# sbokov/AddingDisparityFiltering

Measured on AMD Instinct MI355X. Metric: filtered Mpixels/s (+ achieved HBM GB/s) on 4K disparity, 1/2/4/8 GPUs vs CPU ref, higher is better.
Workload: dtype f32

## Files before the change

addingdisparityfiltering_amd/__init__.py:

```python
from .ximgproc import (
    AM_MAX_TREE_HEIGHT,
    AdaptiveManifoldFilter,
    AdfError,
    BM_COST_CENSUS_CS,
    BM_COST_CENSUS_DENSE,
    BM_COST_CENSUS_SPARSE,
    BM_COST_MCT_DENSE,
    BM_COST_MCT_SPARSE,
    BM_COST_SAD,
    BORDER_CONSTANT,
    BORDER_DEFAULT,
    BORDER_REFLECT,
    BORDER_REFLECT_101,
    BORDER_REPLICATE,
    BORDER_WRAP,
    COLOR_BGR2GRAY,
    CV_16S,
    CV_32F,
    CV_32FC1,
    CV_8U,
    DTF_IC,
    DTF_NC,
    DTF_RF,
    DTFilter,
    DTWindowFilter,
    DT_MAX_ITERS,
    DT_NC_MAX_RADIUS,
    DisparityFilter,
    DisparityWLSFilter,
    FastGlobalSmootherFilter,
    GF_MAX_RADIUS,
    GuidedFilter,
    HANDOFF_IMAGE,
    HANDOFF_IMAGE_PAIR_TAIL,
    HANDOFF_PAIR_PLANE,
    INTER_LINEAR,
    JBF_MAX_RADIUS,
    PATH_CONF_BAND,
    PATH_FUSED_FIRST_PASS,
    PATH_MERGED_PREP,
    PATH_ROW_WEIGHTS_GUIDE,
    PATH_SCALED_FUSED,
    PATH_SCALED_HALF,
    RGF_MAX_ITERS,
    SGBM_COST_BT,
    SGBM_COST_CENSUS_CS,
    SGBM_COST_CENSUS_DENSE,
    SGBM_COST_CENSUS_SPARSE,
    SGBM_COST_MCT_DENSE,
    SGBM_COST_MCT_SPARSE,
    SGBM_RIGHT_FROM_VOLUME,
    SGBM_RIGHT_MATCHER,
    SOLVER_EXACT,
    SOLVER_WAVE,
    StereoBM,
    StereoMatcher,
    StereoSGBM,
    UNKNOWN_DISPARITY,
    WMF_COS,
    WMF_EXP,
    WMF_IV1,
    WMF_IV2,
    WMF_JAC,
    WMF_OFF,
    amFilter,
    amFilterWorkspaceBytes,
    amPlan,
    censusTransform,
    computeBadPixelPercent,
    computeMSE,
    createAMFilter,
    createDTFilter,
    createDTWindowFilter,
    createDisparityWLSFilter,
    createDisparityWLSFilterGeneric,
    createFastGlobalSmootherFilter,
    createGuidedFilter,
    createRightMatcher,
    cvtColor,
    dtFilter,
    dtFilterWorkspaceBytes,
    dtNcRadii,
    dtRfTable,
    dtWindowFilter,
    dtWindowFilterWorkspaceBytes,
    fastGlobalSmootherFilter,
    filterSpeckles,
    releaseCachedMemory,
    getDisparityVis,
    guidedFilter,
    guidedFilterWorkspaceBytes,
    halfSize,
    initUndistortRectifyMap,
    jbfTables,
    jointBilateralFilter,
    matcherViews,
    pointCloud,
    pointCloudWorkspaceBytes,
    readGT,
# ... 17 lines not shown
```

addingdisparityfiltering_amd/_lib.py:

```python
import ctypes as C
import os

_HERE = os.path.dirname(os.path.abspath(__file__))
LIB_PATH = os.environ.get("ADF_WLS_LIB") or os.path.join(_HERE, "libadf_wls.so")

ADF_OK, ADF_EBADARG, ADF_ESIZE, ADF_EHIP, ADF_ENOMEM, ADF_ENODEV = range(6)
SOLVER_EXACT, SOLVER_WAVE = 0, 1
PATH_CONF_BAND, PATH_FUSED_FIRST_PASS, PATH_MERGED_PREP, PATH_SCALED_FUSED, PATH_SCALED_HALF = 1, 2, 4, 8, 16
PATH_ROW_WEIGHTS_GUIDE = 32
HANDOFF_PAIR_PLANE, HANDOFF_IMAGE, HANDOFF_IMAGE_PAIR_TAIL = 0, 1, 2
DEPTH_8U, DEPTH_16S, DEPTH_32S, DEPTH_32F = 0, 3, 4, 5
SGBM_COST_BT, SGBM_COST_CENSUS_DENSE, SGBM_COST_CENSUS_SPARSE = 0, 1, 2
BM_COST_SAD, BM_COST_CENSUS_DENSE, BM_COST_CENSUS_SPARSE = 0, 1, 2
SGBM_COST_MCT_DENSE, SGBM_COST_MCT_SPARSE, SGBM_COST_CENSUS_CS = 4, 5, 6
BM_COST_MCT_DENSE, BM_COST_MCT_SPARSE, BM_COST_CENSUS_CS = 4, 5, 6
SGBM_RIGHT_MATCHER, SGBM_RIGHT_FROM_VOLUME = 0, 1
MISSING_NONE, MISSING_MIN, MISSING_VALUE = 0, 1, 2
WMF_EXP, WMF_IV1, WMF_IV2, WMF_COS, WMF_JAC, WMF_OFF = range(6)
WMF_WEIGHT_ONE, WMF_TABLE_LEVELS, WMF_MAX_RADIUS = 65536, 3 * 256 * 256, 31
GF_MAX_RADIUS = 31
DTF_NC, DTF_IC, DTF_RF, DT_MAX_ITERS = 0, 1, 2, 8
DT_NC_MAX_RADIUS = 127
JBF_MAX_RADIUS = 31
BORDER_REPLICATE, BORDER_REFLECT, BORDER_WRAP, BORDER_REFLECT_101 = 1, 2, 3, 4
RGF_MAX_ITERS = 16
AM_MAX_TREE_HEIGHT = 8


class AdfError(RuntimeError):

    def __init__(self, code, msg):
        super().__init__("adf error %d: %s" % (code, msg))
        self.code = code


class KernelTime(C.Structure):
    _fields_ = [("name", C.c_char * 48), ("launches", C.c_int), ("total_ms", C.c_double),
                ("alg_bytes", C.c_double), ("moved_bytes", C.c_double)]


class Rect(C.Structure):
    _fields_ = [("x", C.c_int), ("y", C.c_int), ("width", C.c_int), ("height", C.c_int)]


class ReprojectParams(C.Structure):
    _fields_ = [("Q", C.c_double * 16), ("disp_scale", C.c_double), ("missing_mode", C.c_int), ("missing_value", C.c_double)]


class RectifyParams(C.Structure):
    _fields_ = [("fx", C.c_double), ("fy", C.c_double), ("cx", C.c_double), ("cy", C.c_double),
                ("dist", C.c_double * 8), ("ir", C.c_double * 9)]


class AmPlan(C.Structure):
    _fields_ = [(k, C.c_int) for k in ("df", "height", "sh", "sw", "manifolds")] + \
               [(k, C.c_float) for k in ("a_root", "a_child", "sr2", "arg_w", "ss", "ratio", "ln_a", "arg_out")]


_vp, _i, _d, _pd, _sz = C.c_void_p, C.c_int, C.c_double, C.c_ssize_t, C.c_size_t
_FILTER_DEV = [_vp, _i, _vp, _pd, _pd, _vp, _pd, _pd, _i, _i, _i, _vp, _pd, _pd, _vp, _pd, _pd,
               C.POINTER(Rect), _vp]
_REPROJECT_DEV = [_i, _vp, _i, _pd, _pd, _i, _i, C.POINTER(ReprojectParams), _vp, _pd, _pd, _i, _vp, _sz, _vp]
_POINT_CLOUD_DEV = [_i, _vp, _i, _pd, _pd, _i, _i, C.POINTER(ReprojectParams), C.POINTER(Rect), _d, _d, _vp, _pd, _pd, _i,
                    _vp, _pd, _vp, _pd, _vp, _pd, _i, _vp, _vp, _sz, _vp]
_RECTIFY_MAP_DEV = [C.POINTER(RectifyParams), _i, _i, _vp, _pd, _vp, _pd, _vp]
_REMAP_DEV = [_i, _vp, _pd, _pd, _i, _i, _i, _vp, _pd, _vp, _pd, _vp, _pd, _pd, _i, _i, _i, _i, _vp, _vp]
_RECTIFY_VIEWS_DEV = [_i, _vp, _pd, _pd, _i, _i, _i, C.POINTER(RectifyParams), _vp, _pd, _pd, _i, _i, _i, _i, _vp, _vp]
_WMF_DEV = [_i, _vp, _pd, _pd, _i, _vp, _pd, _pd, _i, _vp, _pd, _pd, _i, _i, _i, _d, _i, _vp, _pd, _pd, _i, _d, _vp]
_GF_DEV = [_i, _vp, _pd, _pd, _i, _vp, _pd, _pd, _i, _vp, _pd, _pd, _i, _i, _i, _i, _d, _vp, _sz, _vp]
_DT_DEV = [_i, _vp, _pd, _pd, _i, _vp, _pd, _pd, _i, _vp, _pd, _pd, _i, _i, _i, _d, _d, _i, _i, _vp, _sz, _vp]
_JBF_DEV = [_i, _vp, _pd, _pd, _i, _vp, _pd, _pd, _i, _vp, _pd, _pd, _i, _i, _i, _i, _d, _d, _i, _vp]
_AM_DEV = [_i, _vp, _pd, _pd, _i, _vp, _pd, _pd, _i, _vp, _pd, _pd, _i, _i, _i, _d, _d, _i, _i, _vp, _sz, _vp]
_RGF_DEV = [_i, _vp, _pd, _pd, _vp, _pd, _pd, _i, _i, _i, _i, _d, _d, _i, _i, _vp, _sz, _vp]
_FILTER_SCALED_DEV = [_vp, _i, _vp, _pd, _pd, _i, _i, _vp, _pd, _pd, _i, _i, _i, _vp, _pd, _pd, _vp, _pd, _pd,
                      C.POINTER(Rect), _vp]
_FILTER_TYPED_DEV = _FILTER_SCALED_DEV[:5] + [_i] + _FILTER_SCALED_DEV[5:16] + [_i] + _FILTER_SCALED_DEV[16:]
SYMBOLS = [
    ("adf_version", _i, []),
    ("adf_last_error", C.c_char_p, []),
    ("adf_device_count", _i, []),
    ("adf_device_pci_bus_id", _i, [_i, C.c_char_p, _i]),
    ("adf_wls_create", _i, [C.POINTER(_vp), _i, _i, _i, _i, _i, _i]),
    ("adf_wls_destroy", None, [_vp]),
    ("adf_wls_set_lambda", _i, [_vp, _d]),
    ("adf_wls_get_lambda", _i, [_vp, C.POINTER(_d)]),
    ("adf_wls_set_sigma_color", _i, [_vp, _d]),
    ("adf_wls_get_sigma_color", _i, [_vp, C.POINTER(_d)]),
    ("adf_wls_set_lrc_thresh", _i, [_vp, _i]),
    ("adf_wls_get_lrc_thresh", _i, [_vp, C.POINTER(_i)]),
    ("adf_wls_set_depth_discontinuity_radius", _i, [_vp, _i]),
    ("adf_wls_get_depth_discontinuity_radius", _i, [_vp, C.POINTER(_i)]),
    ("adf_wls_set_fgs_params", _i, [_vp, _d, _i]),
    ("adf_wls_set_solver", _i, [_vp, _i]),
    ("adf_wls_get_solver", _i, [_vp, C.POINTER(_i)]),
    ("adf_wls_get_last_solver", _i, [_vp, C.POINTER(_i)]),
    ("adf_wls_get_last_path", _i, [_vp, C.POINTER(_i)]),
    ("adf_wls_get_last_solver_path", _i, [_vp, C.POINTER(_i)]),
    ("adf_wls_get_last_handoff", _i, [_vp, C.POINTER(_i)]),
    ("adf_wls_get_inner_handoffs", _i, [_vp, C.POINTER(_i), C.POINTER(_i)]),
    ("adf_wls_filter_device", _i, _FILTER_DEV),
    ("adf_wls_filter_host", _i, _FILTER_DEV[:-1]),
    ("adf_wls_filter_scaled_device", _i, _FILTER_SCALED_DEV),
    ("adf_wls_filter_scaled_host", _i, _FILTER_SCALED_DEV[:-1]),
    ("adf_wls_filter_f32_device", _i, _FILTER_DEV),
    ("adf_wls_filter_f32_host", _i, _FILTER_DEV[:-1]),
    ("adf_wls_filter_scaled_f32_device", _i, _FILTER_SCALED_DEV),
    ("adf_wls_filter_scaled_f32_host", _i, _FILTER_SCALED_DEV[:-1]),
    ("adf_wls_filter_typed_device", _i, _FILTER_TYPED_DEV),
    ("adf_wls_filter_typed_host", _i, _FILTER_TYPED_DEV[:-1]),
    ("adf_wls_get_confidence_device", _i, [_vp, _i, _vp, _pd, _vp]),
    ("adf_wls_get_confidence_host", _i, [_vp, _i, _vp, _pd]),
    ("adf_wls_get_device", _i, [_vp, C.POINTER(_i)]),
    ("adf_wls_get_roi", _i, [_vp, C.POINTER(Rect)]),
    ("adf_wls_sync", _i, [_vp, _vp]),
    ("adf_wls_workspace_bytes", _sz, [_vp]),
    ("adf_wls_profile_enable", _i, [_vp, _i]),
    ("adf_wls_profile_read", _i, [_vp, _vp, _i, C.POINTER(_i)]),
    ("adf_fgs_create", _i, [C.POINTER(_vp), _vp, _pd, _i, _i, _i, _d, _d, _d, _i, _i]),
    ("adf_fgs_create_device", _i, [C.POINTER(_vp), _vp, _pd, _i, _i, _i, _d, _d, _d, _i, _i, _vp]),
    ("adf_fgs_destroy", None, [_vp]),
    ("adf_release_cached_memory", None, []),
    ("adf_weight_table_host", _i, [C.c_float, _vp, _i]),
    ("adf_fgs_get_device", _i, [_vp, C.POINTER(_i)]),
    ("adf_fgs_get_solver", _i, [_vp, C.POINTER(_i)]),
    ("adf_fgs_filter_host", _i, [_vp, _vp, _pd, _vp, _pd, _i, _i]),
    ("adf_fgs_filter_device", _i, [_vp, _vp, _pd, _vp, _pd, _i, _i, _vp]),
    ("adf_compute_mse_host", _i, [_vp, _pd, _vp, _pd, _i, _i, C.POINTER(Rect), C.POINTER(_d)]),
    ("adf_compute_mse_device", _i, [_vp, _pd, _vp, _pd, _i, _i, C.POINTER(Rect), C.POINTER(_d), _vp]),
    ("adf_compute_bad_pixel_percent_host", _i, [_vp, _pd, _vp, _pd, _i, _i, C.POINTER(Rect), _i, C.POINTER(_d)]),
    ("adf_compute_bad_pixel_percent_device", _i, [_vp, _pd, _vp, _pd, _i, _i, C.POINTER(Rect), _i, C.POINTER(_d), _vp]),
    ("adf_get_disparity_vis_host", _i, [_vp, _pd, _vp, _pd, _i, _i, _d]),
    ("adf_get_disparity_vis_device", _i, [_vp, _pd, _vp, _pd, _i, _i, _d, _vp]),
    ("adf_bm_create", _i, [C.POINTER(_vp), _i, _i]),
    ("adf_bm_destroy", None, [_vp]),
    ("adf_bm_set_params", _i, [_vp, _i, _i, _i, _i, _i, _i]),
    ("adf_bm_get_device", _i, [_vp, C.POINTER(_i)]),
    ("adf_bm_get_params", _i, [_vp] + [C.POINTER(_i)] * 6),
    ("adf_bm_set_cost", _i, [_vp, _i, _i]),
    ("adf_bm_get_cost", _i, [_vp, C.POINTER(_i), C.POINTER(_i)]),
    ("adf_bm_compute_device", _i, [_vp, _i, _vp, _pd, _pd, _vp, _pd, _pd, _i, _i, _vp, _pd, _pd, _vp]),
    ("adf_bm_compute_both_device", _i, [_vp, _i, _vp, _pd, _pd, _vp, _pd, _pd, _i, _i, _vp, _pd, _pd, _vp, _pd, _pd, _vp]),
    ("adf_bm_compute_host", _i, [_vp, _i, _vp, _pd, _pd, _vp, _pd, _pd, _i, _i, _vp, _pd, _pd]),
    ("adf_bm_compute_cost_device", _i, [_vp, _i, _vp, _pd, _pd, _vp, _pd, _pd, _i, _i, _vp, _pd, _pd, _vp, _pd, _pd, _vp]),
    ("adf_bm_compute_cost_host", _i, [_vp, _i, _vp, _pd, _pd, _vp, _pd, _pd, _i, _i, _vp, _pd, _pd, _vp, _pd, _pd]),
    ("adf_bm_compute_both_cost_device", _i, [_vp, _i, _vp, _pd, _pd, _vp, _pd, _pd, _i, _i] + [_vp, _pd, _pd] * 4 + [_vp]),
    ("adf_sgbm_create", _i, [C.POINTER(_vp), _i, _i, _i]),
    ("adf_sgbm_destroy", None, [_vp]),
    ("adf_sgbm_get_device", _i, [_vp, C.POINTER(_i)]),
    ("adf_sgbm_set_params", _i, [_vp] + [_i] * 8),
    ("adf_sgbm_get_params", _i, [_vp] + [C.POINTER(_i)] * 8),
    ("adf_sgbm_set_disp12_max_diff", _i, [_vp, _i]),
    ("adf_sgbm_get_disp12_max_diff", _i, [_vp, C.POINTER(_i)]),
    ("adf_sgbm_set_cost", _i, [_vp, _i, _i]),
    ("adf_sgbm_get_cost", _i, [_vp, C.POINTER(_i), C.POINTER(_i)]),
    ("adf_sgbm_compute_device", _i, [_vp, _i, _vp, _pd, _pd, _vp, _pd, _pd, _i, _i, _i, _vp, _pd, _pd, _vp]),
    ("adf_sgbm_compute_host", _i, [_vp, _i, _vp, _pd, _pd, _vp, _pd, _pd, _i, _i, _i, _vp, _pd, _pd]),
    ("adf_sgbm_compute_both_device", _i, [_vp, _i, _vp, _pd, _pd, _vp, _pd, _pd, _i, _i, _i, _vp, _pd, _pd, _vp, _pd, _pd, _i, _vp]),
    ("adf_sgbm_compute_both_host", _i, [_vp, _i, _vp, _pd, _pd, _vp, _pd, _pd, _i, _i, _i, _vp, _pd, _pd, _vp, _pd, _pd, _i]),
    ("adf_census_transform_device", _i, [_i, _vp, _pd, _pd, _i, _i, _i, _i, _vp, _pd, _pd, _vp]),
    ("adf_census_transform_host", _i, [_i, _vp, _pd, _pd, _i, _i, _i, _i, _vp, _pd, _pd]),
    ("adf_filter_speckles_workspace_bytes", _sz, [_i, _i, _i]),
    ("adf_filter_speckles_device", _i, [_i, _vp, _pd, _pd, _i, _i, _i, _i, _i, _vp, _sz, _vp]),
    ("adf_filter_speckles_host", _i, [_i, _vp, _pd, _pd, _i, _i, _i, _i, _i]),
    ("adf_validate_disparity_device", _i, [_i, _vp, _pd, _pd, _vp, _pd, _pd, _i, _i, _i, _i, _i, _i, _vp]),
    ("adf_validate_disparity_host", _i, [_i, _vp, _pd, _pd, _vp, _pd, _pd, _i, _i, _i, _i, _i, _i]),
    ("adf_half_size", _i, [_i, C.POINTER(_i)]),
    ("adf_prepare_views_device", _i, [_i, _vp, _pd, _pd, _i, _i, _i, _vp, _pd, _pd, _i, _i, _i, _vp]),
    ("adf_prepare_views_host", _i, [_i, _vp, _pd, _pd, _i, _i, _i, _vp, _pd, _pd, _i, _i, _i]),
    ("adf_reproject_workspace_bytes", _sz, [_i]),
    ("adf_reproject_to_3d_device", _i, _REPROJECT_DEV),
    ("adf_reproject_to_3d_host", _i, _REPROJECT_DEV[:-3]),
    ("adf_point_cloud_workspace_bytes", _sz, [_i, _i, _i]),
    ("adf_point_cloud_device", _i, _POINT_CLOUD_DEV),
    ("adf_point_cloud_host", _i, _POINT_CLOUD_DEV[:-3]),
    ("adf_rectify_params_init", _i, [_vp, _vp, _i, _vp, _vp, _i, C.POINTER(RectifyParams)]),
    ("adf_init_undistort_rectify_map_device", _i, _RECTIFY_MAP_DEV),
    ("adf_init_undistort_rectify_map_host", _i, _RECTIFY_MAP_DEV[:-1]),
    ("adf_remap_device", _i, _REMAP_DEV),
    ("adf_remap_host", _i, _REMAP_DEV[:-1]),
    ("adf_rectify_views_device", _i, _RECTIFY_VIEWS_DEV),
    ("adf_rectify_views_host", _i, _RECTIFY_VIEWS_DEV[:-1]),
    ("adf_wmf_weight_table_host", _i, [_d, _i, _vp, _i]),
    ("adf_weighted_median_filter_device", _i, _WMF_DEV),
    ("adf_weighted_median_filter_host", _i, _WMF_DEV[:-1]),
    ("adf_guided_filter_workspace_bytes", _sz, [_i, _i, _i, _i]),
    ("adf_guided_filter_device", _i, _GF_DEV),
    ("adf_guided_filter_host", _i, _GF_DEV[:-3]),
    ("adf_dt_filter_workspace_bytes", _sz, [_i, _i, _i]),
    ("adf_dt_rf_table_host", _i, [_d, _d, _i, _i, _vp]),
    ("adf_dt_filter_device", _i, _DT_DEV),
    ("adf_dt_filter_host", _i, _DT_DEV[:-3]),
    ("adf_dt_window_filter_workspace_bytes", _sz, [_i, _i, _i]),
    ("adf_dt_nc_radii_host", _i, [_d, _i, _vp]),
    ("adf_dt_window_filter_device", _i, _DT_DEV),
    ("adf_dt_window_filter_host", _i, _DT_DEV[:-3]),
    ("adf_jbf_tables_host", _i, [_i, _d, _d, _i, _vp, _vp, C.POINTER(_i)]),
    ("adf_joint_bilateral_filter_device", _i, _JBF_DEV),
    ("adf_joint_bilateral_filter_host", _i, _JBF_DEV[:-1]),
    ("adf_rolling_guidance_workspace_bytes", _sz, [_i, _i, _i, _i, _i]),
    ("adf_rgf_tables_host", _i, [_i, _i, _d, _d, _vp, _vp, C.POINTER(_i), C.POINTER(_i), C.POINTER(C.c_float)]),
    ("adf_rolling_guidance_filter_device", _i, _RGF_DEV),
    ("adf_rolling_guidance_filter_host", _i, _RGF_DEV[:-3]),
    ("adf_am_plan_host", _i, [_d, _d, _i, _i, _i, C.POINTER(AmPlan), _vp]),
    ("adf_am_exp_host", _i, [_vp, _vp, _sz]),
    ("adf_am_filter_workspace_bytes", _sz, [_i, _i, _i, _i, _d, _d, _i]),
# ... 38 lines not shown
```

addingdisparityfiltering_amd/csrc/adf_api.hip:

```cpp
#include "adf_host.h"

#include <cmath>
#include <cstdio>
#include <cstdlib>
#include <cstring>
#include <new>

using namespace adf;

static inline int round_up(int v, int m) { return (v + m - 1) / m * m; }
template <class T> static const T* pairs_on(const T* p, ptrdiff_t pair_stride, int k)
{
    return p ? (const T*)((const char*)p + (ptrdiff_t)k * pair_stride) : nullptr;
}

static Geom make_geom(int W, int H, int rx, int ry, int rw, int rh)
{
    Geom g;
    g.W = W; g.H = H; g.rx = rx; g.ry = ry; g.rw = rw; g.rh = rh;
    g.pw = round_up(rw, 64);
    g.ph = round_up(rh, 64);
    size_t a = (size_t)round_up(rh, TILE_ROWS) * g.pw, b = (size_t)rw * g.ph;
    g.plane = ((a > b ? a : b) + 63) / 64 * 64;
    g.frame = (size_t)W * H;
// ... 1 lines not shown
    g.cpitch = round_up(W + g.cx0 + 3, 4);
    g.cframe = (size_t)g.cpitch * H;
    return g;
}

static Geom plain_conf_layout(Geom g) { g.cx0 = 0; g.cpitch = g.W; g.cframe = g.frame; return g; }

enum KClass { K_FILL = 0, K_WEIGHTS, K_DISC, K_LRC, K_PROLOGUE, K_PASS_H_FIRST, K_PASS_H, K_PASS_V, K_PASS_V_LAST, K_RESIZE, K_QUANT, K_COUNT };
static const char* const kclass_names[K_COUNT] = {"fill_outside", "weights", "discontinuity", "lrc_confidence",
                                                  "plain_prologue", "pass_h_first", "pass_h", "pass_v", "pass_v_last", "resize", "quantise_maps"};
struct Bytes { double alg, moved; };
static Bytes same_bytes(double b) { return Bytes{b, b}; }
static Bytes fill_bytes(double outside, bool conf, double out_b) { return same_bytes(((conf ? 4.0 : 0.0) + out_b) * outside); }
static Bytes weights_bytes(double P, int gch, bool chor) { return same_bytes((gch + (chor ? 8.0 : 4.0)) * P); }
static Bytes disc_bytes(double P, bool both) { return both ? Bytes{4.0 * P, 12.0 * P} : Bytes{2.0 * P, 6.0 * P}; }
static Bytes band_bytes(double P) { return same_bytes(8.0 * P); }
static Bytes merged_bytes(double P, double outside, int gch, double out_b) { return same_bytes((8.0 + gch + 8.0) * P + (4.0 + out_b) * outside); }
static Bytes conf_left_bytes(double P, bool rhs) { const double wu = rhs ? 8.0 : 0.0; return Bytes{(4.0 + wu) * P, (12.0 + wu) * P}; }
static Bytes lrc_bytes(double F, double P, bool rhs, double map_b, double fill)
{
    return Bytes{4.0 * F + (rhs ? 8.0 * P : 0.0) + fill, 4.0 * F + (rhs ? 18.0 + map_b : 12.0) * P + fill};
}
static Bytes prologue_bytes(double P, bool weighted, double map_b) { return same_bytes(((weighted ? 12.0 : 4.0) + map_b) * P); }
static Bytes resize_bytes(double dst_px, double src_px, double elem_b) { return same_bytes(elem_b * dst_px + elem_b * src_px); }
static Bytes quant_bytes(double px, bool q, bool right, bool v) { return same_bytes(((right ? 8.0 : 4.0) + (q ? (right ? 4.0 : 2.0) : 0.0) + (v ? 4.0 : 0.0)) * px); }

struct Profiler {
    bool on = false;
    struct Rec { int cls; hipEvent_t a, b; double alg, moved; };
    std::vector<Rec> recs;
    std::vector<hipEvent_t> pool;
    hipEvent_t get()
    {
        if (!pool.empty()) { hipEvent_t e = pool.back(); pool.pop_back(); return e; }
        hipEvent_t e = nullptr;
        if (hipEventCreate(&e) != hipSuccess) return nullptr;
        return e;
    }
    void clear() { for (auto& r : recs) { pool.push_back(r.a); pool.push_back(r.b); } recs.clear(); }
    void destroy() { clear(); for (auto e : pool) hipEventDestroy(e); pool.clear(); }
};
struct ProfScope {
    Profiler* p; hipStream_t st; Profiler::Rec r{};
    ProfScope(Profiler* prof, int cls, double alg, double moved, hipStream_t s) : p(prof && prof->on ? prof : nullptr), st(s)
    {
        if (!p) return;
        r.cls = cls; r.alg = alg; r.moved = moved; r.a = p->get(); r.b = p->get();
        if (r.a) hipEventRecord(r.a, st);
    }
    ProfScope(Profiler* prof, int cls, Bytes b, hipStream_t s) : ProfScope(prof, cls, b.alg, b.moved, s) {}
    ~ProfScope()
    {
        if (!p) return;
        if (r.b) hipEventRecord(r.b, st);
        if (r.a && r.b) p->recs.push_back(r);
    }
};

struct SolvePlanes {
    float* CH; float* CV;
    float* D; float* F0; float* F1;
    float* A0; float* A1;
    float* B0; float* B1;
};

struct FinalOut {
    int epilogue; void* out; ptrdiff_t stride, pair_stride; int x0, y0, cn, c;
};

static double epilogue_bytes(int epilogue)
{
    return (epilogue == EPI_F32 || epilogue == EPI_WLS_CONF_F32) ? 4.0 : epilogue == EPI_U8 ? 1.0 : 2.0;
}

template <class Args>
static void set_final_out(Args& a, const FinalOut& fo)
{
    a.out = fo.out; a.out_stride = fo.stride; a.out_pair_stride = fo.pair_stride;
    a.out_x0 = fo.x0; a.out_y0 = fo.y0; a.out_cn = fo.cn; a.out_c = fo.c;
}

struct HandoffImage {
    float* image = nullptr; int m = 0; bool inner = false, first = false;
    bool at(int it, int num_iter) const
    {
        if (!image || num_iter < 2) return false;
        return it == num_iter - 1 ? true : it > 0 ? inner : first;
    }
    int inner_count(int num_iter) const
    {
        int n = 0;
        for (int it = 0; it + 1 < num_iter; it++) n += at(it, num_iter);
        return n;
    }
};

static int run_passes(bool wave, const Geom& g, const SolvePlanes& p, int n_rhs, float lambda, float atten, int num_iter,
                      const FinalOut& fo, int n_pairs, hipStream_t st, Profiler* prof = nullptr,
                      const FusedInputs* fuse = nullptr, const GuideWeights* gw = nullptr, const HandoffImage& ho = HandoffImage{})
{
    const double px = (double)g.rw * g.rh * n_pairs;
    float lam = lambda;
    for (int it = 0; it < num_iter; it++, lam *= atten) {
        const bool fused = it == 0 && fuse, last = it == num_iter - 1;
        const int epi = last ? fo.epilogue : EPI_PLANES;
        const double lo_b = (fused && fuse->lo_conf) ? 6.0 * fuse->lo_scale_x * fuse->lo_scale_y : (fused && fuse->dl_f32) ? 8.0 : 6.0;
        const double wb = gw ? (double)gw->ch : 4.0;
        const double hb = fused ? (wb + lo_b + 8.0) * px : (wb + 8.0 * n_rhs) * px;
        const double out_b = (last ? epilogue_bytes(fo.epilogue) : 4.0 * n_rhs) * px;
        const double vb = (4.0 + 4.0 * n_rhs) * px + out_b;
        if (wave) {
            WavePassArgs h{}, v{};
            h.C = p.CH; h.U0 = p.A0; h.U1 = p.A1;
            h.nscan = g.rh; h.len = g.rw; h.pitch = g.pw; h.plane = g.plane; h.lambda = lam;
            if (fused) h.fuse = *fuse;
            if (gw) h.gw = *gw;
            v.C = p.CV; v.U0 = p.A0; v.U1 = p.A1;
            v.nscan = g.rw; v.len = g.rh; v.pitch = g.pw; v.plane = g.plane; v.lambda = lam;
            if (last) set_final_out(v, fo);
            if (ho.at(it, num_iter)) {
                h.image = v.image = ho.image; h.image_m = v.image_m = ho.m;
                h.image_plane = v.image_plane = wave_image_floats(g.pw, ho.m);
            }
            {
                ProfScope ps(prof, fused ? K_PASS_H_FIRST : K_PASS_H, hb, hb, st);
                HIP_TRY(launch_wave_hpass(h, n_rhs, n_pairs, st));
            }
            ProfScope ps(prof, last ? K_PASS_V_LAST : K_PASS_V, vb, vb, st);
            HIP_TRY(launch_wave_vpass(v, n_rhs, epi, n_pairs, st));
        } else {
            PassArgs h{}, v{};
            h.C = p.CH; h.U0 = p.A0; h.U1 = p.A1; h.D = p.D; h.F0 = p.F0; h.F1 = p.F1; h.O0 = p.B0; h.O1 = p.B1;
            h.nscan = g.rh; h.len = g.rw; h.pitch_in = g.ph; h.pitch_out = g.pw; h.plane = g.plane; h.lambda = lam;
            v.C = p.CV; v.U0 = p.B0; v.U1 = p.B1; v.D = p.D; v.F0 = p.F0; v.F1 = p.F1; v.O0 = p.A0; v.O1 = p.A1;
            v.nscan = g.rw; v.len = g.rh; v.pitch_in = g.pw; v.pitch_out = g.ph; v.plane = g.plane; v.lambda = lam;
            if (last) set_final_out(v, fo);
            {
                ProfScope ps(prof, K_PASS_H, hb, (12.0 + 16.0 * n_rhs) * px, st);
                HIP_TRY(launch_exact_pass(h, n_rhs, EPI_PLANES, n_pairs, st));
            }
            ProfScope ps(prof, last ? K_PASS_V_LAST : K_PASS_V, vb, (12.0 + 12.0 * n_rhs) * px + out_b, st);
            HIP_TRY(launch_exact_pass(v, n_rhs, epi, n_pairs, st));
        }
    }
    return ADF_OK;
}

static bool wave_fits(const Geom& g)
{
    return g.rw >= 2 && g.rh >= 2 && g.rw <= wave_max_row_len() && g.rh <= wave_max_col_len();
}

struct ConfResize {
    float* clo; int dW, dH; adf_rect rlo;
    Geom ghi;
    bool band_map;
    int n_pairs;
};

constexpr long long HANDOFF_IMAGE_MIN_PX = 12LL * 3584 * 2160;

struct adf_wls {
    int device = 0;
    int left_offset = 0, right_offset = 0, top_offset = 0, bottom_offset = 0;
    int min_disp = 0;
    bool use_confidence = true;
    double lambda = 8000.0, sigma_color = 1.0;
    int lrc_thresh = 24, disc_radius = 5;
    float roll_off = 0.001f;
    double atten = 0.25; int num_iter = 3;
    int solver = ADF_SOLVER_WAVE;
    int last_solver = ADF_SOLVER_WAVE;
    adf_rect roi{0, 0, 0, 0};
    int last_W = 0, last_H = 0, last_pairs = 0;
    int last_cpitch = 0, last_cx0 = 0;
    long long conf_sig[4] = {0, 0, 0, 0};
    int last_path = 0;
    int last_solver_path = 0;
    Lut lut;
    DevBuf ws;
    DevBuf conf;
    DevBuf stage;
    DevBuf scaled;
    size_t ws_limit = (size_t)64 << 30;
    Profiler prof;
    long long ws_sig[8] = {0, 0, 0, 0, 0, 0, 0, 0};
    hipStream_t side = nullptr;
    hipEvent_t ev_fork = nullptr, ev_join = nullptr;
    bool overlap = true;
    struct LazyConf { bool pending = false; ConfResize resize{}; } lazy_conf;
    bool scaled_half = true;
    bool scaled_fuse = true;
    bool conf_band = true;
    bool merge_small = true;
    bool row_weights_guide = true;
    bool handoff_image = true;
    bool handoff_inner = true;
    long long handoff_min_px = HANDOFF_IMAGE_MIN_PX;
    int last_handoff = ADF_HANDOFF_PAIR_PLANE;
    int last_inner[2] = {0, 0};
    static bool null_caller_of(hipStream_t s) { return s == nullptr || s == hipStreamLegacy || s == hipStreamPerThread; }
    int ensure_side(hipStream_t caller)
    {
        if (side) return ADF_OK;
        int least = 0, greatest = 0, prio = 0, cp = 0;
        if (hipDeviceGetStreamPriorityRange(&least, &greatest) != hipSuccess) { least = greatest = 0; (void)hipGetLastError(); }
        if (null_caller_of(caller) || stream_is_capturing(caller) || hipStreamGetPriority(caller, &cp) != hipSuccess) { cp = 0; (void)hipGetLastError(); }
        prio = (cp != greatest) ? greatest : (greatest < least ? greatest + 1 : greatest);
        if (null_caller_of(caller)) HIP_TRY(hipStreamCreateWithFlags(&side, hipStreamNonBlocking));
        else HIP_TRY(hipStreamCreateWithPriority(&side, hipStreamNonBlocking, prio));
        HIP_TRY(hipEventCreateWithFlags(&ev_fork, hipEventDisableTiming));
        HIP_TRY(hipEventCreateWithFlags(&ev_join, hipEventDisableTiming));
        return ADF_OK;
    }
};

extern "C" int adf_wls_create(adf_wls_t** out, int use_confidence, int l, int r, int t, int b, int min_disp)
{
    if (!out) return fail(ADF_EBADARG, "adf_wls_create: out is NULL");
    *out = nullptr;
    if (l < 0 || r < 0 || t < 0 || b < 0) return fail(ADF_EBADARG, "adf_wls_create: negative offset");
    int n = 0;
    if (hipGetDeviceCount(&n) != hipSuccess || n <= 0)
        return fail(ADF_ENODEV, "adf_wls_create: no HIP device visible");
    adf_wls* h = new (std::nothrow) adf_wls();
    if (!h) return fail(ADF_ENOMEM, "adf_wls_create: out of host memory");
    if (hipGetDevice(&h->device) != hipSuccess) { delete h; return fail(ADF_EHIP, "hipGetDevice failed"); }
    h->use_confidence = use_confidence != 0;
    h->left_offset = l; h->right_offset = r; h->top_offset = t; h->bottom_offset = b;
    h->min_disp = 0; (void)min_disp;
    if (const char* e = getenv("ADF_WS_LIMIT_GB")) {
        double gb = atof(e);
        if (gb > 0) h->ws_limit = (size_t)(gb * (double)((size_t)1 << 30));
    }
    if (const char* e = getenv("ADF_NO_OVERLAP")) h->overlap = atoi(e) == 0;
    if (const char* e = getenv("ADF_CONF_BAND")) h->conf_band = atoi(e) != 0;
    if (const char* e = getenv("ADF_SCALED_FUSE")) h->scaled_fuse = atoi(e) != 0;
    if (const char* e = getenv("ADF_ROW_WEIGHTS_GUIDE")) h->row_weights_guide = atoi(e) != 0;
    if (const char* e = getenv("ADF_LO_HALF")) h->scaled_half = atoi(e) != 0;
    if (const char* e = getenv("ADF_LAST_HANDOFF_IMAGE")) h->handoff_image = atoi(e) != 0;
    if (const char* e = getenv("ADF_INNER_HANDOFF_IMAGE")) h->handoff_inner = atoi(e) != 0;
    if (const char* e = getenv("ADF_LAST_HANDOFF_MIN_PX")) h->handoff_min_px = atoll(e);
    if (const char* e = getenv("ADF_MERGE_SMALL")) h->merge_small = atoi(e) != 0;
    *out = h;
    return ADF_OK;
}

extern "C" void adf_wls_destroy(adf_wls_t* h)
{
    if (!h) return;
    DeviceScope ds(h->device);
    h->lut.release(); h->ws.release(); h->conf.release(); h->stage.release(); h->scaled.release();
    h->prof.destroy();
    if (h->ev_fork) hipEventDestroy(h->ev_fork);
    if (h->ev_join) hipEventDestroy(h->ev_join);
    if (h->side) hipStreamDestroy(h->side);
    delete h;
}


extern "C" int adf_wls_set_lambda(adf_wls_t* h, double v) { NEED_HANDLE(h); h->lambda = v; return ADF_OK; }
extern "C" int adf_wls_get_lambda(const adf_wls_t* h, double* v) { NEED_HANDLE(h); if (v) *v = h->lambda; return ADF_OK; }
extern "C" int adf_wls_set_sigma_color(adf_wls_t* h, double v) { NEED_HANDLE(h); h->sigma_color = v; return ADF_OK; }
extern "C" int adf_wls_get_sigma_color(const adf_wls_t* h, double* v) { NEED_HANDLE(h); if (v) *v = h->sigma_color; return ADF_OK; }
extern "C" int adf_wls_set_lrc_thresh(adf_wls_t* h, int v) { NEED_HANDLE(h); h->lrc_thresh = v; return ADF_OK; }
extern "C" int adf_wls_get_lrc_thresh(const adf_wls_t* h, int* v) { NEED_HANDLE(h); if (v) *v = h->lrc_thresh; return ADF_OK; }
extern "C" int adf_wls_set_depth_discontinuity_radius(adf_wls_t* h, int v) { NEED_HANDLE(h); h->disc_radius = v; return ADF_OK; }
extern "C" int adf_wls_get_depth_discontinuity_radius(const adf_wls_t* h, int* v) { NEED_HANDLE(h); if (v) *v = h->disc_radius; return ADF_OK; }

extern "C" int adf_wls_set_fgs_params(adf_wls_t* h, double atten, int num_iter)
{
    NEED_HANDLE(h);
    if (num_iter < 1) return fail(ADF_EBADARG, "num_iter must be >= 1 (FGS.cpp:143)");
    h->atten = atten; h->num_iter = num_iter;
    return ADF_OK;
}

extern "C" int adf_wls_set_solver(adf_wls_t* h, int solver)
{
    NEED_HANDLE(h);
    if (solver != ADF_SOLVER_EXACT && solver != ADF_SOLVER_WAVE) return fail(ADF_EBADARG, "unknown solver %d", solver);
    h->solver = solver;
    return ADF_OK;
}
extern "C" int adf_wls_get_solver(const adf_wls_t* h, int* v) { NEED_HANDLE(h); if (v) *v = h->solver; return ADF_OK; }
extern "C" int adf_wls_get_last_solver(const adf_wls_t* h, int* v) { NEED_HANDLE(h); if (v) *v = h->last_solver; return ADF_OK; }
extern "C" int adf_wls_get_last_path(const adf_wls_t* h, int* v) { NEED_HANDLE(h); if (v) *v = h->last_path; return ADF_OK; }
extern "C" int adf_wls_get_last_solver_path(const adf_wls_t* h, int* v) { NEED_HANDLE(h); if (v) *v = h->last_solver_path; return ADF_OK; }
extern "C" int adf_wls_get_last_handoff(const adf_wls_t* h, int* v) { NEED_HANDLE(h); if (v) *v = h->last_handoff; return ADF_OK; }

extern "C" int adf_wls_get_inner_handoffs(const adf_wls_t* h, int* full, int* tail)
{
    NEED_HANDLE(h);
    if (full) *full = h->last_inner[0];
    if (tail) *tail = h->last_inner[1];
    return ADF_OK;
}

extern "C" int adf_wls_get_device(const adf_wls_t* h, int* device) { NEED_HANDLE(h); if (device) *device = h->device; return ADF_OK; }
extern "C" int adf_wls_get_roi(const adf_wls_t* h, adf_rect* roi) { NEED_HANDLE(h); if (roi) *roi = h->roi; return ADF_OK; }
extern "C" size_t adf_wls_workspace_bytes(const adf_wls_t* h)
{
    return h ? h->ws.bytes + h->conf.bytes + h->stage.bytes + h->scaled.bytes + h->lut.bytes() : 0;
}

extern "C" int adf_wls_sync(adf_wls_t* h, void* stream)
{
    NEED_HANDLE(h);
    DeviceScope ds(h->device);
    HIP_TRY(hipStreamSynchronize((hipStream_t)stream));
    return ADF_OK;
}

static int ensure_conf_planes(adf_wls* h, const Geom& g, int n_pairs, hipStream_t st)
{
    int rc = h->conf.reserve(g.cframe * sizeof(float) * (size_t)n_pairs, st, FILL_ZERO);
    if (rc) return rc;
    const long long sig[4] = {g.W, g.H, g.cx0, n_pairs};
    if (memcmp(sig, h->conf_sig, sizeof(sig)) != 0) {
        HIP_TRY(hipMemsetAsync(h->conf.p, 0, h->conf.bytes, st));
        memcpy(h->conf_sig, sig, sizeof(sig));
    }
    return ADF_OK;
}

static int quant_pitch(int W) { return round_up(W, 8); }

static size_t wls_pair_ws_bytes(const Geom& g, bool conf, bool wave, bool disc_maps, bool quant_planes, int image_m = 0, bool image_in_chor = false)
{
    size_t planes = wave ? (conf ? 4 : 3) : (conf ? 9 : 6);
    return planes * g.plane * sizeof(float) + (conf && disc_maps ? 2 * g.frame * sizeof(float) : 0) +
           (image_m ? (wave_image_floats(g.pw, image_m) - (image_in_chor ? g.plane : 0)) * sizeof(float) : 0) +
           (quant_planes ? 2 * (size_t)quant_pitch(g.W) * g.H * sizeof(int16_t) : 0);
}

static int resolve_roi(const adf_wls* h, const adf_rect* roi_in, int w, int hgt, adf_rect& roi)
{
    if (roi_in && roi_in->width * roi_in->height != 0) roi = *roi_in;
    else roi = adf_rect{h->left_offset, h->top_offset, w - h->left_offset - h->right_offset, hgt - h->top_offset - h->bottom_offset};
    if (roi.width <= 0 || roi.height <= 0 || roi.x < 0 || roi.y < 0 || roi.x + roi.width > w || roi.y + roi.height > hgt)
        return fail(ADF_ESIZE, "ROI (%d,%d,%d,%d) does not fit a %dx%d map", roi.x, roi.y, roi.width, roi.height, w, hgt);
    return ADF_OK;
}

struct OutMap {
    void* p; ptrdiff_t stride, pair_stride; bool f32;
    size_t esz() const { return f32 ? sizeof(float) : sizeof(int16_t); }
};

struct DispMaps {
    const void* L; ptrdiff_t sL, psL;
    const void* R; ptrdiff_t sR, psR;
    bool f32;
    size_t esz() const { return f32 ? sizeof(float) : sizeof(int16_t); }
    DispMaps from(int k) const { return DispMaps{pairs_on(L, psL, k), sL, psL, pairs_on(R, psR, k), sR, psR, f32}; }
};

struct View { const uint8_t* p; ptrdiff_t stride, pair_stride; int ch, W, H; };

struct WlsCall {
    int n_pairs;
    DispMaps dm; int dW, dH;
    View view;
    OutMap om;
    adf_rect rlo, rhi;
    float resize_factor, x_ratio;
    bool scaled;
};

static int no_right_map() { return fail(ADF_EBADARG, "disparity_map_right is required with use_confidence"); }
static int bad_view_channels() { return fail(ADF_EBADARG, "left_view must be CV_8UC1 or CV_8UC3"); }

static int check_float_maps(const DispMaps& dm, int n_pairs, int dW, int dH, const OutMap& om, int W, int H)
{
    if (!dm.f32) return ADF_OK;
    if ((reinterpret_cast<uintptr_t>(dm.L) | (uintptr_t)dm.sL | (uintptr_t)dm.psL) & 3u ||
        (dm.R && ((reinterpret_cast<uintptr_t>(dm.R) | (uintptr_t)dm.sR | (uintptr_t)dm.psR) & 3u)))
        return fail(ADF_EBADARG, "a float disparity map needs a 4-byte aligned base and strides");
// ... 160 lines not shown
    CONF_SCALED_LO,
    CONF_MERGED,
    CONF_BAND,
    CONF_LEFT,
    CONF_TWO_KERNEL,
};

enum RhsSource {
    RHS_PLAIN,
    RHS_FUSED_VIEW,
    RHS_FUSED_LO,
    RHS_CONF_PROLOGUE,
    RHS_CONF_KERNEL,
};

struct ConfRule { int rrx, thresh, radius; float roll_off; };
static ConfRule conf_rule(const adf_wls* h, const WlsCall& c)
{
    return ConfRule{c.dW - (c.rlo.x + c.rlo.width),
                    (int)(c.resize_factor * h->lrc_thresh),
                    h->disc_radius, h->roll_off / (c.resize_factor * c.resize_factor)};
}

struct ConfOut {
    float* conf;
    float* cL; float* cR;
    float* U0; float* U1; int orient;
    const OutsideArgs* fill;
};

static ConfBandArgs conf_band_args(const MapSource& m, float* conf, const Geom& g, const ConfRule& r)
{
    return ConfBandArgs{m.L, m.sL, m.psL, m.R, m.sR, m.psR, conf, g, r.rrx, r.thresh, r.radius, r.roll_off, 0};
}

static DiscArgs disc_args(const MapSource& m, const ConfOut& o, const Geom& g, const ConfRule& r, int only_view)
{
    return DiscArgs{{m.L, m.R}, {m.sL, m.sR}, {m.psL, m.psR}, {g.rx, r.rrx}, g.ry, g.rw, g.rh, r.radius, r.roll_off,
                    {o.cL, o.cR}, g.W, g.frame, only_view};
}

static LrcArgs lrc_args(const MapSource& m, const ConfOut& o, const Geom& g, const ConfRule& r)
{
    const bool own_f32 = o.U0 && m.rhs_f32();
    LrcArgs a = LrcArgs{m.L, m.sL, m.psL, m.R, m.sR, m.psR, o.cL, o.cR, o.conf, nullptr, 0, 0, 0, 0, o.U0, o.U1,
                        g, r.rrx, r.thresh, o.orient, own_f32 ? 1 : 0};
    if (own_f32) { a.dL = (const int16_t*)m.rhs; a.sL = m.s_rhs; a.psL = m.ps_rhs; }
    if (o.fill) { a.out = o.fill->out; a.sO = o.fill->stride; a.psO = o.fill->pair_stride; a.fill = o.fill->fill; a.out_f32 = o.fill->out_f32; }
    return a;
}

static int conf_stage(Profiler* prof, ConfStage kind, const MapSource& m, const Geom& g, const ConfRule& r, const ConfOut& o,
                      int n, hipStream_t st)
{
    const double F = (double)g.frame * n, P = (double)g.rw * g.rh * n;
    if (kind == CONF_BAND) {
        ProfScope ps(prof, K_LRC, band_bytes(P), st);
        HIP_TRY(launch_conf_band(conf_band_args(m, o.conf, g, r), n, st));
        return ADF_OK;
    }
    {
        ProfScope ps(prof, K_DISC, disc_bytes(P, kind != CONF_LEFT), st);
        HIP_TRY(launch_discontinuity(disc_args(m, o, g, r, kind == CONF_LEFT ? 1 : -1), n, st));
    }
    if (kind == CONF_LEFT) {
        ConfLeftArgs ca{m.L, m.sL, m.psL, m.R, m.sR, m.psR, o.cR, o.conf, o.U0, o.U1, g, r.rrx, r.thresh, r.radius, r.roll_off};
        ProfScope ps(prof, K_LRC, conf_left_bytes(P, o.U0 != nullptr), st);
        HIP_TRY(launch_conf_left(ca, n, st));
        return ADF_OK;
    }
    const double fill = o.fill ? fill_bytes(F - P, false, o.fill->out_f32 ? 4.0 : 2.0).alg : 0.0;
    ProfScope ps(prof, K_LRC, lrc_bytes(F, P, o.U0 != nullptr, m.rhs_f32() ? 4.0 : 2.0, fill), st);
    HIP_TRY(launch_lrc_prologue(lrc_args(m, o, g, r), n, st));
    return ADF_OK;
}

struct ChunkPlan {
    ConfStage stage;
    bool fork_weights;
    bool outside_on_side;
    bool guide_rows;
    bool image;
    bool inner_image;
};

struct WlsPlan {
    Geom g;
    bool wave;
    RhsSource rhs;
    bool band;
    bool quant_planes;
    Geom glo; bool lo_band; size_t dhi_bytes;
    size_t per_pair; int chunk;
    int image_m;
    bool image_in_chor;
    bool first_image;
    ChunkPlan full, tail;
    int path;
    int solver_path;
    bool fused_first() const { return rhs == RHS_FUSED_VIEW || rhs == RHS_FUSED_LO; }
};

static ChunkPlan plan_chunk(const adf_wls* h, ConfStage stage, bool wave, bool guide_rows, bool image, bool inner_image)
{
    const bool fork = stage != CONF_NONE && stage != CONF_MERGED && h->overlap;
    return ChunkPlan{stage, fork, fork && wave && stage != CONF_TWO_KERNEL, guide_rows && stage != CONF_MERGED, image, image && inner_image};
}

static GuideWeights guide_weights(const adf_wls* h, const uint8_t* guide, const View& v, const Geom& g)
{
    return GuideWeights{guide, v.stride, v.pair_stride, v.ch, g.rx, g.ry, h->lut.cur};
}

static WlsPlan plan_wls(const adf_wls* h, const WlsCall& c)
{
    WlsPlan p{};
    const bool conf = h->use_confidence, f32in = c.dm.f32;
    const View& v = c.view;
    const Geom g = p.g = make_geom(v.W, v.H, c.rhi.x, c.rhi.y, c.rhi.width, c.rhi.height);
    p.wave = h->solver == ADF_SOLVER_WAVE && wave_fits(g);
    MapSource m = caller_maps(c.dm);
    bool fuse_lo = false;
    if (c.scaled) {
        p.glo = plain_conf_layout(make_geom(c.dW, c.dH, c.rlo.x, c.rlo.y, c.rlo.width, c.rlo.height));
        p.lo_band = conf && h->conf_band && conf_band_fits(p.glo, h->disc_radius);
        fuse_lo = conf && !f32in && h->scaled_fuse && p.wave &&
                  wave_hpass_can_fuse_lo(first_pass_probe(lo_fuse(h, c, p.lo_band, UNALLOCATED, m, nullptr, g), g.rw));
        p.dhi_bytes = fuse_lo ? 0 : pad_to((size_t)v.W * v.H * c.dm.esz(), 256);
        m.rhs = fuse_lo ? nullptr : UNALLOCATED; m.s_rhs = (ptrdiff_t)(v.W * c.dm.esz()); m.ps_rhs = (ptrdiff_t)p.dhi_bytes;
        m.rhs_depth = f32in ? ADF_32F : ADF_16S;
    }
    ConfStage stage = !conf ? CONF_NONE
                    : c.scaled ? (fuse_lo ? CONF_SCALED_LO : CONF_SCALED)
                    : (p.wave && h->disc_radius <= conf_left_max_radius()) ? CONF_LEFT : CONF_TWO_KERNEL;
    const float* planes = h->conf.p ? (const float*)h->conf.p : UNALLOCATED;
    const bool fused_view = ((stage == CONF_SCALED && !f32in) || stage == CONF_LEFT) && p.wave &&
                            wave_hpass_can_fuse(first_pass_probe(view_fuse(planes, m, g), g.rw));
    p.band = stage == CONF_LEFT && fused_view && h->conf_band && conf_band_fits(g, h->disc_radius);
    if (p.band) stage = CONF_BAND;
    p.quant_planes = f32in && conf && !c.scaled;
    p.rhs = stage == CONF_NONE ? RHS_PLAIN : stage == CONF_SCALED_LO ? RHS_FUSED_LO : fused_view ? RHS_FUSED_VIEW
          : (stage == CONF_SCALED || (stage == CONF_LEFT && p.quant_planes)) ? RHS_CONF_PROLOGUE : RHS_CONF_KERNEL;
    bool guide_rows = false;
    if (p.wave && !c.scaled && h->row_weights_guide) {
        WavePassArgs probe{};
        probe.len = g.rw; probe.gw = guide_weights(h, v.p, v, g);
        WeightArgs wprobe{};
        wprobe.stride = v.stride; wprobe.ch = v.ch; wprobe.chor_orient = ORIENT_N; wprobe.g = g;
        guide_rows = wave_hpass_guide_fits(probe) && weights_stream_fits(wprobe);
    }
    const int image_m = (conf && p.wave && h->handoff_image && h->num_iter >= 2 && wave_hpass_image_fits(g.rw)) ? wave_vpass_image_m(g.rh) : 0;
    const long long roi_px = (long long)g.rw * g.rh;
    const bool may_merge = p.band && h->merge_small && prep_small_fits(g, h->disc_radius, v.ch, 1) && prep_small_guide_fits(g, v.stride, v.ch);
    auto chunk_for = [&](int im) {
        p.image_m = im;
        p.image_in_chor = im && guide_rows && !may_merge;
        p.per_pair = wls_pair_ws_bytes(g, conf, p.wave, !p.band, p.quant_planes, im, p.image_in_chor);
        p.chunk = (int)(h->ws_limit / p.per_pair);
        if (p.chunk < 1) p.chunk = 1;
        if (p.chunk > c.n_pairs) p.chunk = c.n_pairs;
    };
    chunk_for(image_m);
    if (image_m && roi_px * p.chunk < h->handoff_min_px) chunk_for(0);
    auto chunk_of = [&](int n) {
        const bool merged = p.band && h->merge_small && prep_small_fits(g, h->disc_radius, v.ch, n) && prep_small_guide_fits(g, v.stride, v.ch);
        return plan_chunk(h, merged ? CONF_MERGED : stage, p.wave, guide_rows, p.image_m && roi_px * n >= h->handoff_min_px, h->handoff_inner);
    };
    p.first_image = p.rhs == RHS_FUSED_VIEW && wave_hpass_first_image(view_fuse(planes, m, g));
    p.full = chunk_of(p.chunk);
    p.tail = chunk_of(c.n_pairs % p.chunk ? c.n_pairs % p.chunk : p.chunk);
    p.path = ((p.band || p.lo_band) ? ADF_PATH_CONF_BAND : 0) |
             (p.fused_first() ? ADF_PATH_FUSED_FIRST_PASS : 0) |
             ((p.full.stage == CONF_MERGED || p.tail.stage == CONF_MERGED) ? ADF_PATH_MERGED_PREP : 0);
    p.solver_path = (p.full.guide_rows || p.tail.guide_rows) ? ADF_PATH_ROW_WEIGHTS_GUIDE : 0;
    if (p.rhs == RHS_FUSED_LO)
        p.path |= ADF_PATH_SCALED_FUSED |
                  (wave_hpass_lo_half(first_pass_probe(lo_fuse(h, c, p.lo_band, UNALLOCATED, m, nullptr, g), g.rw)) ? ADF_PATH_SCALED_HALF : 0);
    return p;
}

struct ScaledBufs { char* dhi; float *cl, *cr, *clo; float* taps; };

static int scaled_buffers(adf_wls_t* h, const WlsCall& c, const WlsPlan& plan, hipStream_t st, ScaledBufs& b, MapSource& lo)
{
    const bool conf = h->use_confidence, f32in = c.dm.f32, fuse_lo = plan.rhs == RHS_FUSED_LO;
    const size_t n = (size_t)c.n_pairs, lo_px = (size_t)c.dW * c.dH;
    const size_t qframe = (size_t)quant_pitch(c.dW) * c.dH;
    const size_t maps_bytes = pad_to(n * (plan.dhi_bytes + (conf ? 3 * lo_px * sizeof(float) : 0)), 256);
    const size_t taps_bytes = pad_to(fuse_lo ? 2 * ((size_t)c.rhi.width + 4) * sizeof(float) : 0, 256);
    const size_t quant_bytes = f32in ? n * qframe * (4 + (conf ? 4 : 0)) : 0;
    int rc = h->scaled.reserve(maps_bytes + taps_bytes + quant_bytes, st, FILL_ZERO);
    if (rc) return rc;
    b.dhi = (char*)h->scaled.p;
    b.cl = (float*)(b.dhi + n * plan.dhi_bytes);
    b.cr = b.cl + n * lo_px;
    b.clo = b.cr + n * lo_px;
    b.taps = fuse_lo ? (float*)(b.dhi + maps_bytes) : nullptr;
    if (conf && (rc = ensure_conf_planes(h, plan.g, c.n_pairs, st))) return rc;
    lo = caller_maps(c.dm);
    if (f32in) {
        float* v = (float*)(b.dhi + maps_bytes + taps_bytes);
        int16_t* qL = conf ? (int16_t*)(v + n * qframe) : nullptr;
        int16_t* qR = conf ? qL + n * qframe : nullptr;
        if ((rc = quantise_maps(&h->prof, c.dm, c.dW, c.dH, c.n_pairs, qL, qR, v, st, lo))) return rc;
    }
    lo.rhs = fuse_lo ? nullptr : b.dhi; lo.s_rhs = (ptrdiff_t)(c.view.W * c.dm.esz()); lo.ps_rhs = (ptrdiff_t)plan.dhi_bytes;
    lo.rhs_depth = f32in ? ADF_32F : ADF_16S;
    return ADF_OK;
}

static int scaled_conf_maps(adf_wls_t* h, const WlsCall& c, const WlsPlan& plan, const ScaledBufs& b, const MapSource& lo,
                            const ConfRule& rule, hipStream_t st)
{
    Profiler* prof = &h->prof;
    int rc = conf_stage(prof, plan.lo_band ? CONF_BAND : CONF_TWO_KERNEL, lo, plan.glo, rule, ConfOut{b.clo, b.cl, b.cr}, c.n_pairs, st);
    if (rc) return rc;
    const ConfResize cr{b.clo, c.dW, c.dH, c.rlo, plan.g, plan.lo_band, c.n_pairs};
    if (plan.rhs != RHS_FUSED_LO)
        return (rc = resize_conf_planes(h, cr, st, prof)) ? rc : resize_disparity(prof, c, lo, b.dhi, st);
    if (stream_is_capturing(st)) return resize_conf_planes(h, cr, st, prof);
    h->lazy_conf = adf_wls::LazyConf{true, cr};
    return ADF_OK;
}

static int wls_filter_impl(adf_wls_t* h, const WlsCall& c, const WlsPlan& plan, hipStream_t st)
{
    const bool conf = h->use_confidence, wave = plan.wave;
    const Geom& g = plan.g;
    const View& vw = c.view;
    const OutMap& om = c.om;
    const adf_rect& roi = c.rhi;
    const int n_pairs = c.n_pairs, W = vw.W, H = vw.H, gch = vw.ch;
    const double ob_px = (double)om.esz(), db_px = (double)c.dm.esz();
    Profiler* prof = &h->prof;
    int rc;
    ScaledBufs sb{};
    MapSource lo{};
    if (c.scaled && (rc = scaled_buffers(h, c, plan, st, sb, lo))) return rc;
    h->roi = roi; h->last_W = W; h->last_H = H; h->last_pairs = n_pairs;
    h->last_cpitch = g.cpitch; h->last_cx0 = g.cx0; h->last_path = 0; h->last_solver_path = 0;
    h->last_solver = wave ? ADF_SOLVER_WAVE : ADF_SOLVER_EXACT;
    h->last_handoff = ADF_HANDOFF_PAIR_PLANE; h->last_inner[0] = h->last_inner[1] = 0;
    if ((rc = h->ws.reserve(plan.per_pair * (size_t)plan.chunk, st, FILL_ZERO))) return rc;
    if (conf && !c.scaled && (rc = ensure_conf_planes(h, g, n_pairs, st))) return rc;
    {
        const long long sig[8] = {W, H, roi.x, roi.y, roi.width, roi.height,
                                  (long long)plan.image_in_chor * 1024 + (long long)plan.image_m * 16 + (long long)plan.quant_planes * 8 + (long long)plan.band * 4 + (long long)wave * 2 + conf, plan.chunk};
        if (memcmp(sig, h->ws_sig, sizeof(sig)) != 0) {
            HIP_TRY(hipMemsetAsync(h->ws.p, 0, h->ws.bytes, st));
            memcpy(h->ws_sig, sig, sizeof(sig));
        }
    }
    float* base = (float*)h->ws.p;
    auto take = [&](size_t elems) { float* p = base; base += elems * (size_t)plan.chunk; return p; };
    SolvePlanes p{};
    p.CH = take(g.plane);
    float* const image_rest = plan.image_in_chor ? take(wave_image_floats(g.pw, plan.image_m) - g.plane) : nullptr;
    (void)image_rest;
    p.CV = take(g.plane); p.A0 = take(g.plane);
    if (!wave) { p.D = take(g.plane); p.F0 = take(g.plane); p.B0 = take(g.plane); }
    float *cL = nullptr, *cR = nullptr;
    if (conf) {
        p.A1 = take(g.plane);
        if (!wave) { p.F1 = take(g.plane); p.B1 = take(g.plane); }
    }
    float* const image = !plan.image_m ? nullptr : plan.image_in_chor ? p.CH : take(wave_image_floats(g.pw, plan.image_m));
    const size_t qframe = (size_t)quant_pitch(W) * H;
    int16_t* const qL = plan.quant_planes ? (int16_t*)take(qframe) : nullptr;
    int16_t* const qR = qL ? qL + qframe * (size_t)plan.chunk : nullptr;
    if (conf && !plan.band) { cL = take(g.frame); cR = take(g.frame); }
    const int orient_h = wave ? ORIENT_N : ORIENT_T;
    const int orient_u2 = wave ? ORIENT_PAIR : ORIENT_T;
    const int orient_cv = wave ? ORIENT_STRIP : ORIENT_N;
    const int16_t fill = (int16_t)(16 * (h->min_disp - 1));
    const ConfRule rule = conf_rule(h, c);
    h->last_path = plan.path; h->last_solver_path = plan.solver_path;
    auto handoff_of = [&](const ChunkPlan& cp) { return HandoffImage{cp.image ? image : nullptr, plan.image_m, cp.inner_image, cp.inner_image && plan.first_image}; };
    if (wave) { h->last_inner[0] = handoff_of(plan.full).inner_count(h->num_iter); h->last_inner[1] = handoff_of(plan.tail).inner_count(h->num_iter); }
    h->last_handoff = (plan.full.image && plan.tail.image) ? ADF_HANDOFF_IMAGE : plan.full.image ? ADF_HANDOFF_IMAGE_PAIR_TAIL : ADF_HANDOFF_PAIR_PLANE;

    for (int first = 0; first < n_pairs; first += plan.chunk) {
        const int n = (n_pairs - first < plan.chunk) ? n_pairs - first : plan.chunk;
        const ChunkPlan& cp = n == plan.chunk ? plan.full : plan.tail;
        const uint8_t* gv = pairs_on(vw.p, vw.pair_stride, first);
        void* o = (char*)om.p + (ptrdiff_t)first * om.pair_stride;
        float* confp = conf ? (float*)h->conf.p + (size_t)first * g.cframe : nullptr;
        const double F = (double)g.frame * n, P = (double)g.rw * g.rh * n;
        MapSource m = c.scaled ? lo.from(first) : caller_maps(c.dm).from(first);
        OutsideArgs oa{o, om.stride, om.pair_stride, fill, om.f32 ? 1 : 0, c.scaled ? nullptr : confp, g};
        auto fill_outside = [&](hipStream_t s) {
            ProfScope ps(prof, K_FILL, fill_bytes(F - P, oa.conf != nullptr, ob_px), s);
            return launch_outside(oa, n, s);
        };
        WeightArgs wa{gv, vw.stride, vw.pair_stride, gch, h->lut.cur, cp.guide_rows ? nullptr : p.CH, p.CV, orient_h, orient_cv, g,
                      wave ? nullptr : p.B0};
        const GuideWeights gw = guide_weights(h, gv, vw, g);
        auto prologue = [&](bool weighted) {
            PlainPrologueArgs pa{m.rhs, m.s_rhs, m.ps_rhs, m.rhs_depth, 1, 0, p.A0, g, weighted ? orient_u2 : orient_h};
            if (weighted) { pa.conf = confp; pa.U1 = p.A1; }
            ProfScope ps(prof, K_PROLOGUE, prologue_bytes(P, weighted, db_px), st);
            return launch_plain_prologue(pa, n, st);
        };

        hipStream_t wst = st;
        if (cp.fork_weights) {
            if ((rc = h->ensure_side(st))) return rc;
            HIP_TRY(hipEventRecord(h->ev_fork, st));
            HIP_TRY(hipStreamWaitEvent(h->side, h->ev_fork, 0));
            wst = h->side;
        }
        if (cp.stage == CONF_NONE || cp.outside_on_side) HIP_TRY(fill_outside(wst));
        if (cp.stage == CONF_NONE && c.scaled && first == 0 && (rc = resize_disparity(prof, c, lo, sb.dhi, st))) return rc;
        if (cp.stage != CONF_MERGED) {
            ProfScope ps(prof, K_WEIGHTS, weights_bytes(P, gch, !cp.guide_rows), wst);
            HIP_TRY(launch_weights(wa, n, wst));
        }
        if (cp.fork_weights) HIP_TRY(hipEventRecord(h->ev_join, h->side));
        if (plan.quant_planes &&
            (rc = quantise_maps(prof, c.dm.from(first), W, H, n, qL, qR, nullptr, st, m))) return rc;
        switch (cp.stage) {
        case CONF_NONE:
            break;
        case CONF_SCALED:
        case CONF_SCALED_LO:
            if (!cp.outside_on_side) HIP_TRY(fill_outside(st));
            if (first == 0 && (rc = scaled_conf_maps(h, c, plan, sb, lo, rule, st))) return rc;
            break;
        case CONF_MERGED: {
            ProfScope ps(prof, K_LRC, merged_bytes(P, F - P, gch, ob_px), st);
            HIP_TRY(launch_prep_small(conf_band_args(m, confp, g, rule), wa, oa, n, st));
            break;
        }
        case CONF_BAND:
        case CONF_LEFT:
        case CONF_TWO_KERNEL: {
            ConfOut out{confp, cL, cR};
            if (plan.rhs == RHS_CONF_KERNEL) { out.U0 = p.A0; out.U1 = p.A1; out.orient = orient_u2; }
            if (cp.stage == CONF_TWO_KERNEL) out.fill = &oa;
            if ((rc = conf_stage(prof, cp.stage, m, g, rule, out, n, st))) return rc;
            if (cp.stage != CONF_TWO_KERNEL && !cp.outside_on_side) HIP_TRY(fill_outside(st));
            break;
        }
        }
        if (plan.rhs == RHS_PLAIN || plan.rhs == RHS_CONF_PROLOGUE) HIP_TRY(prologue(plan.rhs == RHS_CONF_PROLOGUE));
        if (cp.fork_weights) HIP_TRY(hipStreamWaitEvent(st, h->ev_join, 0));
        const FusedInputs fuse = plan.rhs == RHS_FUSED_LO
            ? lo_fuse(h, c, plan.lo_band, sb.clo + (size_t)first * c.dW * c.dH, m, sb.taps, g) : view_fuse(confp, m, g);
        const int epi = conf ? (om.f32 ? EPI_WLS_CONF_F32 : EPI_WLS_CONF) : (om.f32 ? EPI_F32 : EPI_I16);
        FinalOut fo{epi, o, om.stride, om.pair_stride, roi.x, roi.y, 1, 0};
        rc = run_passes(wave, g, p, conf ? 2 : 1, (float)h->lambda, (float)h->atten, h->num_iter, fo, n, st, prof,
                        plan.fused_first() ? &fuse : nullptr, cp.guide_rows ? &gw : nullptr, handoff_of(cp));
        if (rc) return rc;
    }
    return ADF_OK;
}

static int wls_filter_device(adf_wls_t* h, int n_pairs, const DispMaps& dm, int dW, int dH, const View& view, const OutMap& om,
                             const adf_rect* roi, hipStream_t st)
{
    NEED_HANDLE(h);
    WlsCall c;
    int rc = check_call(h, n_pairs, dm, dW, dH, view, om, roi, c);
    if (rc) return rc;
    DeviceScope ds(h->device);
    h->lazy_conf.pending = false;
    if ((rc = h->lut.ensure((float)h->sigma_color, st))) return rc;
    const WlsPlan plan = plan_wls(h, c);
    rc = wls_filter_impl(h, c, plan, st);
    if (rc == ADF_ENOMEM && plan.image_m) {
        const bool keep = h->handoff_image;
        h->handoff_image = false;
        rc = wls_filter_impl(h, c, plan_wls(h, c), st);
        h->handoff_image = keep;
    }
    if (c.scaled) h->roi = c.rlo;
    return rc;
}

// ... 340 lines not shown
```

addingdisparityfiltering_amd/csrc/adf_host.h:

```cpp
#pragma once

#include "adf_internal.h"
#include "../../include/adf_wls.h"

#include <algorithm>
#include <memory>
#include <vector>

namespace adf {

int fail(int code, const char* fmt, ...);

#define HIP_TRY(expr)                                                                              \
    do {                                                                                           \
        hipError_t e_ = (expr);                                                                    \
        if (e_ != hipSuccess)                                                                      \
            return adf::fail(e_ == hipErrorOutOfMemory ? ADF_ENOMEM : ADF_EHIP, "%s failed: %s",   \
                             #expr, hipGetErrorString(e_));                                        \
    } while (0)
#define NEED_HANDLE(h) do { if (!(h)) return adf::fail(ADF_EBADARG, "%s: handle is NULL", __func__); } while (0)

struct DeviceScope {
    int prev = -1; bool switched = false;
    explicit DeviceScope(int dev)
// ... 16 lines not shown
        if (int rc = f(m0, nm = std::min(n - m0, per_launch))) return rc;
    return ADF_OK;
}

template <class ARGS, class POINT>
ADF_LOCAL int launch_tiles(void (*kernel)(ARGS), size_t lds, int W, int H, int tile_w, int tile_h, int n, ARGS a, hipStream_t st, POINT&& point)
{
    if (lds > 48 * 1024 - 1024) HIP_TRY(hipFuncSetAttribute(reinterpret_cast<const void*>(kernel), hipFuncAttributeMaxDynamicSharedMemorySize, (int)lds));
    const unsigned tiles_y = (unsigned)((H + tile_h - 1) / tile_h);
    a.tiles_x = (unsigned)((W + tile_w - 1) / tile_w);
    const uint64_t tiles = (uint64_t)a.tiles_x * tiles_y;
    constexpr uint64_t PER_LAUNCH = 1u << 22;
    return for_batches(n, GRID_LIMIT, [&](int m0, unsigned nm) {
        point(a, m0);
        for (uint64_t t0 = 0; t0 < tiles; t0 += PER_LAUNCH) {
            a.tile0 = (unsigned)t0;
            hipLaunchKernelGGL(kernel, dim3((unsigned)std::min(tiles - t0, PER_LAUNCH), nm), dim3((unsigned)(tile_w * tile_h)), lds, st, a);
        }
        return launched();
    });
}

ADF_LOCAL bool images_disjoint(int n, ptrdiff_t row_bytes, int rows, ptrdiff_t stride, ptrdiff_t image_stride, bool may_interleave);

constexpr bool known_depth(int depth) { return depth == ADF_8U || depth == ADF_16S || depth == ADF_32F; }
constexpr size_t depth_size(int depth) { return depth == ADF_8U ? 1 : depth == ADF_16S ? 2 : 4; }
inline bool aligned(const void* p, ptrdiff_t stride, ptrdiff_t map_stride, ptrdiff_t es)
{
    return !(((uintptr_t)p & (es - 1)) || (stride & (es - 1)) || (map_stride & (es - 1)));
}
struct Span { uintptr_t lo, hi; };
inline Span span_of(const void* p, int n, ptrdiff_t row_bytes, int rows, ptrdiff_t stride, ptrdiff_t map_stride)
{
    const uintptr_t b = reinterpret_cast<uintptr_t>(p);
    return Span{b, b + (uintptr_t)((ptrdiff_t)(n - 1) * map_stride + (ptrdiff_t)(rows - 1) * stride + row_bytes)};
}
inline bool overlap(Span a, Span b) { return a.lo < b.hi && b.lo < a.hi; }
ADF_LOCAL int border_check(const char* who, int border);

struct FilterImage {
    void* p; ptrdiff_t stride, map_stride;
    uint8_t* map(int m0) const { return static_cast<uint8_t*>(p) + (ptrdiff_t)m0 * map_stride; }
};
struct FilterImages {
    int n, W, H;
    FilterImage guide; int guide_channels;
    FilterImage src; int src_depth;
    FilterImage dst; int dst_depth;
    FilterImage mask;
};
inline FilterImage image_of(const void* p, ptrdiff_t stride, ptrdiff_t map_stride) { return FilterImage{const_cast<void*>(p), stride, map_stride}; }
ADF_LOCAL int filter_geometry_check(const char* who, const FilterImages& im, const char* depths, const char* inputs);

enum Fill { FILL_NONE, FILL_ZERO };
struct DevBuf {
    void* p = nullptr; size_t bytes = 0;
    int reserve(size_t need, hipStream_t st, Fill fill);
    void release() { if (p) hipFree(p); p = nullptr; bytes = 0; }
};

hipError_t device_malloc(void** p, size_t bytes);
void* cache_take(int device, size_t need, hipStream_t st, size_t* bytes);
void cache_give(int device, void* p, size_t bytes, hipStream_t st);
void cache_give_event(int device, void* p, size_t bytes, hipEvent_t ready);

struct Scratch {
    int device = 0; void* p = nullptr; size_t bytes = 0; hipStream_t st = nullptr;
    Scratch() = default;
    Scratch(const Scratch&) = delete;
    Scratch& operator=(const Scratch&) = delete;
    int take(size_t need, hipStream_t stream);
    ~Scratch() { if (p) cache_give(device, p, bytes, st); }
};

ADF_LOCAL int workspace_or_scratch(const char* who, const char* size_fn, void* workspace, size_t workspace_bytes, size_t need,
                                   hipStream_t st, Scratch& blk, void** ws);

struct LutTable;
struct Lut {
    static constexpr int LUT_CACHE = 8;
    struct Entry { std::shared_ptr<LutTable> t; unsigned long long used; };
    std::vector<Entry> tables;
    const float* cur = nullptr;
    unsigned long long tick = 0;
    size_t bytes() const { return tables.size() * sizeof(float) * ADF_LUT_LEVELS; }
    int ensure(float s, hipStream_t st);
    void release() { tables.clear(); cur = nullptr; }
};

struct WmfTable;
ADF_LOCAL int wmf_weights_check(const char* who, double sigma, int weight_type);
ADF_LOCAL int wmf_table_device(double sigma, int weight_type, std::shared_ptr<WmfTable>& out, const uint32_t** dev);

struct JbfTable;
ADF_LOCAL int jbf_params_check(const char* who, int d, double sigma_color, double sigma_space, int joint_channels,
                               double* sc, double* ss, int* r);
constexpr size_t jbf_colour_entries(int channels) { return (size_t)255 * channels + 1; }
constexpr size_t jbf_space_entries(int r) { return (size_t)r * r + 1; }
ADF_LOCAL int jbf_table_device(double sc, double ss, int r, int channels, std::shared_ptr<JbfTable>& out,
                               const float** colour, const float** space);

struct RgfTable;
constexpr size_t RGF_GRID_ENTRIES = 4098;
ADF_LOCAL int rgf_params_check(const char* who, int depth, int d, double sigma_color, double sigma_space,
                               double* sc, double* ss, int* r, float* scale);
ADF_LOCAL size_t rgf_colour_entries(int depth, double sc);
ADF_LOCAL int rgf_table_device(int depth, double sc, double ss, int r, std::shared_ptr<RgfTable>& out,
                               const float** colour, const float** space, int* entries);

int copy_images(void* dst, size_t dst_pitch, ptrdiff_t dst_image_stride, const void* src, size_t src_pitch,
                ptrdiff_t src_image_stride, size_t row_bytes, size_t rows, int n, hipMemcpyKind kind, hipStream_t st);

template <class RUN> int staged_call(const FilterImages& host, size_t ws_bytes, RUN&& run)
{
    FilterImages dev = host;
    const FilterImage* from[4] = {&host.guide, &host.src, &host.mask, &host.dst};
    FilterImage* to[4] = {&dev.guide, &dev.src, &dev.mask, &dev.dst};
    const size_t pixel[4] = {(size_t)host.guide_channels, depth_size(host.src_depth), 1, depth_size(host.dst_depth)};
    size_t row[4], at[5] = {0};
    for (int k = 0; k < 4; k++) {
        row[k] = from[k]->p ? pixel[k] * (size_t)host.W : 0;
        at[k + 1] = at[k] + pad_to(row[k] * (size_t)host.H * (size_t)host.n, 256);
    }
    Scratch blk;
    if (int rc = blk.take(at[4] + ws_bytes, nullptr)) return rc;
    char* base = static_cast<char*>(blk.p);
    for (int k = 0; k < 4; k++) {
        if (!row[k]) continue;
        *to[k] = FilterImage{base + at[k], (ptrdiff_t)row[k], (ptrdiff_t)(row[k] * (size_t)host.H)};
        if (k == 3) break;
        if (int rc = copy_images(to[k]->p, row[k], to[k]->map_stride, from[k]->p, (size_t)from[k]->stride, from[k]->map_stride, row[k],
                                 (size_t)host.H, host.n, hipMemcpyHostToDevice, nullptr))
            return rc;
    }
    if (int rc = run(dev, static_cast<void*>(base + at[4]), (hipStream_t)nullptr)) return rc;
    HIP_TRY(hipStreamSynchronize(nullptr));
    if (int rc = copy_images(host.dst.p, (size_t)host.dst.stride, host.dst.map_stride, dev.dst.p, row[3], dev.dst.map_stride, row[3],
                             (size_t)host.H, host.n, hipMemcpyDeviceToHost, nullptr))
        return rc;
    HIP_TRY(hipStreamSynchronize(nullptr));
    return ADF_OK;
}

}
```

addingdisparityfiltering_amd/csrc/adf_host.hip:

```cpp
#include "adf_host.h"

#include <cmath>
#include <cstdarg>
#include <cstdio>
#include <mutex>
#include <thread>

using namespace adf;

static thread_local char g_err[512] = "";

int adf::fail(int code, const char* fmt, ...)
{
    va_list ap;
    va_start(ap, fmt);
    vsnprintf(g_err, sizeof(g_err), fmt, ap);
    va_end(ap);
    return code;
}

extern "C" int adf_version(void) { return ADF_VERSION; }
extern "C" const char* adf_last_error(void) { return g_err; }
extern "C" int adf_device_count(void)
{
    int n = 0;
    if (hipGetDeviceCount(&n) != hipSuccess) return 0;
    return n;
}

extern "C" int adf_device_pci_bus_id(int device, char* buf, int len)
{
    if (!buf || len < 16) return fail(ADF_EBADARG, "adf_device_pci_bus_id: buffer of at least 16 bytes required");
    buf[0] = 0;
    HIP_TRY(hipDeviceGetPCIBusId(buf, len, device));
    return ADF_OK;
}

bool adf::stream_is_capturing(hipStream_t st)
{
    hipStreamCaptureStatus cs = hipStreamCaptureStatusNone;
    if (hipStreamIsCapturing(st, &cs) != hipSuccess) { (void)hipGetLastError(); return false; }
    return cs != hipStreamCaptureStatusNone;
}

int adf::launched()
{
    const hipError_t e = hipGetLastError();
    return e != hipSuccess ? fail(ADF_EHIP, "%s", hipGetErrorString(e)) : ADF_OK;
}

bool adf::images_disjoint(int n, ptrdiff_t row_bytes, int rows, ptrdiff_t stride, ptrdiff_t image_stride, bool may_interleave)
{
    if (n < 2 || image_stride >= stride * (rows - 1) + row_bytes) return true;
    return may_interleave && image_stride >= row_bytes && image_stride * (n - 1) + row_bytes <= stride;
}

int adf::border_check(const char* who, int border)
{
    if (border == 0 || border == 3)
        return fail(ADF_EBADARG, "%s: %s is not built; BORDER_REPLICATE, BORDER_REFLECT and BORDER_REFLECT_101 are", who, border == 0 ? "BORDER_CONSTANT" : "BORDER_WRAP");
    if (border != ADF_BORDER_REPLICATE && border != ADF_BORDER_REFLECT && border != ADF_BORDER_REFLECT_101)
        return fail(ADF_EBADARG, "%s: borderType %d is not built; BORDER_REPLICATE (1), BORDER_REFLECT (2) and BORDER_REFLECT_101 (4) are", who, border);
    return ADF_OK;
}

int adf::filter_geometry_check(const char* who, const FilterImages& im, const char* depths, const char* inputs)
{
    const FilterImage &g = im.guide, &s = im.src, &d = im.dst, &m = im.mask;
    const ptrdiff_t ss = (ptrdiff_t)depth_size(im.src_depth), ds = (ptrdiff_t)depth_size(im.dst_depth);
    if (!aligned(s.p, s.stride, s.map_stride, ss) || !aligned(d.p, d.stride, d.map_stride, ds))
        return fail(ADF_EBADARG, "%s: src and dst and their strides must be aligned to %s", who, depths);
    if ((int64_t)im.W * im.H >= ((int64_t)1 << 31)) return fail(ADF_ESIZE, "%s: W*H must be below 2^31", who);
    const ptrdiff_t srow = (ptrdiff_t)im.W * ss, drow = (ptrdiff_t)im.W * ds, grow = (ptrdiff_t)im.W * im.guide_channels, mrow = im.W;
    if (s.stride < srow || d.stride < drow || (g.p && g.stride < grow) || (m.p && m.stride < mrow))
        return fail(ADF_ESIZE, "%s: row stride smaller than a row", who);
    if (im.n > 1 && (s.map_stride < 0 || (g.p && g.map_stride < 0) || (m.p && m.map_stride < 0)))
        return fail(ADF_ESIZE, "%s: map strides must not be negative", who);
    if (!images_disjoint(im.n, drow, im.H, d.stride, d.map_stride, false))
        return fail(ADF_ESIZE, "%s: destination maps of the batch overlap (map stride smaller than a map)", who);
    const Span out = span_of(d.p, im.n, drow, im.H, d.stride, d.map_stride);
    if (overlap(out, span_of(s.p, im.n, srow, im.H, s.stride, s.map_stride)) ||
        (g.p && overlap(out, span_of(g.p, im.n, grow, im.H, g.stride, g.map_stride))) ||
        (m.p && overlap(out, span_of(m.p, im.n, mrow, im.H, m.stride, m.map_stride))))
        return fail(ADF_EBADARG, "%s: dst must not overlap %s", who, inputs);
    return ADF_OK;
}

int adf::DevBuf::reserve(size_t need, hipStream_t st, Fill fill)
{
    if (need <= bytes) return ADF_OK;
    if (p) { HIP_TRY(hipStreamSynchronize(st)); HIP_TRY(hipFree(p)); p = nullptr; bytes = 0; }
    need = pad_to(need, 256);
    HIP_TRY(device_malloc(&p, need));
    bytes = need;
    if (fill == FILL_ZERO) HIP_TRY(hipMemsetAsync(p, 0, need, st));
    return ADF_OK;
}

template <class T, class KEY> struct ADF_LOCAL DeviceTable {
    using Elem = T;
    using Key = KEY;
    int device = 0; KEY key{}; size_t count = 0; T* dev = nullptr;
    DeviceTable() = default;
    DeviceTable(const DeviceTable&) = delete;
    DeviceTable& operator=(const DeviceTable&) = delete;
    ~DeviceTable() { if (dev) { DeviceScope ds(device); hipFree(dev); } }
};
struct adf::LutTable : DeviceTable<float, float> {};

template <class TABLE> struct TableStore {
    static constexpr size_t CAP = 16;
    std::mutex m;
    std::vector<std::shared_ptr<TABLE>> tables;
    static TableStore& get() { static TableStore* s = new TableStore; return *s; }
    template <class SAME> std::shared_ptr<TABLE> find(SAME&& same)
    {
        std::lock_guard<std::mutex> lk(m);
        for (size_t k = 0; k < tables.size(); k++)
            if (same(*tables[k])) {
                auto t = tables[k];
                tables.erase(tables.begin() + (ptrdiff_t)k); tables.push_back(t);
                return t;
            }
        return nullptr;
    }
    void add(const std::shared_ptr<TABLE>& t)
    {
        std::lock_guard<std::mutex> lk(m);
        if (tables.size() >= CAP) tables.erase(tables.begin());
        tables.push_back(t);
    }
    void clear() { std::lock_guard<std::mutex> lk(m); tables.clear(); }
};
using LutStore = TableStore<LutTable>;

template <class TABLE, class COUNT, class BUILD>
static int table_device(const char* what, const typename TABLE::Key& key, COUNT&& count, BUILD&& build, std::shared_ptr<TABLE>& out)
{
    using Elem = typename TABLE::Elem;
    int device = 0;
    if (hipGetDevice(&device) != hipSuccess) return fail(ADF_ENODEV, "no HIP device");
    out = TableStore<TABLE>::get().find([&](const TABLE& q) { return q.device == device && q.key == key; });
    if (out) return ADF_OK;
    std::vector<Elem> host(count());
    build(host.data());
    Elem* d = nullptr;
    HIP_TRY(device_malloc(reinterpret_cast<void**>(&d), sizeof(Elem) * host.size()));
    hipError_t e = hipMemcpy(d, host.data(), sizeof(Elem) * host.size(), hipMemcpyHostToDevice);
    if (e != hipSuccess) { hipFree(d); return fail(ADF_EHIP, "%s table upload failed: %s", what, hipGetErrorString(e)); }
    out = std::make_shared<TABLE>();
    out->device = device; out->key = key; out->count = host.size(); out->dev = d;
    TableStore<TABLE>::get().add(out);
    return ADF_OK;
}

static void lut_build_host(float s, float* host)
{
    auto span = [&](int a, int b) { for (int i = a; i < b; i++) host[i] = -expf(-sqrtf((float)i) / s); };
    int n = ADF_LUT_LEVELS;
    if (s > 0.0f) {
        const double lim = 110.0 * (double)s;
        if (lim * lim * 1.001 + 2.0 < (double)ADF_LUT_LEVELS) {
            int i0 = (int)(lim * lim * 1.001) + 2;
            while (i0 < ADF_LUT_LEVELS && !(-sqrtf((float)i0) / s <= -110.0f)) i0++;
            n = i0;
        }
    }
    for (int i = n; i < ADF_LUT_LEVELS; i++) host[i] = -0.0f;
    unsigned hw = std::thread::hardware_concurrency();
    int nt = (int)(hw >= 16 ? 8 : hw >= 4 ? hw / 2 : 1);
    if (n < 32768) nt = 1;
    if (nt <= 1) { span(0, n); return; }
    std::vector<std::thread> th;
    const int per = (n + nt - 1) / nt;
    bool ok = true;
    int done = std::min(per, n);
    for (int t = 1; t < nt && ok; t++) {
        const int a = t * per, b = std::min(n, a + per);
        if (a >= b) break;
        try { th.emplace_back(span, a, b); done = b; } catch (...) { ok = false; }
    }
    span(0, std::min(per, n));
    for (auto& t : th) t.join();
    if (done < n) span(done, n);
}

int adf::Lut::ensure(float s, hipStream_t st)
{
    for (auto& e : tables)
        if (e.t->key == s) { e.used = ++tick; cur = e.t->dev; return ADF_OK; }
    if ((int)tables.size() >= LUT_CACHE) {
        size_t lru = 0;
        for (size_t k = 1; k < tables.size(); k++) if (tables[k].used < tables[lru].used) lru = k;
        HIP_TRY(hipStreamSynchronize(st));
        tables.erase(tables.begin() + (ptrdiff_t)lru);
    }
    int device = 0;
    HIP_TRY(hipGetDevice(&device));
    std::shared_ptr<LutTable> t = LutStore::get().find([&](const LutTable& q) { return q.device == device && q.key == s; });
    if (!t) {
        std::vector<float> host(ADF_LUT_LEVELS);
        lut_build_host(s, host.data());
        float* d = nullptr;
        HIP_TRY(hipMalloc(&d, sizeof(float) * ADF_LUT_LEVELS));
        hipError_t e = hipMemcpy(d, host.data(), sizeof(float) * ADF_LUT_LEVELS, hipMemcpyHostToDevice);
        if (e != hipSuccess) { hipFree(d); return fail(ADF_EHIP, "LUT upload failed: %s", hipGetErrorString(e)); }
        t = std::make_shared<LutTable>();
        t->device = device; t->key = s; t->count = ADF_LUT_LEVELS; t->dev = d;
        LutStore::get().add(t);
    }
    tables.push_back(Entry{t, ++tick});
    cur = t->dev;
    return ADF_OK;
}

struct WmfKey {
    double sigma; int type;
    bool operator==(const WmfKey& o) const { return sigma == o.sigma && type == o.type; }
};
struct adf::WmfTable : DeviceTable<uint32_t, WmfKey> {};
using WmfStore = TableStore<WmfTable>;

static void wmf_build_host(double sigma, int weight_type, uint32_t* host)
{
    if (weight_type == ADF_WMF_OFF) { std::fill(host, host + ADF_WMF_TABLE_LEVELS, (uint32_t)ADF_WMF_WEIGHT_ONE); return; }
    int i = 0;
    for (; i < ADF_WMF_TABLE_LEVELS; i++) {
        const double e = exp(-(double)i / (2.0 * sigma * sigma)) * 65536.0;
        if (e < 0.25) break;
        host[i] = (uint32_t)lrint(e);
    }
    std::fill(host + i, host + ADF_WMF_TABLE_LEVELS, 0u);
}

int adf::wmf_weights_check(const char* who, double sigma, int weight_type)
{
    if (weight_type != ADF_WMF_EXP && weight_type != ADF_WMF_OFF)
        return fail(ADF_EBADARG, "%s: weight_type must be ADF_WMF_EXP (0) or ADF_WMF_OFF (5); WMF_IV1, WMF_IV2, WMF_COS and WMF_JAC are not built", who);
    if (!std::isfinite(sigma) || !(sigma > 0.0)) return fail(ADF_EBADARG, "%s: sigma must be finite and > 0", who);
    return ADF_OK;
}

int adf::wmf_table_device(double sigma, int weight_type, std::shared_ptr<WmfTable>& out, const uint32_t** dev)
{
    if (weight_type == ADF_WMF_OFF) sigma = 1.0;
    if (int rc = table_device("weighted median", WmfKey{sigma, weight_type}, [] { return (size_t)ADF_WMF_TABLE_LEVELS; },
                              [&](uint32_t* host) { wmf_build_host(sigma, weight_type, host); }, out))
        return rc;
    *dev = out->dev;
    return ADF_OK;
}

extern "C" int adf_wmf_weight_table_host(double sigma, int weight_type, uint32_t* table, int levels)
{
    if (!table || levels != ADF_WMF_TABLE_LEVELS) return fail(ADF_EBADARG, "adf_wmf_weight_table_host: table must hold %d entries", ADF_WMF_TABLE_LEVELS);
    if (int rc = wmf_weights_check("adf_wmf_weight_table_host", sigma, weight_type)) return rc;
    wmf_build_host(sigma, weight_type, table);
    return ADF_OK;
}

struct JbfKey {
    double sc, ss; int r, channels;
    bool operator==(const JbfKey& o) const { return sc == o.sc && ss == o.ss && r == o.r && channels == o.channels; }
};
struct adf::JbfTable : DeviceTable<float, JbfKey> {};
using JbfStore = TableStore<JbfTable>;

static void jbf_build_space(double ss, int r, float* space)
{
    const double cs = -0.5 / (ss * ss);
    space[0] = 1.0f;
    for (int q = 1; q < (int)jbf_space_entries(r); q++) space[q] = (float)exp((double)q * cs);
}

static void jbf_build_host(double sc, double ss, int r, int channels, float* colour, float* space)
{
    const double cc = -0.5 / (sc * sc);
    colour[0] = 1.0f;
    for (int a = 1; a < (int)jbf_colour_entries(channels); a++) colour[a] = (float)exp((double)(a * a) * cc);
    jbf_build_space(ss, r, space);
}

int adf::jbf_params_check(const char* who, int d, double sigma_color, double sigma_space, int joint_channels,
                          double* sc, double* ss, int* r)
{
    if (joint_channels != 1 && joint_channels != 3) return fail(ADF_EBADARG, "%s: joint must have 1 or 3 channels", who);
    if (!std::isfinite(sigma_color) || !std::isfinite(sigma_space) || !std::isfinite((float)sigma_color) || !std::isfinite((float)sigma_space))
        return fail(ADF_EBADARG, "%s: sigmaColor and sigmaSpace must be finite (as float32 too)", who);
    *sc = sigma_color <= 0 ? 1.0 : sigma_color;
    *ss = sigma_space <= 0 ? 1.0 : sigma_space;
    const double rr = std::max(1.0, d <= 0 ? std::nearbyint(*ss * 1.5) : (double)(d / 2));
    if (!(rr <= (double)ADF_JBF_MAX_RADIUS))
        return fail(ADF_EBADARG, "%s: the radius (d / 2, or cvRound(1.5 sigmaSpace) for d <= 0) must not exceed %d", who, ADF_JBF_MAX_RADIUS);
    *r = (int)rr;
    return ADF_OK;
// ... 80 lines not shown
{
    double sc, ss;
    int r;
    float k;
    if (int rc = rgf_params_check("adf_rgf_tables_host", depth, d, sigma_color, sigma_space, &sc, &ss, &r, &k)) return rc;
    if (radius) *radius = r;
    if (scale) *scale = k;
    if (colour_entries) *colour_entries = (int)rgf_colour_entries(depth, sc);
    if (!colour && !space) return ADF_OK;
    if (!colour || !space) return fail(ADF_EBADARG, "adf_rgf_tables_host: colour and space must both be given (or neither: the sizes alone)");
    rgf_build_colour(depth, sc, colour);
    jbf_build_space(ss, r, space);
    return ADF_OK;
}

struct BlockCache {
    struct Ent { int device; void* p; size_t bytes; hipEvent_t ready; };
    static constexpr size_t CAP_BYTES = (size_t)3 << 30;
    static constexpr size_t CAP_ENTRIES = 8;
    std::mutex m;
    std::vector<Ent> ents;
    size_t total = 0;
    static BlockCache& get() { static BlockCache* c = new BlockCache; return *c; }
    static void drop(const Ent& e)
    {
        DeviceScope ds(e.device);
        if (e.ready) { hipEventSynchronize(e.ready); hipEventDestroy(e.ready); }
        hipFree(e.p);
    }
    void* take(int device, size_t need, hipStream_t st, size_t* bytes)
    {
        Ent hit{};
        {
            std::lock_guard<std::mutex> lk(m);
            size_t best = ents.size();
            for (size_t k = 0; k < ents.size(); k++)
                if (ents[k].device == device && ents[k].bytes >= need && ents[k].bytes <= need + need / 4 + ((size_t)1 << 20) &&
                    (best == ents.size() || ents[k].bytes < ents[best].bytes))
                    best = k;
            if (best == ents.size()) return nullptr;
            hit = ents[best];
            ents.erase(ents.begin() + (ptrdiff_t)best);
            total -= hit.bytes;
        }
        if (hit.ready) {
            const hipError_t e = hipStreamWaitEvent(st, hit.ready, 0);
            if (e != hipSuccess) hipEventSynchronize(hit.ready);
            hipEventDestroy(hit.ready);
        }
        *bytes = hit.bytes;
        return hit.p;
    }
    void give(int device, void* p, size_t bytes, hipEvent_t ready)
    {
        std::vector<Ent> out;
        {
            std::lock_guard<std::mutex> lk(m);
            ents.push_back(Ent{device, p, bytes, ready});
            total += bytes;
            while (!ents.empty() && (total > CAP_BYTES || ents.size() > CAP_ENTRIES)) {
                out.push_back(ents.front());
                total -= ents.front().bytes;
                ents.erase(ents.begin());
            }
        }
        for (auto& e : out) drop(e);
    }
    void clear()
    {
        std::vector<Ent> out;
        { std::lock_guard<std::mutex> lk(m); out.swap(ents); total = 0; }
        for (auto& e : out) drop(e);
    }
};

extern "C" int adf_weight_table_host(float sigma_color, float* table, int levels)
{
    if (!table || levels != ADF_LUT_LEVELS) return fail(ADF_EBADARG, "table must hold %d floats", ADF_LUT_LEVELS);
    if (!(sigma_color >= 0.0f)) return fail(ADF_EBADARG, "sigma_color must be >= 0 (FGS.cpp:143)");
    lut_build_host(sigma_color, table);
    return ADF_OK;
}

namespace adf {
hipError_t device_malloc(void** p, size_t bytes)
{
    hipError_t e = hipMalloc(p, bytes);
    if (e == hipErrorOutOfMemory) {
        (void)hipGetLastError();
        BlockCache::get().clear();
        e = hipMalloc(p, bytes);
    }
    if (e != hipSuccess) *p = nullptr;
    return e;
}

void* cache_take(int device, size_t need, hipStream_t st, size_t* bytes) { return BlockCache::get().take(device, need, st, bytes); }

void cache_give(int device, void* p, size_t bytes, hipStream_t st)
{
    hipEvent_t ev = nullptr;
    if (hipEventCreateWithFlags(&ev, hipEventDisableTiming) != hipSuccess || hipEventRecord(ev, st) != hipSuccess) {
        (void)hipGetLastError();
        if (ev) hipEventDestroy(ev);
        ev = nullptr;
        hipStreamSynchronize(st);
    }
    BlockCache::get().give(device, p, bytes, ev);
}

void cache_give_event(int device, void* p, size_t bytes, hipEvent_t ready) { BlockCache::get().give(device, p, bytes, ready); }

int Scratch::take(size_t need, hipStream_t stream)
{
    if (hipGetDevice(&device) != hipSuccess) return fail(ADF_ENODEV, "no HIP device");
    st = stream;
    if ((p = cache_take(device, need, st, &bytes))) return ADF_OK;
    HIP_TRY(device_malloc(&p, need));
    bytes = need;
    return ADF_OK;
}

int workspace_or_scratch(const char* who, const char* size_fn, void* workspace, size_t workspace_bytes, size_t need,
                         hipStream_t st, Scratch& blk, void** ws)
{
    *ws = workspace;
    if (workspace) {
        if (workspace_bytes < need) return fail(ADF_ESIZE, "%s: workspace smaller than %s", who, size_fn);
        return (uintptr_t)workspace & 3 ? fail(ADF_EBADARG, "%s: workspace must be 4-byte aligned", who) : ADF_OK;
    }
    if (stream_is_capturing(st)) return fail(ADF_EBADARG, "%s: a call captured into a graph needs a caller workspace", who);
    const int rc = blk.take(need, st);
    *ws = blk.p;
    return rc;
}

int copy_images(void* dst, size_t dst_pitch, ptrdiff_t dst_image_stride, const void* src, size_t src_pitch,
                ptrdiff_t src_image_stride, size_t row_bytes, size_t rows, int n, hipMemcpyKind kind, hipStream_t st)
{
    for (int k = 0; k < n; k++)
        HIP_TRY(hipMemcpy2DAsync((char*)dst + k * dst_image_stride, dst_pitch, (const char*)src + k * src_image_stride, src_pitch,
                                 row_bytes, rows, kind, st));
    return ADF_OK;
}
}

extern "C" void adf_release_cached_memory(void)
{
    BlockCache::get().clear();
    LutStore::get().clear();
    WmfStore::get().clear();
    JbfStore::get().clear();
    RgfStore::get().clear();
}
```

addingdisparityfiltering_amd/csrc/adf_internal.h:

```cpp
#pragma once

#include <hip/hip_runtime.h>
#include <stddef.h>
#include <stdint.h>
#include "../../include/adf_wls.h"

#define ADF_LUT_LEVELS (3 * 256 * 256)
#define ADF_EPS 1e-43f

namespace adf {

struct Geom {
    int W, H;
    int rx, ry, rw, rh;
    int pw, ph;
    size_t plane;
    size_t frame;
    int cpitch, cx0;
    size_t cframe;
};

enum Orient { ORIENT_N = 0, ORIENT_T = 1, ORIENT_PAIR = 2, ORIENT_STRIP = 3 };
#define ADF_STRIP 16
constexpr int TILE_ROWS = 2;
// ... 4 lines not shown
    EPI_I16 = 2,
    EPI_F32 = 3,
    EPI_U8 = 4,
    EPI_WLS_CONF_F32 = 5
};
constexpr int N_EPILOGUES = EPI_WLS_CONF_F32 + 1;

struct DiscArgs {
    const int16_t* disp[2]; ptrdiff_t stride[2], pair_stride[2];
    int rx[2]; int ry, rw, rh;
    int radius; float roll_off;
    float* dst[2]; int W; size_t frame;
    int only_view;
};

struct ConfLeftArgs {
    const int16_t* dL; ptrdiff_t sL, psL;
    const int16_t* dR; ptrdiff_t sR, psR;
    const float* cR;
    float* conf;
    float* U0; float* U1;
    Geom g; int rrx; int thresh;
    int radius; float roll_off;
};

struct ConfBandArgs {
    const int16_t* dL; ptrdiff_t sL, psL;
    const int16_t* dR; ptrdiff_t sR, psR;
    float* conf;
    Geom g; int rrx; int thresh;
    int radius; float roll_off;
    int rows_per_band;
};

struct OutsideArgs {
    void* out; ptrdiff_t stride, pair_stride; int16_t fill; int out_f32;
    float* conf;
    Geom g;
};

struct LrcArgs {
    const int16_t* dL; ptrdiff_t sL, psL;
    const int16_t* dR; ptrdiff_t sR, psR;
    const float* cL; const float* cR;
    float* conf;
    void* out; ptrdiff_t sO, psO; int16_t fill; int out_f32;
    float* U0; float* U1;
    Geom g; int rrx;
    int thresh; int orient;
    int dl_f32 = 0;
};

struct PlainPrologueArgs {
    const void* src; ptrdiff_t stride, pair_stride;
    int depth, cn, c;
    float* U0; Geom g; int orient;
    const float* conf; float* U1;
    int pair2, c2;
};

constexpr int DEPTH_WLS_F32 = 0x100 | ADF_32F;

struct QuantArgs {
    const void* src[2]; ptrdiff_t stride[2], pair_stride[2];
    int16_t* q[2]; float* v;
    int W, H, pitch; size_t frame;
    int n_pairs;
};

struct ResizeArgs {
    const void* src; ptrdiff_t sstride, spair; int sw, sh;
    void* dst; ptrdiff_t dstride, dpair; int dw, dh;
    double scale_x, scale_y;
    float post_scale; int is16;
    int zero_outside = 0, vx0 = 0, vy0 = 0, vx1 = 0, vy1 = 0;
};

struct WeightArgs {
    const uint8_t* guide; ptrdiff_t stride, pair_stride; int ch;
    const float* lut;
    float* chor; float* cvert; int chor_orient, cvert_orient;
    Geom g;
    float* scratch;
};

struct PassArgs {
    const float* C; const float* U0; const float* U1;
    float* D; float* F0; float* F1;
    float* O0; float* O1;
    void* out; ptrdiff_t out_stride, out_pair_stride;
    int out_x0, out_y0, out_cn, out_c;
    int nscan, len, pitch_in, pitch_out;
    size_t plane;
    float lambda;
};

struct FusedInputs {
    const float* conf_in; size_t conf_frame; int conf_pitch, conf_x0, conf_y0;
    int dl_f32;
    const void* dl_in; ptrdiff_t dl_stride, dl_pair_stride; int dl_x0, dl_y0;
    const float* lo_conf; ptrdiff_t lo_conf_stride, lo_conf_pair;
    const int16_t* lo_dl; ptrdiff_t lo_dl_stride, lo_dl_pair;
    int lo_w, lo_h, hi_x0, hi_y0;
    double lo_scale_x, lo_scale_y; float lo_post_scale;
    int lo_zero_outside, lo_vx0, lo_vy0, lo_vx1, lo_vy1;
    int lo_half;
    float* lo_taps;
};

struct GuideWeights {
    const uint8_t* guide; ptrdiff_t stride, pair_stride;
    int ch, x0, y0;
    const float* lut;
};

struct WavePassArgs {
    const float* C; float* U0; float* U1;
    FusedInputs fuse;
    void* out; ptrdiff_t out_stride, out_pair_stride;
    int out_x0, out_y0, out_cn, out_c;
    int nscan, len, pitch;
    size_t plane;
    float lambda;
    GuideWeights gw;
    float* image; size_t image_plane; int image_m;
};
static_assert(sizeof(WavePassArgs) == 352 && offsetof(WavePassArgs, out) == 208 && offsetof(WavePassArgs, nscan) == 248 &&
              offsetof(WavePassArgs, plane) == 264 && offsetof(WavePassArgs, lambda) == 272 && offsetof(WavePassArgs, gw) == 280 &&
              offsetof(WavePassArgs, image) == 328 && sizeof(GuideWeights) == 48, "WavePassArgs layout");

hipError_t launch_discontinuity(const DiscArgs& a, int n_pairs, hipStream_t st);
hipError_t launch_lrc_prologue(const LrcArgs& a, int n_pairs, hipStream_t st);
hipError_t launch_conf_left(const ConfLeftArgs& a, int n_pairs, hipStream_t st);
hipError_t launch_outside(const OutsideArgs& a, int n_pairs, hipStream_t st);
bool conf_band_fits(const Geom& g, int radius);
hipError_t launch_conf_band(const ConfBandArgs& a, int n_pairs, hipStream_t st);
bool prep_small_guide_fits(const Geom& g, ptrdiff_t guide_stride, int channels);
bool prep_small_fits(const Geom& g, int radius, int channels, int n_pairs);
hipError_t launch_prep_small(const ConfBandArgs& c, const WeightArgs& w, const OutsideArgs& o, int n_pairs, hipStream_t st);
int conf_left_max_radius();
hipError_t launch_plain_prologue(const PlainPrologueArgs& a, int n_pairs, hipStream_t st);
hipError_t launch_quantise_maps(const QuantArgs& a, hipStream_t st);
hipError_t launch_weights(const WeightArgs& a, int n_pairs, hipStream_t st);
bool weights_stream_fits(const WeightArgs& a);
hipError_t launch_resize_linear(const ResizeArgs& a, int n_pairs, hipStream_t st);
hipError_t launch_exact_pass(const PassArgs& a, int n_rhs, int epilogue, int n_pairs, hipStream_t st);
hipError_t launch_wave_hpass(const WavePassArgs& a, int n_rhs, int n_pairs, hipStream_t st);
hipError_t launch_wave_vpass(const WavePassArgs& a, int n_rhs, int epilogue, int n_pairs, hipStream_t st);
int wave_max_row_len();
bool wave_hpass_can_fuse(const WavePassArgs& a);
bool wave_hpass_can_fuse_lo(const WavePassArgs& a);
bool wave_hpass_lo_half(const WavePassArgs& a);
bool wave_hpass_guide_fits(const WavePassArgs& a);
int wave_max_col_len();
bool wave_hpass_image_fits(int row_len);
bool wave_hpass_first_image(const FusedInputs& f);
int wave_vpass_image_m(int col_len);
inline size_t wave_image_floats(int pitch, int m) { return (size_t)pitch * (size_t)(64 * m) * 2; }
int max_disc_radius();

namespace tile {
constexpr int TX = 64;
constexpr int TY = 32;
constexpr int NT = 256;
}

#if defined(__HIPCC__)
__device__ __forceinline__ size_t pair_index(int i, int j, int pw)
{
    constexpr int TR = TILE_ROWS;
    return (size_t)(i / TR) * (size_t)(2 * TR * pw) + (size_t)((j >> 4) * (32 * TR) + (i % TR) * 32 + (j & 15));
}
__device__ __forceinline__ size_t strip_index(int i, int j, int rh)
{
    return ((size_t)(j >> 4) * (size_t)rh + (size_t)i) * ADF_STRIP + (size_t)(j & 15);
}
struct RhsPlanes { float* U0; float* U1; };
__device__ __forceinline__ RhsPlanes rhs_planes(float* U0, float* U1, int orient, size_t pz, size_t plane)
{
    const bool pair = orient == ORIENT_PAIR;
    float* u0 = U0 + pz * (pair ? 2 : 1) * plane;
    return RhsPlanes{u0, pair ? u0 + ADF_STRIP : U1 ? U1 + pz * plane : nullptr};
}
__device__ __forceinline__ size_t rhs_index(int orient, int i, int j, const Geom& g)
{
    return orient == ORIENT_PAIR ? pair_index(i, j, g.pw) : orient == ORIENT_T ? (size_t)j * g.ph + i : (size_t)i * g.pw + j;
}
struct RhsTile {
    float t0[tile::TX * (tile::TY + 1)], t1[tile::TX * (tile::TY + 1)];
    __device__ __forceinline__ void stage(int tx, int y, float v0, float v1) { t0[tx * (tile::TY + 1) + y] = v0; t1[tx * (tile::TY + 1) + y] = v1; }
    __device__ __forceinline__ void store(float* U0, float* U1, const Geom& g, int j0, int i0) const
    {
        __syncthreads();
#pragma unroll
        for (int m = 0; m < tile::TX / 8; m++) {
            const int cidx = threadIdx.x / tile::TY + 8 * m, ridx = threadIdx.x % tile::TY, j = j0 + cidx, i = i0 + ridx;
            if ((unsigned)j < (unsigned)g.rw && (unsigned)i < (unsigned)g.rh) {
                const size_t o = rhs_index(ORIENT_T, i, j, g);
                U0[o] = t0[cidx * (tile::TY + 1) + ridx];
                if (U1) U1[o] = t1[cidx * (tile::TY + 1) + ridx];
            }
        }
    }
};
__device__ __forceinline__ void store_fill(void* map, ptrdiff_t row_offset_bytes, int j, int16_t fill, int f32)
{
    char* row = reinterpret_cast<char*>(map) + row_offset_bytes;
    if (f32) reinterpret_cast<float*>(row)[j] = (float)fill;
    else reinterpret_cast<int16_t*>(row)[j] = fill;
}
__device__ __forceinline__ float wls_f32_value(float x) { return !(__builtin_fabsf(x) < 2147483648.0f) ? -32768.0f : x; }
__device__ __forceinline__ float wls_input_value(float d)
// ... 28 lines not shown
```

addingdisparityfiltering_amd/csrc/fgs_wave_v.hip:

```cpp
#include "fgs_wave_common.h"

namespace adf {

namespace {
using namespace wave;

constexpr int VT = 512;
constexpr int VC = 16;
typedef float v4f __attribute__((ext_vector_type(4)));

template <int EPI>
__device__ __forceinline__ v2f epi_value(v2f u0, v2f u1)
{
    if (EPI == EPI_WLS_CONF || EPI == EPI_WLS_CONF_F32) {
        const v2f sc = vsplat(0x1p64f);
        return u0 * (vrcp_nr(vfma(u1, sc, vsplat(ADF_EPS * 0x1p64f))) * sc);
    }
    return u0;
}

template <int EPI>
__device__ __forceinline__ unsigned epi_pack16(v2f u0, v2f u1)
{
    const v2f x = epi_value<EPI>(u0, u1);
    const bool o0 = !(__builtin_fabsf(x.x) < 2147483648.0f), o1 = !(__builtin_fabsf(x.y) < 2147483648.0f);
    const int i0 = (int)(o0 ? -32768.0f : __builtin_rintf(x.x)), i1 = (int)(o1 ? -32768.0f : __builtin_rintf(x.y));
    typedef short s2 __attribute__((ext_vector_type(2)));
    return __builtin_bit_cast(unsigned, (s2)__builtin_amdgcn_cvt_pk_i16(i0, i1));
}

template <int EPI>
__device__ __forceinline__ v2f epi_f32(v2f u0, v2f u1)
{
    const v2f x = epi_value<EPI>(u0, u1);
    if (EPI == EPI_WLS_CONF_F32) return (v2f){wls_f32_value(x.x), wls_f32_value(x.y)};
    return x;
}

template <int EPI, bool F32>
__device__ __forceinline__ auto epi_out(v2f u0, v2f u1)
{
    if constexpr (F32) return epi_f32<EPI>(u0, u1);
    else return epi_pack16<EPI>(u0, u1);
}
__device__ __forceinline__ void put_first(char* dst, unsigned v) { reinterpret_cast<uint16_t*>(dst)[0] = (uint16_t)v; }
__device__ __forceinline__ void put_first(char* dst, v2f v) { reinterpret_cast<float*>(dst)[0] = v.x; }
__device__ __forceinline__ void put_second(char* dst, unsigned v) { reinterpret_cast<uint16_t*>(dst)[1] = (uint16_t)(v >> 16); }
__device__ __forceinline__ void put_second(char* dst, v2f v) { reinterpret_cast<float*>(dst)[1] = v.y; }
__device__ __forceinline__ void put_both(char* dst, unsigned v) { *reinterpret_cast<unsigned*>(dst) = v; }
__device__ __forceinline__ void put_both(char* dst, v2f v) { *reinterpret_cast<v2f*>(dst) = v; }

__device__ __forceinline__ bool out_pairs_aligned(const WavePassArgs& a, unsigned esz)
{
    const unsigned m = 2u * esz - 1u;
    return ((reinterpret_cast<uintptr_t>(a.out) | (uintptr_t)a.out_stride | (uintptr_t)a.out_pair_stride) & m) == 0 &&
           (((unsigned)a.out_x0 * esz) & m) == 0;
}

template <int EPI, bool F32, bool LAST_ODD, int M>
__device__ __forceinline__ void store_rows(const v2f (&f0)[M], const v2f (&f1)[M], char* dst, ptrdiff_t stride, bool aligned, int hv2, int hv1)
{
#pragma unroll
    for (int i = 0; i < M; i++) {
        const auto v = epi_out<EPI, F32>(f0[i], f1[i]);
        if (i < hv2) {
            if (aligned) put_both(dst, v);
            else { put_first(dst, v); put_second(dst, v); }
        }
        if constexpr (LAST_ODD) {
            if (i < hv1) put_first(dst, v);
        }
        dst += stride;
        ADF_STEP_FENCE();
    }
}

template <int R>
__device__ __forceinline__ unsigned vstep(int r0, int i, int pitch)
{
    constexpr unsigned TR = TILE_ROWS;
    if (R > 1) return ((((unsigned)r0 + (unsigned)i + 1u) & (TR - 1u)) == 0u) ? 2u * TR * (unsigned)pitch * 4u - (TR - 1u) * 128u : 128u;
    return (unsigned)pitch * 4u;
}

template <int M, int R, int EPI, int VCW = VC, int NCH = 64, bool IMG = false>
__global__ void __launch_bounds__(VT) wave_vpass_kernel(WavePassArgs a)
{
    static_assert((VCW == 16 && NCH == 64) || (VCW == 8 && NCH == 128), "whole strips of 64 chunks or half strips of 128");
    static_assert(!IMG || (R == 2 && VCW == VC && (EPI == EPI_PLANES || EPI == EPI_WLS_CONF || EPI == EPI_WLS_CONF_F32)), "the image: whole strips, both right-hand sides, the plain pass or the filter's epilogues");
    static_assert((VCW / 2) * NCH == VT, "one thread per (chunk, column pair)");
    constexpr int XPN = VCW / 2;
    __shared__ float nb[4][NCH][VCW];
    __shared__ float red[5][VCW][NCH];
    __shared__ float xs[2][VCW][NCH];
    const int tid = threadIdx.x;
    const int xp = tid & (XPN - 1), cidx = tid / XPN;
    int strip = VCW == VC ? (int)blockIdx.x : (int)(blockIdx.x >> 1);
    if (VCW == VC) {
        const int nfull = (int)(gridDim.x / 32) * 32;
        if ((EPI != EPI_PLANES || R == 1) && (int)blockIdx.x < nfull) {
            const int grp = blockIdx.x >> 5, w = blockIdx.x & 31;
            strip = (grp << 5) + ((w & 7) << 2) + (w >> 3);
        }
    }
    const unsigned c16 = 2u * (unsigned)xp + (VCW == VC ? 0u : 8u * (blockIdx.x & 1u));
    const int col = strip * VC + (int)c16;
    const size_t pb = (size_t)blockIdx.y * a.plane;
    const int r0 = cidx * M;
    const int h = a.len;

    const char* bC = reinterpret_cast<const char*>(a.C + pb);
    char* b0 = reinterpret_cast<char*>(a.U0 + (R > 1 ? 2 * pb : pb));
    char* b1 = (R > 1) ? b0 + 4 * VC : nullptr;
    constexpr unsigned TR = TILE_ROWS;
    const unsigned voff0 = (R > 1) ? (((unsigned)r0 / TR) * (2u * TR * (unsigned)a.pitch) + (unsigned)strip * (32u * TR) + ((unsigned)r0 % TR) * 32u + c16) * 4u
                                   : ((unsigned)r0 * (unsigned)a.pitch + (unsigned)col) * 4u;
    const unsigned pitch_c = 4u * VC;
    const unsigned coff0 = (((unsigned)strip * (unsigned)h + (unsigned)r0) * VC + c16) * 4u;

    v2f c[M], f0[M], f1[M];
    const unsigned safe = (R > 1) ? ((unsigned)strip * (32u * TR) + c16) * 4u : (unsigned)col * 4u;
    const unsigned csafe = ((unsigned)strip * (unsigned)h * VC + c16) * 4u;
    v2f a_s = vsplat(0.0f);
    if (cidx > 0 && r0 - 1 < h) a_s = *reinterpret_cast<const v2f*>(bC + (coff0 - pitch_c)) * vsplat(a.lambda);
    {
        unsigned voff = voff0, coff = coff0;
        const v2f lam = vsplat(a.lambda);
        const char* bI = IMG ? reinterpret_cast<const char*>(a.image + (size_t)blockIdx.y * a.image_plane) : nullptr;
        unsigned ioff = (((unsigned)strip * (NCH / 8) + ((unsigned)tid >> 6)) * (unsigned)M) * 1024u + ((unsigned)tid & 63u) * 16u;
#pragma unroll
        for (int i = 0; i < M; i++) {
            const bool ok = r0 + i < h;
            c[i] = *reinterpret_cast<const v2f*>(bC + (ok ? coff : csafe));
            if constexpr (IMG) {
                const v4f q = *reinterpret_cast<const v4f*>(bI + ioff);
                f0[i] = (v2f){q.x, q.y}; f1[i] = (v2f){q.z, q.w};
                ioff += 1024u;
            } else {
                const unsigned vo = ok ? voff : safe;
                f0[i] = *reinterpret_cast<const v2f*>(b0 + vo);
                f1[i] = (R > 1) ? *reinterpret_cast<const v2f*>(b1 + vo) : vsplat(0.0f);
                voff += vstep<R>(r0, i, a.pitch);
            }
            coff += pitch_c;
            ADF_STEP_FENCE();
        }
#pragma unroll
        for (int i = 0; i < M; i++) c[i] *= lam;
    }

    Boundary<v2f, R> bd;
    chunk_boundary<M, R>(c, f0, f1, a_s, bd);
    *reinterpret_cast<v2f*>(&nb[0][cidx][2 * xp]) = bd.GS0;
    *reinterpret_cast<v2f*>(&nb[1][cidx][2 * xp]) = bd.GS1;
    *reinterpret_cast<v2f*>(&nb[2][cidx][2 * xp]) = bd.PS;
    *reinterpret_cast<v2f*>(&nb[3][cidx][2 * xp]) = bd.QS;
    __syncthreads();
    {
        v2f nGS0 = vsplat(0.f), nGS1 = nGS0, nPS = nGS0, nQS = nGS0;
        if (cidx < NCH - 1) {
            nGS0 = *reinterpret_cast<const v2f*>(&nb[0][cidx + 1][2 * xp]); nGS1 = *reinterpret_cast<const v2f*>(&nb[1][cidx + 1][2 * xp]);
            nPS = *reinterpret_cast<const v2f*>(&nb[2][cidx + 1][2 * xp]); nQS = *reinterpret_cast<const v2f*>(&nb[3][cidx + 1][2 * xp]);
        }
        v2f al, be, ga, p0, p1;
        separator_row<M, R>(c, f0, f1, bd, nGS0, nGS1, nPS, nQS, al, be, ga, p0, p1);
        red[0][2 * xp][cidx] = al.x; red[1][2 * xp][cidx] = be.x; red[2][2 * xp][cidx] = ga.x;
        red[3][2 * xp][cidx] = p0.x; red[4][2 * xp][cidx] = p1.x;
        red[0][2 * xp + 1][cidx] = al.y; red[1][2 * xp + 1][cidx] = be.y; red[2][2 * xp + 1][cidx] = ga.y;
        red[3][2 * xp + 1][cidx] = p0.y; red[4][2 * xp + 1][cidx] = p1.y;
    }
    __syncthreads();
    if constexpr (NCH == 64) {
        const int wv = tid >> 6, lane = tid & 63;
#pragma unroll
        for (int e = 0; e < 2; e++) {
            const int cc = 2 * wv + e;
            float x0, x1;
            pcr64<R>(lane, red[0][cc][lane], red[1][cc][lane], red[2][cc][lane], red[3][cc][lane], red[4][cc][lane], x0, x1);
            xs[0][cc][lane] = x0; xs[1][cc][lane] = x1;
        }
    } else {
        const int cc = tid >> 6, lane = tid & 63;
        reduced128<R>(lane, red[0][cc], red[1][cc], red[2][cc], red[3][cc], red[4][cc], 1, xs[0][cc], xs[1][cc]);
    }
    __syncthreads();
    {
        const int cc = 2 * xp;
        const v2f xR0 = {xs[0][cc][cidx], xs[0][cc + 1][cidx]}, xR1 = {xs[1][cc][cidx], xs[1][cc + 1][cidx]};
        v2f xL0 = vsplat(0.0f), xL1 = xL0;
        if (cidx > 0) {
            xL0 = (v2f){xs[0][cc][cidx - 1], xs[0][cc + 1][cidx - 1]};
            xL1 = (v2f){xs[1][cc][cidx - 1], xs[1][cc + 1][cidx - 1]};
        }
        chunk_solve<M, R>(c, f0, f1, a_s, xL0, xL1, xR0, xR1);
    }

    unsigned voff = voff0;
    asm volatile("" : "+v"(voff));
    if (EPI == EPI_PLANES) {
#pragma unroll
        for (int i = 0; i < M; i++) {
            if (r0 + i < h) {
                *reinterpret_cast<v2f*>(b0 + voff) = f0[i];
                if (R > 1) *reinterpret_cast<v2f*>(b1 + voff) = f1[i];
            }
            voff += vstep<R>(r0, i, a.pitch);
        }
    } else {
        int r0e = r0, cole = col;
        asm volatile("" : "+v"(r0e), "+v"(cole));
        char* ob = reinterpret_cast<char*>(a.out) + (ptrdiff_t)blockIdx.y * a.out_pair_stride +
                   (ptrdiff_t)(a.out_y0 + r0e) * a.out_stride;
        const int esz = (EPI == EPI_F32 || EPI == EPI_WLS_CONF_F32) ? 4 : (EPI == EPI_U8) ? 1 : 2;
        unsigned ooff = (unsigned)((a.out_x0 + cole) * a.out_cn + a.out_c) * (unsigned)esz;
        const bool fast16 = (EPI == EPI_WLS_CONF || EPI == EPI_I16) && a.out_cn == 1;
        const bool fast32 = (EPI == EPI_WLS_CONF_F32 || (EPI == EPI_F32 && R == 1)) && a.out_cn == 1;
        if (fast16 || fast32) {
            const int hv2 = (cole + 1 < a.nscan ? h : 0) - r0e;
            const int hv1 = (cole + 1 == a.nscan ? h : 0) - r0e;
            char* dst = ob + ooff;
            if (fast16 && (a.nscan & 1)) store_rows<EPI, false, true>(f0, f1, dst, a.out_stride, out_pairs_aligned(a, 2), hv2, hv1);
            else if (fast16) {
                const int hv = (cole < a.nscan ? h : 0) - r0e;
                if (out_pairs_aligned(a, 2)) store_rows<EPI, false, false>(f0, f1, dst, a.out_stride, true, hv, 0);
                else store_rows<EPI, false, false>(f0, f1, dst, a.out_stride, false, hv, 0);
            } else if (out_pairs_aligned(a, 4)) store_rows<EPI, true, true>(f0, f1, dst, a.out_stride, true, hv2, hv1);
            else store_rows<EPI, true, true>(f0, f1, dst, a.out_stride, false, hv2, hv1);
        } else if (EPI != EPI_WLS_CONF_F32) {
#pragma unroll
        for (int i = 0; i < M; i++) {
            if (r0 + i < h) {
#pragma unroll
                for (int e = 0; e < 2; e++) {
                    if (col + e < a.nscan) {
                        char* dst = ob + ooff + (unsigned)(e * a.out_cn * esz);
                        if (EPI == EPI_WLS_CONF) {
                            const float rcp = 1.0f / (f1[i][e] + ADF_EPS);
                            *reinterpret_cast<int16_t*>(dst) = sat16(f0[i][e] * rcp);
                        } else {
#pragma unroll
                            for (int r = 0; r < R; r++) {
                                const float x = r ? f1[i][e] : f0[i][e];
                                char* d = dst + r * esz;
                                if (EPI == EPI_I16) *reinterpret_cast<int16_t*>(d) = sat16(x);
                                else if (EPI == EPI_U8) *reinterpret_cast<uint8_t*>(d) = sat8(x);
                                else *reinterpret_cast<float*>(d) = x;
                            }
                        }
                    }
                }
            }
            ooff += (unsigned)a.out_stride;
        }
        }
    }
}

template <int M, int VCW = VC, int NCH = 64>
hipError_t launch_v(const WavePassArgs& a, int n_rhs, int epi, int n_pairs, hipStream_t st)
{
    dim3 grid(a.pitch / VCW, n_pairs), block(VT);
    constexpr int N_EPI = N_EPILOGUES;
    if (n_rhs < 1 || n_rhs > 2 || epi < 0 || epi >= N_EPI) return hipErrorInvalidValue;
    return dispatch_index<2 * N_EPI>((n_rhs - 1) * N_EPI + epi, [&](auto K) {
        constexpr int R = decltype(K)::value / N_EPI + 1, EPI = decltype(K)::value % N_EPI;
        if constexpr (R == 1 && (EPI == EPI_WLS_CONF || EPI == EPI_WLS_CONF_F32)) return hipErrorInvalidValue;
        else {
            if (a.image) {
                if constexpr (R == 2 && VCW == VC && (EPI == EPI_PLANES || EPI == EPI_WLS_CONF || EPI == EPI_WLS_CONF_F32)) {
                    if (a.image_m != M || a.image_plane < wave_image_floats(a.pitch, M)) return hipErrorInvalidValue;
                    hipLaunchKernelGGL((wave_vpass_kernel<M, R, EPI, VCW, NCH, true>), grid, block, 0, st, a);
                    return hipGetLastError();
                } else return hipErrorInvalidValue;
            }
            hipLaunchKernelGGL((wave_vpass_kernel<M, R, EPI, VCW, NCH>), grid, block, 0, st, a);
            return hipGetLastError();
        }
    });
}

constexpr Bucket COL_BUCKETS[] = {{2, 64}, {4, 64}, {8, 64}, {12, 64}, {18, 64}, {26, 64}, {34, 64}, {20, 128}, {26, 128}, {34, 128}};
constexpr int N_COL_BUCKETS = sizeof(COL_BUCKETS) / sizeof(COL_BUCKETS[0]);

}

int wave_max_col_len() { return COL_BUCKETS[N_COL_BUCKETS - 1].m * COL_BUCKETS[N_COL_BUCKETS - 1].chunks; }

int wave_vpass_image_m(int col_len)
{
    if (col_len < 2 || col_len > wave_max_col_len()) return 0;
    const Bucket& b = COL_BUCKETS[bucket_index(COL_BUCKETS, col_len)];
    return b.chunks == 64 ? b.m : 0;
}

hipError_t launch_wave_vpass(const WavePassArgs& a, int n_rhs, int epilogue, int n_pairs, hipStream_t st)
{
    if (a.len < 2 || a.len > wave_max_col_len() || a.pitch % 64 != 0 || a.pitch < a.nscan) return hipErrorInvalidValue;
    if (epilogue == EPI_WLS_CONF_F32 && a.out_cn != 1) return hipErrorInvalidValue;
    return dispatch_index<N_COL_BUCKETS>(bucket_index(COL_BUCKETS, a.len), [&](auto I) {
        constexpr Bucket b = COL_BUCKETS[decltype(I)::value];
        return launch_v<b.m, b.chunks == 64 ? VC : VC / 2, b.chunks>(a, n_rhs, epilogue, n_pairs, st);
    });
}

}
```

addingdisparityfiltering_amd/csrc/prep_bodies.h:

```cpp
#pragma once
#include "adf_internal.h"

namespace adf {
namespace prep {

#define ADF_PREP_ST(p, v) __builtin_nontemporal_store((v), (p))

constexpr int WS_U = 4;
constexpr int WS_NT = 128;
constexpr int WS_COLS = 4;
constexpr int WS_BCOLS = WS_NT * WS_COLS;
constexpr int WS_LUT_HEAD = 2048;

template <int CH>
struct WsShared {
    float lut_head[WS_LUT_HEAD];
};

typedef unsigned ws_v4u __attribute__((ext_vector_type(4)));
typedef unsigned ws_v2u __attribute__((ext_vector_type(2)));
typedef float ws_v4f __attribute__((ext_vector_type(4)));

template <int CH> struct WsWin;
template <> struct WsWin<3> { ws_v4u a; unsigned b; };
// ... 64 lines not shown
        const unsigned e = __builtin_amdgcn_alignbyte(w.a.y, w.a.x, m);
        const unsigned nb = __builtin_amdgcn_alignbyte(0u, w.a.y, m) & 0xffu;
#pragma unroll
        for (int k = 0; k < WS_COLS; k++) {
            const int v = (int)((e >> (8 * k)) & 0xffu);
            const int r = k < WS_COLS - 1 ? (int)((e >> (8 * k + 8)) & 0xffu) : (int)nb;
            const int u = (int)((pv.q[0] >> (8 * k)) & 0xffu);
            hidx[k] = HOR ? ws_dist2_c1(v, r) : 0;
            vidx[k] = ws_dist2_c1(u, v);
        }
        pv.q[0] = e;
    }
}

__device__ __forceinline__ __amdgpu_buffer_rsrc_t ws_window(const void* p, size_t bytes)
{
    const uintptr_t b = reinterpret_cast<uintptr_t>(p);
    const unsigned lo = (unsigned)__builtin_amdgcn_readfirstlane((int)(unsigned)(b & 0xffffffffu));
    const unsigned hi = (unsigned)__builtin_amdgcn_readfirstlane((int)(unsigned)(b >> 32));
    const unsigned n = (unsigned)__builtin_amdgcn_readfirstlane((int)(unsigned)bytes);
    return __builtin_amdgcn_make_buffer_rsrc(reinterpret_cast<void*>((uintptr_t)lo | ((uintptr_t)hi << 32)), (short)0, (int)n, 0x00020000);
}
constexpr unsigned WS_DROP = 0x80000000u;

struct WsPending { float wl[2 * WS_COLS]; unsigned g[2 * WS_COLS]; };
template <bool HOR>
__device__ __forceinline__ void ws_lookup_issue(const float* lut_head, const __amdgpu_buffer_rsrc_t& lutwin, const int (&hidx)[WS_COLS],
                                                const int (&vidx)[WS_COLS], WsPending& p)
{
#pragma unroll
    for (int k = 0; k < WS_COLS; k++) {
        p.wl[k] = HOR ? lut_head[min(hidx[k], WS_LUT_HEAD - 1)] : 0.0f;
        p.wl[WS_COLS + k] = lut_head[min(vidx[k], WS_LUT_HEAD - 1)];
    }
#pragma unroll
    for (int k = 0; k < WS_COLS; k++) {
        p.g[k] = HOR ? __builtin_amdgcn_raw_buffer_load_b32(lutwin, hidx[k] >= WS_LUT_HEAD ? (unsigned)hidx[k] * 4u : WS_DROP, 0, 0) : 0u;
        p.g[WS_COLS + k] = __builtin_amdgcn_raw_buffer_load_b32(lutwin, vidx[k] >= WS_LUT_HEAD ? (unsigned)vidx[k] * 4u : WS_DROP, 0, 0);
    }
}
template <bool HOR>
__device__ __forceinline__ void ws_lookup_finish(const WsPending& p, float (&wh)[WS_COLS], float (&wv)[WS_COLS])
{
#pragma unroll
    for (int k = 0; k < WS_COLS; k++) {
        wh[k] = !HOR ? 0.0f : p.g[k] != 0u ? __uint_as_float(p.g[k]) : p.wl[k];
        wv[k] = p.g[WS_COLS + k] != 0u ? __uint_as_float(p.g[WS_COLS + k]) : p.wl[WS_COLS + k];
    }
}

struct WsOut {
    __amdgpu_buffer_rsrc_t chor, cvert; unsigned mh[WS_COLS], mv[WS_COLS]; unsigned ho, vo, hstep, vstep; bool st_ok, strip;
    __device__ __forceinline__ void init(const WeightArgs& a, size_t pz, int j0, int y_first)
    {
        const Geom& g = a.g;
        chor = ws_window(a.chor ? a.chor + pz * g.plane : a.chor, a.chor ? g.plane * sizeof(float) : 0);
        cvert = ws_window(a.cvert + pz * g.plane, g.plane * sizeof(float));
        strip = a.cvert_orient == ORIENT_STRIP;
#pragma unroll
        for (int k = 0; k < WS_COLS; k++) { mh[k] = (j0 + k < g.rw - 1) ? 0xffffffffu : 0u; mv[k] = (j0 + k < g.rw) ? 0xffffffffu : 0u; }
        st_ok = j0 >= 0 && j0 < g.pw;
        ho = ((unsigned)y_first * (unsigned)g.pw + (unsigned)j0) * 4u;
        vo = (strip ? ((unsigned)(j0 >> 4) * (unsigned)g.rh + (unsigned)y_first) * ADF_STRIP + (unsigned)(j0 & 15)
                    : (unsigned)y_first * (unsigned)g.pw + (unsigned)j0) * 4u;
        hstep = (unsigned)g.pw * 4u; vstep = (strip ? (unsigned)ADF_STRIP : (unsigned)g.pw) * 4u;
    }
    __device__ __forceinline__ void store_h(int t, const float (&wh)[WS_COLS], bool on) const
    {
        ws_v4u o;
#pragma unroll
        for (int k = 0; k < WS_COLS; k++) o[k] = __float_as_uint(wh[k]) & mh[k];
        __builtin_amdgcn_raw_buffer_store_b128(o, chor, (on && st_ok) ? ho + (unsigned)t * hstep : WS_DROP, 0, 2 );
    }
    __device__ __forceinline__ void store_v(int t, const float (&wv)[WS_COLS], bool last_row, bool on) const
    {
        const unsigned last = last_row ? 0u : 0xffffffffu;
        ws_v4u o;
#pragma unroll
        for (int k = 0; k < WS_COLS; k++) o[k] = __float_as_uint(wv[k]) & mv[k] & last;
        const unsigned off = (on && st_ok) ? vo + (unsigned)t * vstep : WS_DROP;
        if (strip) __builtin_amdgcn_raw_buffer_store_b128(o, cvert, off, 0, 0);
        else __builtin_amdgcn_raw_buffer_store_b128(o, cvert, off, 0, 2);
    }
};

template <int CH, bool HOR = true>
__device__ __forceinline__ void weights_stream_body(const WeightArgs& a, int bx, int by, int nby, size_t pz, WsShared<CH>& sh, bool active)
{
    static_assert(CH == 1 || CH == 3, "guides have one or three channels");
    float (&lut_head)[WS_LUT_HEAD] = sh.lut_head;
    const Geom& g = a.g;
    const int tid = active ? (int)threadIdx.x : 0;
    if (active)
        for (int q = tid; q < WS_LUT_HEAD; q += WS_NT) lut_head[q] = a.lut[q];
    __syncthreads();
    const int ws_rows = (g.rh + nby - 1) / nby;
    const int x0 = bx * WS_BCOLS, y0 = by * ws_rows;
    if (!active || y0 >= g.rh) return;
    constexpr int WS_PRIO = 3;
    __builtin_amdgcn_s_setprio(WS_PRIO);
    const int nrows = min(ws_rows, g.rh - y0) + 1;
    const int j0 = x0 + WS_COLS * tid;

    const int r_first = g.ry + y0, r_last = g.ry + min(y0 + nrows - 1, g.rh - 1);
    const WsGuide gd = ws_guide(reinterpret_cast<uintptr_t>(a.guide) + (uintptr_t)((ptrdiff_t)pz * a.pair_stride + (ptrdiff_t)r_first * a.stride),
                                a.stride, r_last - r_first + 1, g.W * CH);
    const unsigned col_off = gd.mis + (unsigned)((g.rx + x0) * CH);
    const unsigned lane_off = (unsigned)(tid * WS_COLS * CH);
    auto row_off = [&](int n) -> unsigned { return col_off + (unsigned)(min(y0 + n, g.rh - 1) - y0) * gd.stride; };
    auto load = [&](int n) -> WsWin<CH> { return ws_load<CH, HOR>(gd, (row_off(n) & ~3u) + lane_off); };

    WsOut out;
    out.init(a, pz, j0, y0);
    const __amdgpu_buffer_rsrc_t lutwin = ws_window(a.lut, sizeof(float) * ADF_LUT_LEVELS);
    WsPrev<CH> pv;
#pragma unroll
    for (int k = 0; k < WS_COLS; k++) { pv.q[k] = 0; pv.qa[k] = 0; }
    WsWin<CH> nxt[WS_U], cur[WS_U];
#pragma unroll
    for (int s = 0; s < WS_U; s++) nxt[s] = load(s < nrows ? s : nrows - 1);
    WsPending pend;
    {
        int hidx[WS_COLS], vidx[WS_COLS];
        ws_indices<CH, HOR>(nxt[0], row_off(0) & 3u, pv, hidx, vidx);
        ws_lookup_issue<HOR>(lut_head, lutwin, hidx, vidx, pend);
    }
    for (int n0 = 0; n0 < nrows; n0 += WS_U) {
#pragma unroll
        for (int s = 0; s < WS_U; s++) {
            cur[s] = nxt[s];
            if constexpr (CH == 3) asm volatile("" : "+v"(cur[s].a), "+v"(cur[s].b)); else asm volatile("" : "+v"(cur[s].a));
        }
#pragma unroll
        for (int s = 0; s < WS_U; s++) nxt[s] = load(min(n0 + WS_U + s, nrows - 1));
#pragma unroll
        for (int s = 0; s < WS_U; s++) {
            const int n = n0 + s;
            WsPending ahead;
            {
                int hidx[WS_COLS], vidx[WS_COLS];
                ws_indices<CH, HOR>(s + 1 < WS_U ? cur[s + 1 < WS_U ? s + 1 : 0] : nxt[0], row_off(min(n + 1, nrows - 1)) & 3u, pv, hidx, vidx);
                ws_lookup_issue<HOR>(lut_head, lutwin, hidx, vidx, ahead);
            }
            float wh[WS_COLS], wv[WS_COLS];
            ws_lookup_finish<HOR>(pend, wh, wv);
            if constexpr (HOR) out.store_h(n, wh, n < nrows - 1);
            out.store_v(n - 1, wv, y0 + n - 1 == g.rh - 1, n >= 1 && n < nrows);
            pend = ahead;
        }
    }
}


}
}
```

addingdisparityfiltering_amd/csrc/weights_kernels.hip:

```cpp
#include "adf_internal.h"
#include "prep_bodies.h"
#include <cstdlib>

namespace adf {

namespace {

#define ADF_ST(p, v) __builtin_nontemporal_store((v), (p))
constexpr int TX = 64, TY = 32, NT = 256;
constexpr int LUT_HEAD = 2048;

template <int CH>
__global__ void __launch_bounds__(NT) weights_kernel(WeightArgs a)
{
    constexpr int RB = (TX + 1) * CH;
    constexpr int RW = (RB + 3) / 4 + 1;
    __shared__ unsigned gw[(TY + 1) * RW];
    __shared__ int mis[TY + 1];
    __shared__ float th[TX * (TY + 1)];
    __shared__ float lut_head[LUT_HEAD];
    const Geom& g = a.g;
    const int tid = threadIdx.x, tx = tid % TX, ty = tid / TX;
    const int x0 = blockIdx.x * TX, y0 = blockIdx.y * TY;
    const size_t pz = blockIdx.z;
    const unsigned char* gp = a.guide + (ptrdiff_t)pz * a.pair_stride;
    const int last_px = min(x0 + TX, g.rw - 1);
    const int need = (last_px - x0 + 1) * CH;

    for (int rr = ty; rr < TY + 1; rr += NT / TX) {
        const int gi = min(y0 + rr, g.rh - 1);
        const unsigned char* rowp = gp + (ptrdiff_t)(g.ry + gi) * a.stride + (ptrdiff_t)(g.rx + x0) * CH;
        const int m = (int)(reinterpret_cast<uintptr_t>(rowp) & 3u);
        const unsigned* wp = reinterpret_cast<const unsigned*>(rowp - m);
        const int nw = (m + need + 3) >> 2;
        for (int w = tx; w < nw; w += TX) gw[rr * RW + w] = wp[w];
        if (tx == 0) mis[rr] = m;
    }
    for (int q = tid; q < LUT_HEAD; q += NT) lut_head[q] = a.lut[q];
    __syncthreads();

    const unsigned char* gb = reinterpret_cast<const unsigned char*>(gw);
    float* chor = a.chor + pz * g.plane;
    float* cvert = a.cvert + pz * g.plane;
    int hidx[TY / 4], vidx[TY / 4];
#pragma unroll
    for (int kk = 0; kk < TY / 4; kk++) {
        const int r = ty + 4 * kk;
        const unsigned char* p = gb + r * (RW * 4) + mis[r] + tx * CH;
        const unsigned char* pd = gb + (r + 1) * (RW * 4) + mis[r + 1] + tx * CH;
        int hi = 0, vi = 0;
#pragma unroll
        for (int c = 0; c < CH; c++) {
            const int v = p[c];
            const int dh = v - (int)p[CH + c];
            const int dv = v - (int)pd[c];
            hi += dh * dh; vi += dv * dv;
        }
        hidx[kk] = hi; vidx[kk] = vi;
    }
    float wh[TY / 4], wv[TY / 4];
    bool big = false;
#pragma unroll
    for (int kk = 0; kk < TY / 4; kk++) {
        wh[kk] = lut_head[min(hidx[kk], LUT_HEAD - 1)];
        wv[kk] = lut_head[min(vidx[kk], LUT_HEAD - 1)];
        big = big || hidx[kk] >= LUT_HEAD || vidx[kk] >= LUT_HEAD;
    }
    if (big) {
#pragma unroll
        for (int kk = 0; kk < TY / 4; kk++) {
            if (hidx[kk] >= LUT_HEAD) wh[kk] = a.lut[hidx[kk]];
            if (vidx[kk] >= LUT_HEAD) wv[kk] = a.lut[vidx[kk]];
        }
    }
    const int j = x0 + tx;
#pragma unroll
    for (int kk = 0; kk < TY / 4; kk++) {
        const int r = ty + 4 * kk;
        const int i = y0 + r;
        const bool ok = i < g.rh && j < g.rw;
        const float h = (j == g.rw - 1) ? 0.0f : wh[kk];
        const float v = (i == g.rh - 1) ? 0.0f : wv[kk];
        if (a.chor_orient == ORIENT_N) { if (ok) chor[(size_t)i * g.pw + j] = h; }
        else th[tx * (TY + 1) + r] = ok ? h : 0.0f;
        if (ok) cvert[a.cvert_orient == ORIENT_STRIP ? strip_index(i, j, g.rh) : (size_t)i * g.pw + j] = v;
    }
    if (a.chor_orient == ORIENT_T) {
        __syncthreads();
#pragma unroll
        for (int m = 0; m < TX / 8; m++) {
            const int cidx = tid / TY + 8 * m, ridx = tid % TY;
            const int jj = x0 + cidx, ii = y0 + ridx;
            if (jj < g.rw && ii < g.rh) chor[(size_t)jj * g.ph + ii] = th[cidx * (TY + 1) + ridx];
        }
    }
}

template <int CH, bool HOR>
__global__ void __launch_bounds__(prep::WS_NT) weights_stream_kernel(WeightArgs a)
{
    __shared__ prep::WsShared<CH> sh;
    prep::weights_stream_body<CH, HOR>(a, blockIdx.x, blockIdx.y, gridDim.y, blockIdx.z, sh, true);
}

__global__ void __launch_bounds__(256) transpose_n_to_t_kernel(const float* __restrict__ src, float* __restrict__ dst, Geom g)
{
    __shared__ float tile[64][65];
    const int tid = threadIdx.x;
    const int j0 = blockIdx.x * 64, i0 = blockIdx.y * 64;
    const size_t pb = (size_t)blockIdx.z * g.plane;
    const int c4 = tid & 15, r = tid >> 4;
#pragma unroll
    for (int m = 0; m < 4; m++) {
        const int row = r + 16 * m;
        float4 v = make_float4(0.f, 0.f, 0.f, 0.f);
        if (i0 + row < g.rh) v = *reinterpret_cast<const float4*>(src + pb + (size_t)(i0 + row) * g.pw + j0 + 4 * c4);
        tile[row][4 * c4 + 0] = v.x; tile[row][4 * c4 + 1] = v.y; tile[row][4 * c4 + 2] = v.z; tile[row][4 * c4 + 3] = v.w;
    }
    __syncthreads();
#pragma unroll
    for (int m = 0; m < 4; m++) {
        const int col = r + 16 * m;
        if (j0 + col < g.rw) {
            const float4 v = make_float4(tile[4 * c4 + 0][col], tile[4 * c4 + 1][col], tile[4 * c4 + 2][col], tile[4 * c4 + 3][col]);
            *reinterpret_cast<float4*>(dst + pb + (size_t)(j0 + col) * g.ph + i0 + 4 * c4) = v;
        }
    }
}

}

bool weights_stream_fits(const WeightArgs& a)
{
    static const bool force_generic = [] { const char* e = getenv("ADF_WEIGHTS_GENERIC"); return e && atoi(e) != 0; }();
    return !force_generic && a.chor_orient == ORIENT_N && a.stride > 0 && a.stride < ((ptrdiff_t)1 << 29) && (size_t)a.g.W * a.ch < ((size_t)1 << 29);
}

hipError_t launch_weights(const WeightArgs& a, int n_pairs, hipStream_t st)
{
    const bool hor = a.chor != nullptr;
    if (a.chor_orient == ORIENT_T && a.cvert_orient == ORIENT_N && a.scratch) {
        WeightArgs b = a;
        b.chor = a.scratch; b.chor_orient = ORIENT_N; b.scratch = nullptr;
        hipError_t e = launch_weights(b, n_pairs, st);
        if (e != hipSuccess) return e;
        dim3 grid(a.g.pw / 64, a.g.ph / 64, n_pairs);
        hipLaunchKernelGGL(transpose_n_to_t_kernel, grid, dim3(256), 0, st, a.scratch, a.chor, a.g);
        return hipGetLastError();
    }
    if (a.cvert_orient != ORIENT_N && !(a.cvert_orient == ORIENT_STRIP && a.chor_orient == ORIENT_N)) return hipErrorInvalidValue;
    if (weights_stream_fits(a)) {
        dim3 sgrid((a.g.rw + prep::WS_BCOLS - 1) / prep::WS_BCOLS, 1, n_pairs);
        {
            int rpb = 128;
            while (rpb > 16 && ((a.g.rh + rpb - 1) / rpb) * (int)(sgrid.x * sgrid.z) < 2048) rpb >>= 1;
            while (rpb > 4 && ((a.g.rh + rpb - 1) / rpb) * (int)(sgrid.x * sgrid.z) < 512) rpb >>= 1;
            while (rpb > 1 && (size_t)(rpb + 1) * (size_t)a.stride >= ((size_t)1 << 30)) rpb >>= 1;
            sgrid.y = (a.g.rh + rpb - 1) / rpb;
        }
        if (a.ch == 1 && hor) hipLaunchKernelGGL((weights_stream_kernel<1, true>), sgrid, dim3(prep::WS_NT), 0, st, a);
        else if (a.ch == 1) hipLaunchKernelGGL((weights_stream_kernel<1, false>), sgrid, dim3(prep::WS_NT), 0, st, a);
        else if (a.ch == 3 && hor) hipLaunchKernelGGL((weights_stream_kernel<3, true>), sgrid, dim3(prep::WS_NT), 0, st, a);
        else if (a.ch == 3) hipLaunchKernelGGL((weights_stream_kernel<3, false>), sgrid, dim3(prep::WS_NT), 0, st, a);
        else return hipErrorInvalidValue;
        return hipGetLastError();
    }
    if (!hor) return hipErrorInvalidValue;
    dim3 grid((a.g.rw + TX - 1) / TX, (a.g.rh + TY - 1) / TY, n_pairs);
    if (a.ch == 1) hipLaunchKernelGGL(weights_kernel<1>, grid, dim3(NT), 0, st, a);
    else if (a.ch == 3) hipLaunchKernelGGL(weights_kernel<3>, grid, dim3(NT), 0, st, a);
    else return hipErrorInvalidValue;
    return hipGetLastError();
}

}
```

addingdisparityfiltering_amd/ximgproc.py:

```python
import ctypes as C
import functools
import math

import numpy as np

from . import _lib
from ._lib import SGBM_COST_BT, SGBM_COST_CENSUS_DENSE, SGBM_COST_CENSUS_SPARSE
from ._lib import BM_COST_SAD, BM_COST_CENSUS_DENSE, BM_COST_CENSUS_SPARSE
from ._lib import SGBM_COST_MCT_DENSE, SGBM_COST_MCT_SPARSE, SGBM_COST_CENSUS_CS
from ._lib import BM_COST_MCT_DENSE, BM_COST_MCT_SPARSE, BM_COST_CENSUS_CS
from ._lib import SGBM_RIGHT_MATCHER, SGBM_RIGHT_FROM_VOLUME
from ._lib import WMF_EXP, WMF_IV1, WMF_IV2, WMF_COS, WMF_JAC, WMF_OFF
from ._lib import GF_MAX_RADIUS
from ._lib import DTF_NC, DTF_IC, DTF_RF, DT_MAX_ITERS, DT_NC_MAX_RADIUS
from ._lib import RGF_MAX_ITERS, AM_MAX_TREE_HEIGHT
from ._lib import JBF_MAX_RADIUS, BORDER_REPLICATE, BORDER_REFLECT, BORDER_WRAP, BORDER_REFLECT_101
from ._lib import AdfError, HANDOFF_IMAGE, HANDOFF_IMAGE_PAIR_TAIL, HANDOFF_PAIR_PLANE, PATH_CONF_BAND, PATH_FUSED_FIRST_PASS, PATH_MERGED_PREP, PATH_ROW_WEIGHTS_GUIDE, PATH_SCALED_FUSED, PATH_SCALED_HALF, Rect, SOLVER_EXACT, SOLVER_WAVE

try:
    import torch
except Exception:
    torch = None


def _is_torch(a):
    return torch is not None and isinstance(a, torch.Tensor)


def _as_rect(roi):
    if roi is None:
        return None
    if isinstance(roi, Rect):
        return roi
    x, y, w, h = roi
    return Rect(int(x), int(y), int(w), int(h))


_ITEMSIZE = {np.int16: 2, np.uint8: 1, np.float32: 4, np.uint64: 8, np.int32: 4}
_TORCH_DTYPE = {np.int16: torch.int16, np.uint8: torch.uint8, np.float32: torch.float32, np.uint64: torch.int64, np.int32: torch.int32} if torch is not None else {}
_raw_stream = getattr(getattr(torch, "_C", None), "_cuda_getCurrentRawStream", None) if torch is not None else None


class _Image:

    def __init__(self, arr, dtype_np, what, batched, allow_channels=(1,)):
        self.keep = arr
        if _is_torch(arr):
            if not arr.is_cuda:
                arr = arr.cpu().numpy()
            else:
                if arr.dtype != _TORCH_DTYPE[dtype_np]:
                    raise AdfError(_lib.ADF_EBADARG, "%s must have dtype %s" % (what, _TORCH_DTYPE[dtype_np]))
                self.device = True
                isz = _ITEMSIZE[dtype_np]
                self.ptr = arr.data_ptr()
                self._finish(arr.shape, [q * isz for q in arr.stride()], isz, what, batched, allow_channels)
                return
        a = np.asarray(arr)
        if a.dtype != np.dtype(dtype_np):
            raise AdfError(_lib.ADF_EBADARG, "%s must have dtype %s (got %s)" % (what, np.dtype(dtype_np), a.dtype))
        self.device = False
        self.keep = a
        self.ptr = a.ctypes.data
        self._finish(a.shape, a.strides, a.itemsize, what, batched, allow_channels)

    def _finish(self, shape, strides, itemsize, what, batched, allow_channels):
        nd = len(shape)
        k = 1 if batched else 0
        if nd - k == 2:
            self.c, sc, sx = 1, itemsize, strides[k + 1]
        elif nd - k == 3:
            self.c, sc, sx = shape[k + 2], strides[k + 2], strides[k + 1]
        else:
            raise AdfError(_lib.ADF_EBADARG, "%s has an unsupported shape %s" % (what, tuple(shape)))
        self.n, self.pair_stride = (shape[0], strides[0]) if batched else (1, 0)
        self.h, self.w, self.stride = shape[k], shape[k + 1], strides[k]
        if self.n < 1 or self.h < 1 or self.w < 1:
            raise AdfError(_lib.ADF_EBADARG, "%s is empty" % what)
        if self.c not in allow_channels:
            raise AdfError(_lib.ADF_EBADARG, "%s must have %s channel(s)" % (what, " or ".join(map(str, allow_channels))))
        if sc != itemsize or sx != itemsize * self.c:
            raise AdfError(_lib.ADF_ESIZE, "%s rows must be dense (channel-interleaved, unit pixel stride)" % what)


def _empty(img, shape, dtype_np):
    if img.device:
        return torch.empty(shape, dtype=_TORCH_DTYPE[dtype_np], device=img.keep.device)
    return np.empty(shape, dtype_np)


def _out_like(img, batched, dtype_np):
    return _empty(img, (img.n, img.h, img.w) if batched else (img.h, img.w), dtype_np)


def _stream_of(img):
    if img.device:
        dev = img.keep.device
        if _raw_stream is not None and dev.index is not None:
            return _raw_stream(dev.index)
        return torch.cuda.current_stream(dev).cuda_stream
# ... 37 lines not shown
    for im in imgs:
        if im is not None and im.device and im.keep.device.index != dev:
            raise AdfError(_lib.ADF_EBADARG, "%s lives on cuda:%d; tensors on cuda:%s cannot be passed to it "
                                             "(create one handle per GPU)" % (what, dev, im.keep.device.index))


def _map_dtype(m, exactly=None):
    dt = getattr(m, "dtype", None)
    want = np.float32 if exactly is None else exactly
    if _is_torch(m):
        has = dt is _TORCH_DTYPE[want]
    else:
        has = dt is not None and np.dtype(dt) == np.dtype(want)
    return want if has else (np.int16 if exactly is None else None)


class DisparityFilter:

    def filter(self, disparity_map_left, left_view, filtered_disparity_map=None,
               disparity_map_right=None, ROI=None, right_view=None):
        raise NotImplementedError


class DisparityWLSFilter(_Handle, DisparityFilter):
    _destroy = "adf_wls_destroy"

    def __init__(self, use_confidence, left_offset=0, right_offset=0, top_offset=0, bottom_offset=0,
                 min_disp=0):
        self._h = C.c_void_p()
        _lib.check(_lib.lib().adf_wls_create(C.byref(self._h), int(bool(use_confidence)), left_offset,
                                             right_offset, top_offset, bottom_offset, min_disp))
        self._use_confidence = bool(use_confidence)
        self._last = None
        self._dev = _read(_lib.lib().adf_wls_get_device, C.c_int, self._h)

    def getLambda(self):
        return _read(_lib.lib().adf_wls_get_lambda, C.c_double, self._h)

    def setLambda(self, _lambda):
        _lib.check(_lib.lib().adf_wls_set_lambda(self._h, float(_lambda)))

    def getSigmaColor(self):
        return _read(_lib.lib().adf_wls_get_sigma_color, C.c_double, self._h)

    def setSigmaColor(self, _sigma_color):
        _lib.check(_lib.lib().adf_wls_set_sigma_color(self._h, float(_sigma_color)))

    def getLRCthresh(self):
        return _read(_lib.lib().adf_wls_get_lrc_thresh, C.c_int, self._h)

    def setLRCthresh(self, _LRC_thresh):
        _lib.check(_lib.lib().adf_wls_set_lrc_thresh(self._h, int(_LRC_thresh)))

    def getDepthDiscontinuityRadius(self):
        return _read(_lib.lib().adf_wls_get_depth_discontinuity_radius, C.c_int, self._h)

    def setDepthDiscontinuityRadius(self, _disc_radius):
        _lib.check(_lib.lib().adf_wls_set_depth_discontinuity_radius(self._h, int(_disc_radius)))

    def setFGSParams(self, lambda_attenuation=0.25, num_iter=3):
        _lib.check(_lib.lib().adf_wls_set_fgs_params(self._h, float(lambda_attenuation), int(num_iter)))

    def setSolver(self, solver):
        _lib.check(_lib.lib().adf_wls_set_solver(self._h, int(solver)))

    def getSolver(self):
        return _read(_lib.lib().adf_wls_get_solver, C.c_int, self._h)

    def getLastSolver(self):
        return _read(_lib.lib().adf_wls_get_last_solver, C.c_int, self._h)

    def getLastPath(self):
        return _read(_lib.lib().adf_wls_get_last_path, C.c_int, self._h)

    def getLastSolverPath(self):
        return _read(_lib.lib().adf_wls_get_last_solver_path, C.c_int, self._h)

    def getLastHandoff(self):
        return _read(_lib.lib().adf_wls_get_last_handoff, C.c_int, self._h)

    def getInnerHandoffs(self):
        full, tail = C.c_int(0), C.c_int(0)
        _lib.check(_lib.lib().adf_wls_get_inner_handoffs(self._h, C.byref(full), C.byref(tail)))
        return full.value, tail.value

    def enableProfiling(self, on=True):
        _lib.check(_lib.lib().adf_wls_profile_enable(self._h, int(bool(on))))

    def readProfile(self):
        buf = (_lib.KernelTime * 16)()
        n = C.c_int()
        _lib.check(_lib.lib().adf_wls_profile_read(self._h, buf, 16, C.byref(n)))
        return {buf[k].name.decode(): dict(launches=buf[k].launches, total_ms=buf[k].total_ms,
                                           alg_bytes=buf[k].alg_bytes, moved_bytes=buf[k].moved_bytes)
                for k in range(n.value)}

    def workspaceBytes(self):
        return int(_lib.lib().adf_wls_workspace_bytes(self._h))

    def filter(self, disparity_map_left, left_view, filtered_disparity_map=None,
               disparity_map_right=None, ROI=None, right_view=None):
        return self._filter("adf_wls_filter_scaled", np.int16, disparity_map_left, left_view, filtered_disparity_map,
                            disparity_map_right, ROI)

    def filterFloat(self, disparity_map_left, left_view, filtered_disparity_map=None,
                    disparity_map_right=None, ROI=None):
        return self._filter("adf_wls_filter_scaled_f32", np.float32, disparity_map_left, left_view, filtered_disparity_map,
                            disparity_map_right, ROI)

    def _filter(self, entry, out_dtype, disparity_map_left, left_view, filtered_disparity_map, disparity_map_right, ROI):
        if disparity_map_left is None:
            raise AdfError(_lib.ADF_EBADARG, "disparity_map_left is empty")
        if left_view is None:
            raise AdfError(_lib.ADF_EBADARG, "left_view is empty")
        batched = len(disparity_map_left.shape) == 3
        mdt = _map_dtype(disparity_map_left)
        if mdt is np.float32 and disparity_map_right is not None and _map_dtype(disparity_map_right, np.int16) is np.int16:
            mdt = np.int16
        dl = _Image(disparity_map_left, mdt, "disparity_map_left", batched)
        gv = _Image(left_view, np.uint8, "left_view", batched, allow_channels=(1, 3))
        if gv.n != dl.n:
            raise AdfError(_lib.ADF_ESIZE, "batch sizes of disparity maps and views differ")
        dr = None
        if disparity_map_right is not None and getattr(disparity_map_right, "size", 1) != 0:
            dr = _Image(disparity_map_right, mdt, "disparity_map_right", batched)
            if (dr.n, dr.h, dr.w) != (dl.n, dl.h, dl.w):
                raise AdfError(_lib.ADF_ESIZE, "left and right disparity maps differ in size")
        elif self._use_confidence:
            raise AdfError(_lib.ADF_EBADARG, "disparity_map_right is required with use_confidence")
        if gv.device != dl.device or (dr is not None and dr.device != dl.device):
            raise AdfError(_lib.ADF_EBADARG, "inputs must all be numpy arrays or all be CUDA tensors")
        if filtered_disparity_map is None:
            filtered_disparity_map = _out_like(gv, batched, out_dtype)
        out = _Image(filtered_disparity_map, out_dtype, "filtered_disparity_map", batched)
        if (out.n, out.h, out.w) != (gv.n, gv.h, gv.w) or out.device != dl.device:
            raise AdfError(_lib.ADF_ESIZE, "filtered_disparity_map has the wrong size or placement")
        if dl.device:
            _check_device(self._dev, (dl, gv, dr, out), "this DisparityWLSFilter")
        roi = _as_rect(ROI)
        args = (self._h, dl.n,
                dl.ptr, dl.stride, dl.pair_stride, dl.w, dl.h,
                gv.ptr, gv.stride, gv.pair_stride, gv.c, gv.w, gv.h,
                out.ptr, out.stride, out.pair_stride,
                dr.ptr if dr else None, dr.stride if dr else 0, dr.pair_stride if dr else 0,
                C.byref(roi) if roi is not None else None)
        if mdt is np.float32:
            entry = "adf_wls_filter_typed"
            args = args[:5] + (_lib.DEPTH_32F,) + args[5:16] + (_DEPTH[out_dtype],) + args[16:]
        if dl.device:
            _lib.check(getattr(_lib.lib(), entry + "_device")(*args, _stream_of(dl)))
        else:
            _lib.check(getattr(_lib.lib(), entry + "_host")(*args))
        self._last = (batched, dl.device, gv)
        return filtered_disparity_map

    def getConfidenceMap(self, pair=None):
        if self._last is None or not self._use_confidence:
            return np.zeros((0, 0), np.float32)
        batched, device, ex = self._last
        pairs = range(ex.n) if pair is None else [pair]
        outs = []
        for k in pairs:
            o = _empty(ex, (ex.h, ex.w), np.float32)
            _call("adf_wls_get_confidence", ex, (self._h, k, o.data_ptr() if device else o.ctypes.data, ex.w * 4))
            outs.append(o)
        if pair is not None or not batched:
# ... 1266 lines not shown
```

include/adf_wls.h:

```cpp
#ifndef ADF_WLS_H
#define ADF_WLS_H

#include <stddef.h>
#include <stdint.h>

#ifdef __cplusplus
extern "C" {
#endif

#define ADF_VERSION 100

enum adf_status {
    ADF_OK = 0,
    ADF_EBADARG = 1,
    ADF_ESIZE = 2,
    ADF_EHIP = 3,
    ADF_ENOMEM = 4,
    ADF_ENODEV = 5
};

enum adf_solver { ADF_SOLVER_EXACT = 0, ADF_SOLVER_WAVE = 1 };

enum adf_depth { ADF_8U = 0, ADF_16S = 3, ADF_32S = 4, ADF_32F = 5 };

typedef struct adf_wls adf_wls_t;
typedef struct adf_fgs adf_fgs_t;

typedef struct adf_rect { int x, y, width, height; } adf_rect;

int adf_version(void);
const char* adf_last_error(void);
int adf_device_count(void);
int adf_device_pci_bus_id(int device, char* buf, int len);


int adf_wls_create(adf_wls_t** out, int use_confidence, int left_offset, int right_offset,
                   int top_offset, int bottom_offset, int min_disp);
void adf_wls_destroy(adf_wls_t* h);

int adf_wls_set_lambda(adf_wls_t* h, double lambda);
int adf_wls_get_lambda(const adf_wls_t* h, double* lambda);
int adf_wls_set_sigma_color(adf_wls_t* h, double sigma_color);
int adf_wls_get_sigma_color(const adf_wls_t* h, double* sigma_color);
int adf_wls_set_lrc_thresh(adf_wls_t* h, int lrc_thresh);
int adf_wls_get_lrc_thresh(const adf_wls_t* h, int* lrc_thresh);
int adf_wls_set_depth_discontinuity_radius(adf_wls_t* h, int radius);
int adf_wls_get_depth_discontinuity_radius(const adf_wls_t* h, int* radius);

int adf_wls_set_fgs_params(adf_wls_t* h, double lambda_attenuation, int num_iter);
int adf_wls_set_solver(adf_wls_t* h, int solver);
int adf_wls_get_solver(const adf_wls_t* h, int* solver);
int adf_wls_get_last_solver(const adf_wls_t* h, int* solver);
#define ADF_PATH_CONF_BAND 1
#define ADF_PATH_FUSED_FIRST_PASS 2
#define ADF_PATH_MERGED_PREP 4
#define ADF_PATH_SCALED_FUSED 8
#define ADF_PATH_SCALED_HALF 16
int adf_wls_get_last_path(const adf_wls_t* h, int* path_flags);
#define ADF_PATH_ROW_WEIGHTS_GUIDE 32
int adf_wls_get_last_solver_path(const adf_wls_t* h, int* path_flags);
#define ADF_HANDOFF_PAIR_PLANE 0
#define ADF_HANDOFF_IMAGE 1
#define ADF_HANDOFF_IMAGE_PAIR_TAIL 2
int adf_wls_get_last_handoff(const adf_wls_t* h, int* form);
int adf_wls_get_inner_handoffs(const adf_wls_t* h, int* full, int* tail);

int adf_wls_filter_device(adf_wls_t* h, int n_pairs,
                          const int16_t* disp_left, ptrdiff_t disp_left_stride, ptrdiff_t disp_left_pair_stride,
                          const uint8_t* left_view, ptrdiff_t view_stride, ptrdiff_t view_pair_stride,
                          int view_channels, int W, int H,
                          int16_t* out, ptrdiff_t out_stride, ptrdiff_t out_pair_stride,
                          const int16_t* disp_right, ptrdiff_t disp_right_stride, ptrdiff_t disp_right_pair_stride,
                          const adf_rect* roi, void* stream);

int adf_wls_filter_host(adf_wls_t* h, int n_pairs,
                        const int16_t* disp_left, ptrdiff_t disp_left_stride, ptrdiff_t disp_left_pair_stride,
                        const uint8_t* left_view, ptrdiff_t view_stride, ptrdiff_t view_pair_stride,
                        int view_channels, int W, int H,
                        int16_t* out, ptrdiff_t out_stride, ptrdiff_t out_pair_stride,
                        const int16_t* disp_right, ptrdiff_t disp_right_stride, ptrdiff_t disp_right_pair_stride,
                        const adf_rect* roi);

int adf_wls_filter_scaled_device(adf_wls_t* h, int n_pairs,
                                 const int16_t* disp_left, ptrdiff_t disp_left_stride, ptrdiff_t disp_left_pair_stride,
                                 int disp_W, int disp_H,
                                 const uint8_t* left_view, ptrdiff_t view_stride, ptrdiff_t view_pair_stride,
                                 int view_channels, int W, int H,
                                 int16_t* out, ptrdiff_t out_stride, ptrdiff_t out_pair_stride,
                                 const int16_t* disp_right, ptrdiff_t disp_right_stride, ptrdiff_t disp_right_pair_stride,
                                 const adf_rect* roi, void* stream);
int adf_wls_filter_scaled_host(adf_wls_t* h, int n_pairs,
                               const int16_t* disp_left, ptrdiff_t disp_left_stride, ptrdiff_t disp_left_pair_stride,
                               int disp_W, int disp_H,
                               const uint8_t* left_view, ptrdiff_t view_stride, ptrdiff_t view_pair_stride,
                               int view_channels, int W, int H,
                               int16_t* out, ptrdiff_t out_stride, ptrdiff_t out_pair_stride,
                               const int16_t* disp_right, ptrdiff_t disp_right_stride, ptrdiff_t disp_right_pair_stride,
                               const adf_rect* roi);

int adf_wls_filter_f32_device(adf_wls_t* h, int n_pairs,
                              const int16_t* disp_left, ptrdiff_t disp_left_stride, ptrdiff_t disp_left_pair_stride,
                              const uint8_t* left_view, ptrdiff_t view_stride, ptrdiff_t view_pair_stride,
                              int view_channels, int W, int H,
                              float* out, ptrdiff_t out_stride, ptrdiff_t out_pair_stride,
                              const int16_t* disp_right, ptrdiff_t disp_right_stride, ptrdiff_t disp_right_pair_stride,
                              const adf_rect* roi, void* stream);
int adf_wls_filter_f32_host(adf_wls_t* h, int n_pairs,
                            const int16_t* disp_left, ptrdiff_t disp_left_stride, ptrdiff_t disp_left_pair_stride,
                            const uint8_t* left_view, ptrdiff_t view_stride, ptrdiff_t view_pair_stride,
                            int view_channels, int W, int H,
                            float* out, ptrdiff_t out_stride, ptrdiff_t out_pair_stride,
                            const int16_t* disp_right, ptrdiff_t disp_right_stride, ptrdiff_t disp_right_pair_stride,
                            const adf_rect* roi);
int adf_wls_filter_scaled_f32_device(adf_wls_t* h, int n_pairs,
                                     const int16_t* disp_left, ptrdiff_t disp_left_stride, ptrdiff_t disp_left_pair_stride,
                                     int disp_W, int disp_H,
                                     const uint8_t* left_view, ptrdiff_t view_stride, ptrdiff_t view_pair_stride,
                                     int view_channels, int W, int H,
                                     float* out, ptrdiff_t out_stride, ptrdiff_t out_pair_stride,
                                     const int16_t* disp_right, ptrdiff_t disp_right_stride, ptrdiff_t disp_right_pair_stride,
                                     const adf_rect* roi, void* stream);
int adf_wls_filter_scaled_f32_host(adf_wls_t* h, int n_pairs,
                                   const int16_t* disp_left, ptrdiff_t disp_left_stride, ptrdiff_t disp_left_pair_stride,
                                   int disp_W, int disp_H,
                                   const uint8_t* left_view, ptrdiff_t view_stride, ptrdiff_t view_pair_stride,
                                   int view_channels, int W, int H,
                                   float* out, ptrdiff_t out_stride, ptrdiff_t out_pair_stride,
                                   const int16_t* disp_right, ptrdiff_t disp_right_stride, ptrdiff_t disp_right_pair_stride,
                                   const adf_rect* roi);

int adf_wls_filter_typed_device(adf_wls_t* h, int n_pairs,
                                const void* disp_left, ptrdiff_t disp_left_stride, ptrdiff_t disp_left_pair_stride, int disp_depth,
                                int disp_W, int disp_H,
                                const uint8_t* left_view, ptrdiff_t view_stride, ptrdiff_t view_pair_stride,
                                int view_channels, int W, int H,
                                void* out, ptrdiff_t out_stride, ptrdiff_t out_pair_stride, int out_depth,
                                const void* disp_right, ptrdiff_t disp_right_stride, ptrdiff_t disp_right_pair_stride,
                                const adf_rect* roi, void* stream);
int adf_wls_filter_typed_host(adf_wls_t* h, int n_pairs,
                              const void* disp_left, ptrdiff_t disp_left_stride, ptrdiff_t disp_left_pair_stride, int disp_depth,
                              int disp_W, int disp_H,
                              const uint8_t* left_view, ptrdiff_t view_stride, ptrdiff_t view_pair_stride,
                              int view_channels, int W, int H,
                              void* out, ptrdiff_t out_stride, ptrdiff_t out_pair_stride, int out_depth,
                              const void* disp_right, ptrdiff_t disp_right_stride, ptrdiff_t disp_right_pair_stride,
                              const adf_rect* roi);

int adf_wls_get_confidence_device(adf_wls_t* h, int pair, float* dst, ptrdiff_t dst_stride, void* stream);
int adf_wls_get_confidence_host(adf_wls_t* h, int pair, float* dst, ptrdiff_t dst_stride);
int adf_wls_get_device(const adf_wls_t* h, int* device);
int adf_wls_get_roi(const adf_wls_t* h, adf_rect* roi);
int adf_wls_sync(adf_wls_t* h, void* stream);
size_t adf_wls_workspace_bytes(const adf_wls_t* h);

typedef struct adf_kernel_time {
    char name[48];
    int launches;
    double total_ms;
    double alg_bytes;
    double moved_bytes;
} adf_kernel_time;
int adf_wls_profile_enable(adf_wls_t* h, int on);
int adf_wls_profile_read(adf_wls_t* h, adf_kernel_time* out, int capacity, int* count);


int adf_fgs_create(adf_fgs_t** out, const uint8_t* guide, ptrdiff_t guide_stride, int guide_channels,
                   int w, int h, double lambda, double sigma_color, double lambda_attenuation,
                   int num_iter, int solver);
int adf_fgs_create_device(adf_fgs_t** out, const uint8_t* guide, ptrdiff_t guide_stride, int guide_channels,
                          int w, int h, double lambda, double sigma_color, double lambda_attenuation,
                          int num_iter, int solver, void* stream);
void adf_fgs_destroy(adf_fgs_t* h);
void adf_release_cached_memory(void);
#define ADF_WEIGHT_TABLE_LEVELS (3 * 256 * 256)
int adf_weight_table_host(float sigma_color, float* table, int levels);
int adf_fgs_get_device(const adf_fgs_t* h, int* device);
int adf_fgs_get_solver(const adf_fgs_t* h, int* solver);

int adf_fgs_filter_host(adf_fgs_t* h, const void* src, ptrdiff_t src_stride, void* dst,
                        ptrdiff_t dst_stride, int depth, int channels);
int adf_fgs_filter_device(adf_fgs_t* h, const void* src, ptrdiff_t src_stride, void* dst,
                          ptrdiff_t dst_stride, int depth, int channels, void* stream);


#define ADF_UNKNOWN_DISPARITY 16320

int adf_compute_mse_host(const int16_t* gt, ptrdiff_t gt_stride, const int16_t* src, ptrdiff_t src_stride,
                         int W, int H, const adf_rect* roi, double* mse);
int adf_compute_mse_device(const int16_t* gt, ptrdiff_t gt_stride, const int16_t* src, ptrdiff_t src_stride,
                           int W, int H, const adf_rect* roi, double* mse, void* stream);
int adf_compute_bad_pixel_percent_host(const int16_t* gt, ptrdiff_t gt_stride, const int16_t* src, ptrdiff_t src_stride,
                                       int W, int H, const adf_rect* roi, int thresh, double* percent);
int adf_compute_bad_pixel_percent_device(const int16_t* gt, ptrdiff_t gt_stride, const int16_t* src, ptrdiff_t src_stride,
                                         int W, int H, const adf_rect* roi, int thresh, double* percent, void* stream);
int adf_get_disparity_vis_host(const int16_t* src, ptrdiff_t src_stride, uint8_t* dst, ptrdiff_t dst_stride,
                               int W, int H, double scale);
int adf_get_disparity_vis_device(const int16_t* src, ptrdiff_t src_stride, uint8_t* dst, ptrdiff_t dst_stride,
                                 int W, int H, double scale, void* stream);

typedef struct adf_bm adf_bm_t;
int adf_bm_create(adf_bm_t** out, int num_disparities, int block_size);
void adf_bm_destroy(adf_bm_t* h);
int adf_bm_set_params(adf_bm_t* h, int min_disparity, int num_disparities, int block_size,
                      int prefilter_cap, int texture_threshold, int uniqueness_ratio);
int adf_bm_get_device(const adf_bm_t* h, int* device);
int adf_bm_get_params(const adf_bm_t* h, int* min_disparity, int* num_disparities, int* block_size,
                      int* prefilter_cap, int* texture_threshold, int* uniqueness_ratio);
#define ADF_BM_COST_SAD 0
#define ADF_BM_COST_CENSUS_DENSE 1
#define ADF_BM_COST_CENSUS_SPARSE 2
#define ADF_BM_COST_MCT_DENSE 4
#define ADF_BM_COST_MCT_SPARSE 5
#define ADF_BM_COST_CENSUS_CS 6
int adf_bm_set_cost(adf_bm_t* h, int cost_type, int census_size);
int adf_bm_get_cost(const adf_bm_t* h, int* cost_type, int* census_size);
int adf_bm_compute_device(adf_bm_t* h, int n_pairs,
                          const uint8_t* left, ptrdiff_t left_stride, ptrdiff_t left_pair_stride,
                          const uint8_t* right, ptrdiff_t right_stride, ptrdiff_t right_pair_stride,
                          int W, int H,
                          int16_t* disparity, ptrdiff_t disp_stride, ptrdiff_t disp_pair_stride,
                          void* stream);
int adf_bm_compute_both_device(adf_bm_t* h, int n_pairs,
                               const uint8_t* left, ptrdiff_t left_stride, ptrdiff_t left_pair_stride,
                               const uint8_t* right, ptrdiff_t right_stride, ptrdiff_t right_pair_stride,
                               int W, int H,
                               int16_t* disp_left, ptrdiff_t disp_left_stride, ptrdiff_t disp_left_pair_stride,
                               int16_t* disp_right, ptrdiff_t disp_right_stride, ptrdiff_t disp_right_pair_stride,
                               void* stream);
int adf_bm_compute_host(adf_bm_t* h, int n_pairs,
                        const uint8_t* left, ptrdiff_t left_stride, ptrdiff_t left_pair_stride,
                        const uint8_t* right, ptrdiff_t right_stride, ptrdiff_t right_pair_stride,
                        int W, int H,
                        int16_t* disparity, ptrdiff_t disp_stride, ptrdiff_t disp_pair_stride);
int adf_bm_compute_cost_device(adf_bm_t* h, int n_pairs,
                               const uint8_t* left, ptrdiff_t left_stride, ptrdiff_t left_pair_stride,
                               const uint8_t* right, ptrdiff_t right_stride, ptrdiff_t right_pair_stride,
                               int W, int H,
                               int16_t* disparity, ptrdiff_t disp_stride, ptrdiff_t disp_pair_stride,
                               int16_t* cost, ptrdiff_t cost_stride, ptrdiff_t cost_pair_stride,
                               void* stream);
int adf_bm_compute_cost_host(adf_bm_t* h, int n_pairs,
                             const uint8_t* left, ptrdiff_t left_stride, ptrdiff_t left_pair_stride,
                             const uint8_t* right, ptrdiff_t right_stride, ptrdiff_t right_pair_stride,
                             int W, int H,
                             int16_t* disparity, ptrdiff_t disp_stride, ptrdiff_t disp_pair_stride,
                             int16_t* cost, ptrdiff_t cost_stride, ptrdiff_t cost_pair_stride);
int adf_bm_compute_both_cost_device(adf_bm_t* h, int n_pairs,
                                    const uint8_t* left, ptrdiff_t left_stride, ptrdiff_t left_pair_stride,
                                    const uint8_t* right, ptrdiff_t right_stride, ptrdiff_t right_pair_stride,
                                    int W, int H,
                                    int16_t* disp_left, ptrdiff_t disp_left_stride, ptrdiff_t disp_left_pair_stride,
                                    int16_t* disp_right, ptrdiff_t disp_right_stride, ptrdiff_t disp_right_pair_stride,
                                    int16_t* cost_left, ptrdiff_t cost_left_stride, ptrdiff_t cost_left_pair_stride,
                                    int16_t* cost_right, ptrdiff_t cost_right_stride, ptrdiff_t cost_right_pair_stride,
                                    void* stream);

#define ADF_SGBM_MODE_SGBM 0
#define ADF_SGBM_MODE_HH 1
// ... 254 lines not shown
```

Baseline: 44310.

## Store vertical weights as 16-bit LUT indices and expand in the vertical pass

The weights kernel can now write Cvert as 16-bit indices into the colour LUT instead of f32 weights, clamped at the table's first zero entry. The vertical wave pass reads these indices, expands them through a shared-memory copy of the table head, and falls back to buffer loads for indices beyond the head. This halves the bytes written and read for Cvert on every iteration. In exchange it adds index expansion and possible scattered LUT gathers inside the solver pass, and it only applies when the image hand-off runs at every iteration.

```diff
diff --git a/addingdisparityfiltering_amd/__init__.py b/addingdisparityfiltering_amd/__init__.py
--- a/addingdisparityfiltering_amd/__init__.py
+++ b/addingdisparityfiltering_amd/__init__.py
@@ -15,6 +15,8 @@
     BORDER_REPLICATE,
     BORDER_WRAP,
     COLOR_BGR2GRAY,
+    CVERT_FLOAT,
+    CVERT_INDEX16,
     CV_16S,
     CV_32F,
     CV_32FC1,
diff --git a/addingdisparityfiltering_amd/_lib.py b/addingdisparityfiltering_amd/_lib.py
--- a/addingdisparityfiltering_amd/_lib.py
+++ b/addingdisparityfiltering_amd/_lib.py
@@ -9,6 +9,7 @@
 PATH_CONF_BAND, PATH_FUSED_FIRST_PASS, PATH_MERGED_PREP, PATH_SCALED_FUSED, PATH_SCALED_HALF = 1, 2, 4, 8, 16
 PATH_ROW_WEIGHTS_GUIDE = 32
 HANDOFF_PAIR_PLANE, HANDOFF_IMAGE, HANDOFF_IMAGE_PAIR_TAIL = 0, 1, 2
+CVERT_FLOAT, CVERT_INDEX16 = 0, 1
 DEPTH_8U, DEPTH_16S, DEPTH_32S, DEPTH_32F = 0, 3, 4, 5
 SGBM_COST_BT, SGBM_COST_CENSUS_DENSE, SGBM_COST_CENSUS_SPARSE = 0, 1, 2
 BM_COST_SAD, BM_COST_CENSUS_DENSE, BM_COST_CENSUS_SPARSE = 0, 1, 2
@@ -98,6 +99,7 @@
     ("adf_wls_get_last_solver_path", _i, [_vp, C.POINTER(_i)]),
     ("adf_wls_get_last_handoff", _i, [_vp, C.POINTER(_i)]),
     ("adf_wls_get_inner_handoffs", _i, [_vp, C.POINTER(_i), C.POINTER(_i)]),
+    ("adf_wls_get_cvert_form", _i, [_vp, C.POINTER(_i), C.POINTER(_i)]),
     ("adf_wls_filter_device", _i, _FILTER_DEV),
     ("adf_wls_filter_host", _i, _FILTER_DEV[:-1]),
     ("adf_wls_filter_scaled_device", _i, _FILTER_SCALED_DEV),
@@ -121,6 +123,7 @@
     ("adf_fgs_destroy", None, [_vp]),
     ("adf_release_cached_memory", None, []),
     ("adf_weight_table_host", _i, [C.c_float, _vp, _i]),
+    ("adf_cvert_index_host", _i, [C.c_float, _i, C.POINTER(_i), C.POINTER(_i)]),
     ("adf_fgs_get_device", _i, [_vp, C.POINTER(_i)]),
     ("adf_fgs_get_solver", _i, [_vp, C.POINTER(_i)]),
     ("adf_fgs_filter_host", _i, [_vp, _vp, _pd, _vp, _pd, _i, _i]),
diff --git a/addingdisparityfiltering_amd/csrc/adf_api.hip b/addingdisparityfiltering_amd/csrc/adf_api.hip
--- a/addingdisparityfiltering_amd/csrc/adf_api.hip
+++ b/addingdisparityfiltering_amd/csrc/adf_api.hip
@@ -107,6 +107,7 @@
 
 struct HandoffImage {
     float* image = nullptr; int m = 0; bool inner = false, first = false;
+    const float* index_lut = nullptr;
     bool at(int it, int num_iter) const
     {
         if (!image || num_iter < 2) return false;
@@ -146,7 +147,8 @@
             if (ho.at(it, num_iter)) {
                 h.image = v.image = ho.image; h.image_m = v.image_m = ho.m;
                 h.image_plane = v.image_plane = wave_image_floats(g.pw, ho.m);
-            }
+                if (ho.index_lut) { v.c_index = 1; v.gw.lut = ho.index_lut; }
+            } else if (ho.index_lut) return fail(ADF_EBADARG, "run_passes: Cvert as indices needs the image at every hand-off");
             {
                 ProfScope ps(prof, fused ? K_PASS_H_FIRST : K_PASS_H, hb, hb, st);
                 HIP_TRY(launch_wave_hpass(h, n_rhs, n_pairs, st));
@@ -224,6 +226,8 @@
     long long handoff_min_px = HANDOFF_IMAGE_MIN_PX;
     int last_handoff = ADF_HANDOFF_PAIR_PLANE;
     int last_inner[2] = {0, 0};
+    bool cvert_index = true;
+    int last_cvert[2] = {ADF_CVERT_FLOAT, ADF_CVERT_FLOAT};
     static bool null_caller_of(hipStream_t s) { return s == nullptr || s == hipStreamLegacy || s == hipStreamPerThread; }
     int ensure_side(hipStream_t caller)
     {
@@ -267,6 +271,7 @@
     if (const char* e = getenv("ADF_INNER_HANDOFF_IMAGE")) h->handoff_inner = atoi(e) != 0;
     if (const char* e = getenv("ADF_LAST_HANDOFF_MIN_PX")) h->handoff_min_px = atoll(e);
     if (const char* e = getenv("ADF_MERGE_SMALL")) h->merge_small = atoi(e) != 0;
+    if (const char* e = getenv("ADF_CVERT_INDEX")) h->cvert_index = atoi(e) != 0;
     *out = h;
     return ADF_OK;
 }
@@ -319,6 +324,14 @@
     NEED_HANDLE(h);
     if (full) *full = h->last_inner[0];
     if (tail) *tail = h->last_inner[1];
+    return ADF_OK;
+}
+
+extern "C" int adf_wls_get_cvert_form(const adf_wls_t* h, int* full, int* tail)
+{
+    NEED_HANDLE(h);
+    if (full) *full = h->last_cvert[0];
+    if (tail) *tail = h->last_cvert[1];
     return ADF_OK;
 }
 
@@ -645,6 +658,7 @@
     bool guide_rows;
     bool image;
     bool inner_image;
+    bool cvert_index;
 };
 
 struct WlsPlan {
@@ -667,7 +681,7 @@
 static ChunkPlan plan_chunk(const adf_wls* h, ConfStage stage, bool wave, bool guide_rows, bool image, bool inner_image)
 {
     const bool fork = stage != CONF_NONE && stage != CONF_MERGED && h->overlap;
-    return ChunkPlan{stage, fork, fork && wave && stage != CONF_TWO_KERNEL, guide_rows && stage != CONF_MERGED, image, image && inner_image};
+    return ChunkPlan{stage, fork, fork && wave && stage != CONF_TWO_KERNEL, guide_rows && stage != CONF_MERGED, image, image && inner_image, false};
 }
 
 static GuideWeights guide_weights(const adf_wls* h, const uint8_t* guide, const View& v, const Geom& g)
@@ -727,7 +741,10 @@
     if (image_m && roi_px * p.chunk < h->handoff_min_px) chunk_for(0);
     auto chunk_of = [&](int n) {
         const bool merged = p.band && h->merge_small && prep_small_fits(g, h->disc_radius, v.ch, n) && prep_small_guide_fits(g, v.stride, v.ch);
-        return plan_chunk(h, merged ? CONF_MERGED : stage, p.wave, guide_rows, p.image_m && roi_px * n >= h->handoff_min_px, h->handoff_inner);
+        ChunkPlan cp = plan_chunk(h, merged ? CONF_MERGED : stage, p.wave, guide_rows, p.image_m && roi_px * n >= h->handoff_min_px, h->handoff_inner);
+        cp.cvert_index = h->cvert_index && cvert_index_allowed(v.ch, h->lut.cur_t) && cp.guide_rows && h->num_iter >= 2 &&
+                         cp.image && cp.inner_image && p.first_image;
+        return cp;
     };
     p.first_image = p.rhs == RHS_FUSED_VIEW && wave_hpass_first_image(view_fuse(planes, m, g));
     p.full = chunk_of(p.chunk);
@@ -838,7 +855,10 @@
     const int16_t fill = (int16_t)(16 * (h->min_disp - 1));
     const ConfRule rule = conf_rule(h, c);
     h->last_path = plan.path; h->last_solver_path = plan.solver_path;
-    auto handoff_of = [&](const ChunkPlan& cp) { return HandoffImage{cp.image ? image : nullptr, plan.image_m, cp.inner_image, cp.inner_image && plan.first_image}; };
+    auto handoff_of = [&](const ChunkPlan& cp) {
+        return HandoffImage{cp.image ? image : nullptr, plan.image_m, cp.inner_image, cp.inner_image && plan.first_image, cp.cvert_index ? h->lut.cur : nullptr};
+    };
+    h->last_cvert[0] = plan.full.cvert_index ? ADF_CVERT_INDEX16 : ADF_CVERT_FLOAT; h->last_cvert[1] = plan.tail.cvert_index ? ADF_CVERT_INDEX16 : ADF_CVERT_FLOAT;
     if (wave) { h->last_inner[0] = handoff_of(plan.full).inner_count(h->num_iter); h->last_inner[1] = handoff_of(plan.tail).inner_count(h->num_iter); }
     h->last_handoff = (plan.full.image && plan.tail.image) ? ADF_HANDOFF_IMAGE : plan.full.image ? ADF_HANDOFF_IMAGE_PAIR_TAIL : ADF_HANDOFF_PAIR_PLANE;
 
@@ -857,6 +877,7 @@
         };
         WeightArgs wa{gv, vw.stride, vw.pair_stride, gch, h->lut.cur, cp.guide_rows ? nullptr : p.CH, p.CV, orient_h, orient_cv, g,
                       wave ? nullptr : p.B0};
+        if (cp.cvert_index) wa.cvert_t = h->lut.cur_t < CVERT_INDEX_MAX ? h->lut.cur_t : CVERT_INDEX_MAX;
         const GuideWeights gw = guide_weights(h, gv, vw, g);
         auto prologue = [&](bool weighted) {
             PlainPrologueArgs pa{m.rhs, m.s_rhs, m.ps_rhs, m.rhs_depth, 1, 0, p.A0, g, weighted ? orient_u2 : orient_h};
diff --git a/addingdisparityfiltering_amd/csrc/adf_host.h b/addingdisparityfiltering_amd/csrc/adf_host.h
--- a/addingdisparityfiltering_amd/csrc/adf_host.h
+++ b/addingdisparityfiltering_amd/csrc/adf_host.h
@@ -122,11 +122,16 @@
     struct Entry { std::shared_ptr<LutTable> t; unsigned long long used; };
     std::vector<Entry> tables;
     const float* cur = nullptr;
+    int cur_t = 0;
     unsigned long long tick = 0;
     size_t bytes() const { return tables.size() * sizeof(float) * ADF_LUT_LEVELS; }
     int ensure(float s, hipStream_t st);
     void release() { tables.clear(); cur = nullptr; }
 };
+
+ADF_LOCAL int lut_first_zero(const float* table);
+constexpr int CVERT_INDEX_MAX = 0xFFFE;
+inline bool cvert_index_allowed(int channels, int t) { return channels == 1 || t <= CVERT_INDEX_MAX; }
 
 struct WmfTable;
 ADF_LOCAL int wmf_weights_check(const char* who, double sigma, int weight_type);
diff --git a/addingdisparityfiltering_amd/csrc/adf_host.hip b/addingdisparityfiltering_amd/csrc/adf_host.hip
--- a/addingdisparityfiltering_amd/csrc/adf_host.hip
+++ b/addingdisparityfiltering_amd/csrc/adf_host.hip
@@ -3,6 +3,7 @@
 #include <cmath>
 #include <cstdarg>
 #include <cstdio>
+#include <cstring>
 #include <mutex>
 #include <thread>
 
@@ -106,7 +107,7 @@
     DeviceTable& operator=(const DeviceTable&) = delete;
     ~DeviceTable() { if (dev) { DeviceScope ds(device); hipFree(dev); } }
 };
-struct adf::LutTable : DeviceTable<float, float> {};
+struct adf::LutTable : DeviceTable<float, float> { int t = 0; };
 
 template <class TABLE> struct TableStore {
     static constexpr size_t CAP = 16;
@@ -185,10 +186,22 @@
     if (done < n) span(done, n);
 }
 
+int adf::lut_first_zero(const float* table)
+{
+    int t = ADF_LUT_LEVELS;
+    while (t > 0) {
+        uint32_t bits;
+        memcpy(&bits, &table[t - 1], sizeof(bits));
+        if (bits != 0x80000000u) break;
+        t--;
+    }
+    return t;
+}
+
 int adf::Lut::ensure(float s, hipStream_t st)
 {
     for (auto& e : tables)
-        if (e.t->key == s) { e.used = ++tick; cur = e.t->dev; return ADF_OK; }
+        if (e.t->key == s) { e.used = ++tick; cur = e.t->dev; cur_t = e.t->t; return ADF_OK; }
     if ((int)tables.size() >= LUT_CACHE) {
         size_t lru = 0;
         for (size_t k = 1; k < tables.size(); k++) if (tables[k].used < tables[lru].used) lru = k;
@@ -206,11 +219,11 @@
         hipError_t e = hipMemcpy(d, host.data(), sizeof(float) * ADF_LUT_LEVELS, hipMemcpyHostToDevice);
         if (e != hipSuccess) { hipFree(d); return fail(ADF_EHIP, "LUT upload failed: %s", hipGetErrorString(e)); }
         t = std::make_shared<LutTable>();
-        t->device = device; t->key = s; t->count = ADF_LUT_LEVELS; t->dev = d;
+        t->device = device; t->key = s; t->count = ADF_LUT_LEVELS; t->dev = d; t->t = lut_first_zero(host.data());
         LutStore::get().add(t);
     }
     tables.push_back(Entry{t, ++tick});
-    cur = t->dev;
+    cur = t->dev; cur_t = t->t;
     return ADF_OK;
 }
 
@@ -457,6 +470,18 @@
     return ADF_OK;
 }
 
+extern "C" int adf_cvert_index_host(float sigma_color, int channels, int* first_zero, int* allowed)
+{
+    if (!(sigma_color >= 0.0f)) return fail(ADF_EBADARG, "sigma_color must be >= 0 (FGS.cpp:143)");
+    if (channels != 1 && channels != 3) return fail(ADF_EBADARG, "guides have one or three channels");
+    std::vector<float> host(ADF_LUT_LEVELS);
+    lut_build_host(sigma_color, host.data());
+    const int t = lut_first_zero(host.data());
+    if (first_zero) *first_zero = t;
+    if (allowed) *allowed = cvert_index_allowed(channels, t) ? 1 : 0;
+    return ADF_OK;
+}
+
 namespace adf {
 hipError_t device_malloc(void** p, size_t bytes)
 {
diff --git a/addingdisparityfiltering_amd/csrc/adf_internal.h b/addingdisparityfiltering_amd/csrc/adf_internal.h
--- a/addingdisparityfiltering_amd/csrc/adf_internal.h
+++ b/addingdisparityfiltering_amd/csrc/adf_internal.h
@@ -110,6 +110,7 @@
     float* chor; float* cvert; int chor_orient, cvert_orient;
     Geom g;
     float* scratch;
+    int cvert_t;
 };
 
 struct PassArgs {
@@ -152,10 +153,11 @@
     float lambda;
     GuideWeights gw;
     float* image; size_t image_plane; int image_m;
+    int c_index;
 };
 static_assert(sizeof(WavePassArgs) == 352 && offsetof(WavePassArgs, out) == 208 && offsetof(WavePassArgs, nscan) == 248 &&
               offsetof(WavePassArgs, plane) == 264 && offsetof(WavePassArgs, lambda) == 272 && offsetof(WavePassArgs, gw) == 280 &&
-              offsetof(WavePassArgs, image) == 328 && sizeof(GuideWeights) == 48, "WavePassArgs layout");
+              offsetof(WavePassArgs, image) == 328 && offsetof(WavePassArgs, c_index) == 348 && sizeof(GuideWeights) == 48, "WavePassArgs layout");
 
 hipError_t launch_discontinuity(const DiscArgs& a, int n_pairs, hipStream_t st);
 hipError_t launch_lrc_prologue(const LrcArgs& a, int n_pairs, hipStream_t st);
diff --git a/addingdisparityfiltering_amd/csrc/fgs_wave_v.hip b/addingdisparityfiltering_amd/csrc/fgs_wave_v.hip
--- a/addingdisparityfiltering_amd/csrc/fgs_wave_v.hip
+++ b/addingdisparityfiltering_amd/csrc/fgs_wave_v.hip
@@ -1,4 +1,5 @@
 #include "fgs_wave_common.h"
+#include "prep_bodies.h"
 
 namespace adf {
 
@@ -83,9 +84,25 @@
     return (unsigned)pitch * 4u;
 }
 
-template <int M, int R, int EPI, int VCW = VC, int NCH = 64, bool IMG = false>
+constexpr int CIDX_WINDOW = 17;
+
+__device__ __forceinline__ float cidx_head(const float* lut_head, unsigned k)
+{
+    const float hv = lut_head[min(k, (unsigned)prep::WS_LUT_HEAD - 1u)];
+    return k < (unsigned)prep::WS_LUT_HEAD ? hv : __uint_as_float(k == 0xffffu ? 0u : k);
+}
+__device__ __forceinline__ v2f cidx_expand(const float* lut_head, unsigned w) { return (v2f){cidx_head(lut_head, w & 0xffffu), cidx_head(lut_head, w >> 16)}; }
+__device__ __forceinline__ bool cidx_pending(float v) { return (int)__float_as_uint(v) > 0; }
+__device__ __forceinline__ unsigned cidx_fetch(const __amdgpu_buffer_rsrc_t& lutwin, float v)
+{
+    return __builtin_amdgcn_raw_buffer_load_b32(lutwin, cidx_pending(v) ? __float_as_uint(v) * 4u : prep::WS_DROP, 0, 0);
+}
+__device__ __forceinline__ float cidx_take(float v, unsigned g) { return cidx_pending(v) ? __uint_as_float(g) : v; }
+
+template <int M, int R, int EPI, int VCW = VC, int NCH = 64, bool IMG = false, bool CIDX = false>
 __global__ void __launch_bounds__(VT) wave_vpass_kernel(WavePassArgs a)
 {
+    static_assert(!CIDX || (IMG && VT * 4 == prep::WS_LUT_HEAD), "indices: with the image; one float4 of the table's head per thread");
     static_assert((VCW == 16 && NCH == 64) || (VCW == 8 && NCH == 128), "whole strips of 64 chunks or half strips of 128");
     static_assert(!IMG || (R == 2 && VCW == VC && (EPI == EPI_PLANES || EPI == EPI_WLS_CONF || EPI == EPI_WLS_CONF_F32)), "the image: whole strips, both right-hand sides, the plain pass or the filter's epilogues");
     static_assert((VCW / 2) * NCH == VT, "one thread per (chunk, column pair)");
@@ -122,16 +139,32 @@
     const unsigned safe = (R > 1) ? ((unsigned)strip * (32u * TR) + c16) * 4u : (unsigned)col * 4u;
     const unsigned csafe = ((unsigned)strip * (unsigned)h * VC + c16) * 4u;
     v2f a_s = vsplat(0.0f);
+    if constexpr (!CIDX) {
     if (cidx > 0 && r0 - 1 < h) a_s = *reinterpret_cast<const v2f*>(bC + (coff0 - pitch_c)) * vsplat(a.lambda);
+    }
     {
         unsigned voff = voff0, coff = coff0;
         const v2f lam = vsplat(a.lambda);
         const char* bI = IMG ? reinterpret_cast<const char*>(a.image + (size_t)blockIdx.y * a.image_plane) : nullptr;
         unsigned ioff = (((unsigned)strip * (NCH / 8) + ((unsigned)tid >> 6)) * (unsigned)M) * 1024u + ((unsigned)tid & 63u) * 16u;
+        float* const lut_head = &red[0][0][0];
+        v4f head4;
+        unsigned as_w = 0;
+        const bool has_as = cidx > 0 && r0 - 1 < h;
+        if constexpr (CIDX) {
+            head4 = *reinterpret_cast<const v4f*>(a.gw.lut + 4 * tid);
+            as_w = *reinterpret_cast<const unsigned*>(bC + ((has_as ? coff0 - pitch_c : csafe) >> 1));
+#pragma unroll
+            for (int i = 0; i < M; i++) {
+                c[i].x = __uint_as_float(*reinterpret_cast<const unsigned*>(bC + ((r0 + i < h ? coff : csafe) >> 1)));
+                coff += pitch_c;
+                ADF_STEP_FENCE();
+            }
+        }
 #pragma unroll
         for (int i = 0; i < M; i++) {
             const bool ok = r0 + i < h;
-            c[i] = *reinterpret_cast<const v2f*>(bC + (ok ? coff : csafe));
+            if constexpr (!CIDX) c[i] = *reinterpret_cast<const v2f*>(bC + (ok ? coff : csafe));
             if constexpr (IMG) {
                 const v4f q = *reinterpret_cast<const v4f*>(bI + ioff);
                 f0[i] = (v2f){q.x, q.y}; f1[i] = (v2f){q.z, q.w};
@@ -144,6 +177,35 @@
             }
             coff += pitch_c;
             ADF_STEP_FENCE();
+        }
+        if constexpr (CIDX) {
+            *reinterpret_cast<v4f*>(lut_head + 4 * tid) = head4;
+            __syncthreads();
+            v2f as_c = cidx_expand(lut_head, as_w);
+            bool pending = cidx_pending(as_c.x) || cidx_pending(as_c.y);
+#pragma unroll
+            for (int i = 0; i < M; i++) {
+                c[i] = cidx_expand(lut_head, __float_as_uint(c[i].x));
+                pending = pending || cidx_pending(c[i].x) || cidx_pending(c[i].y);
+            }
+            if (__builtin_amdgcn_ballot_w64(pending) != 0) {
+                const __amdgpu_buffer_rsrc_t lutwin = prep::ws_window(a.gw.lut, sizeof(float) * ADF_LUT_LEVELS);
+                const unsigned ga0 = cidx_fetch(lutwin, as_c.x), ga1 = cidx_fetch(lutwin, as_c.y);
+#pragma unroll
+                for (int i0 = 0; i0 < M; i0 += CIDX_WINDOW) {
+                    unsigned g[CIDX_WINDOW][2];
+#pragma unroll
+                    for (int k = 0; k < CIDX_WINDOW; k++)
+                        if (i0 + k < M) { g[k][0] = cidx_fetch(lutwin, c[i0 + k].x); g[k][1] = cidx_fetch(lutwin, c[i0 + k].y); }
+                    ADF_STEP_FENCE();
+#pragma unroll
+                    for (int k = 0; k < CIDX_WINDOW; k++)
+                        if (i0 + k < M) c[i0 + k] = (v2f){cidx_take(c[i0 + k].x, g[k][0]), cidx_take(c[i0 + k].y, g[k][1])};
+                    ADF_STEP_FENCE();
+                }
+                as_c = (v2f){cidx_take(as_c.x, ga0), cidx_take(as_c.y, ga1)};
+            }
+            if (has_as) a_s = as_c * lam;
         }
 #pragma unroll
         for (int i = 0; i < M; i++) c[i] *= lam;
@@ -269,10 +331,15 @@
             if (a.image) {
                 if constexpr (R == 2 && VCW == VC && (EPI == EPI_PLANES || EPI == EPI_WLS_CONF || EPI == EPI_WLS_CONF_F32)) {
                     if (a.image_m != M || a.image_plane < wave_image_floats(a.pitch, M)) return hipErrorInvalidValue;
+                    if (a.c_index) {
+                        if (!a.gw.lut) return hipErrorInvalidValue;
+                        hipLaunchKernelGGL((wave_vpass_kernel<M, R, EPI, VCW, NCH, true, true>), grid, block, 0, st, a);
+                    } else
                     hipLaunchKernelGGL((wave_vpass_kernel<M, R, EPI, VCW, NCH, true>), grid, block, 0, st, a);
                     return hipGetLastError();
                 } else return hipErrorInvalidValue;
             }
+            if (a.c_index) return hipErrorInvalidValue;
             hipLaunchKernelGGL((wave_vpass_kernel<M, R, EPI, VCW, NCH>), grid, block, 0, st, a);
             return hipGetLastError();
         }
diff --git a/addingdisparityfiltering_amd/csrc/prep_bodies.h b/addingdisparityfiltering_amd/csrc/prep_bodies.h
--- a/addingdisparityfiltering_amd/csrc/prep_bodies.h
+++ b/addingdisparityfiltering_amd/csrc/prep_bodies.h
@@ -170,18 +170,31 @@
         if (strip) __builtin_amdgcn_raw_buffer_store_b128(o, cvert, off, 0, 0);
         else __builtin_amdgcn_raw_buffer_store_b128(o, cvert, off, 0, 2);
     }
+    __device__ __forceinline__ void store_v_index(int t, const int (&vidx)[WS_COLS], unsigned tmax, bool last_row, bool on) const
+    {
+        const unsigned last = last_row ? 0u : 0xffffffffu;
+        unsigned k16[WS_COLS];
+#pragma unroll
+        for (int k = 0; k < WS_COLS; k++) k16[k] = (mv[k] & last) ? min((unsigned)vidx[k], tmax) : 0xffffu;
+        const ws_v2u o = {k16[0] | (k16[1] << 16), k16[2] | (k16[3] << 16)};
+        const unsigned off = (on && st_ok) ? (vo + (unsigned)t * vstep) >> 1 : WS_DROP;
+        __builtin_amdgcn_raw_buffer_store_b64(o, cvert, off, 0, 0);
+    }
 };
 
-template <int CH, bool HOR = true>
+template <int CH, bool HOR = true, bool IDX = false>
 __device__ __forceinline__ void weights_stream_body(const WeightArgs& a, int bx, int by, int nby, size_t pz, WsShared<CH>& sh, bool active)
 {
     static_assert(CH == 1 || CH == 3, "guides have one or three channels");
+    static_assert(!IDX || !HOR, "the index form is Cvert's");
     float (&lut_head)[WS_LUT_HEAD] = sh.lut_head;
     const Geom& g = a.g;
     const int tid = active ? (int)threadIdx.x : 0;
-    if (active)
-        for (int q = tid; q < WS_LUT_HEAD; q += WS_NT) lut_head[q] = a.lut[q];
-    __syncthreads();
+    if constexpr (!IDX) {
+        if (active)
+            for (int q = tid; q < WS_LUT_HEAD; q += WS_NT) lut_head[q] = a.lut[q];
+        __syncthreads();
+    }
     const int ws_rows = (g.rh + nby - 1) / nby;
     const int x0 = bx * WS_BCOLS, y0 = by * ws_rows;
     if (!active || y0 >= g.rh) return;
@@ -208,10 +221,15 @@
 #pragma unroll
     for (int s = 0; s < WS_U; s++) nxt[s] = load(s < nrows ? s : nrows - 1);
     WsPending pend;
+    int pend_idx[WS_COLS];
+    const unsigned tmax = (unsigned)a.cvert_t;
     {
         int hidx[WS_COLS], vidx[WS_COLS];
         ws_indices<CH, HOR>(nxt[0], row_off(0) & 3u, pv, hidx, vidx);
-        ws_lookup_issue<HOR>(lut_head, lutwin, hidx, vidx, pend);
+        if constexpr (IDX) {
+#pragma unroll
+            for (int k = 0; k < WS_COLS; k++) pend_idx[k] = vidx[k];
+        } else ws_lookup_issue<HOR>(lut_head, lutwin, hidx, vidx, pend);
     }
     for (int n0 = 0; n0 < nrows; n0 += WS_U) {
 #pragma unroll
@@ -224,21 +242,25 @@
 #pragma unroll
         for (int s = 0; s < WS_U; s++) {
             const int n = n0 + s;
-            WsPending ahead;
-            {
-                int hidx[WS_COLS], vidx[WS_COLS];
-                ws_indices<CH, HOR>(s + 1 < WS_U ? cur[s + 1 < WS_U ? s + 1 : 0] : nxt[0], row_off(min(n + 1, nrows - 1)) & 3u, pv, hidx, vidx);
+            int hidx[WS_COLS], vidx[WS_COLS];
+            ws_indices<CH, HOR>(s + 1 < WS_U ? cur[s + 1 < WS_U ? s + 1 : 0] : nxt[0], row_off(min(n + 1, nrows - 1)) & 3u, pv, hidx, vidx);
+            if constexpr (IDX) {
+                out.store_v_index(n - 1, pend_idx, tmax, y0 + n - 1 == g.rh - 1, n >= 1 && n < nrows);
+#pragma unroll
+                for (int k = 0; k < WS_COLS; k++) pend_idx[k] = vidx[k];
+            } else {
+                WsPending ahead;
                 ws_lookup_issue<HOR>(lut_head, lutwin, hidx, vidx, ahead);
+                float wh[WS_COLS], wv[WS_COLS];
+                ws_lookup_finish<HOR>(pend, wh, wv);
+                if constexpr (HOR) out.store_h(n, wh, n < nrows - 1);
+                out.store_v(n - 1, wv, y0 + n - 1 == g.rh - 1, n >= 1 && n < nrows);
+                pend = ahead;
             }
-            float wh[WS_COLS], wv[WS_COLS];
-            ws_lookup_finish<HOR>(pend, wh, wv);
-            if constexpr (HOR) out.store_h(n, wh, n < nrows - 1);
-            out.store_v(n - 1, wv, y0 + n - 1 == g.rh - 1, n >= 1 && n < nrows);
-            pend = ahead;
-        }
-    }
-}
-
-
-}
-}
+        }
+    }
+}
+
+
+}
+}
diff --git a/addingdisparityfiltering_amd/csrc/weights_kernels.hip b/addingdisparityfiltering_amd/csrc/weights_kernels.hip
--- a/addingdisparityfiltering_amd/csrc/weights_kernels.hip
+++ b/addingdisparityfiltering_amd/csrc/weights_kernels.hip
@@ -96,11 +96,11 @@
     }
 }
 
-template <int CH, bool HOR>
+template <int CH, bool HOR, bool IDX = false>
 __global__ void __launch_bounds__(prep::WS_NT) weights_stream_kernel(WeightArgs a)
 {
     __shared__ prep::WsShared<CH> sh;
-    prep::weights_stream_body<CH, HOR>(a, blockIdx.x, blockIdx.y, gridDim.y, blockIdx.z, sh, true);
+    prep::weights_stream_body<CH, HOR, IDX>(a, blockIdx.x, blockIdx.y, gridDim.y, blockIdx.z, sh, true);
 }
 
 __global__ void __launch_bounds__(256) transpose_n_to_t_kernel(const float* __restrict__ src, float* __restrict__ dst, Geom g)
@@ -139,6 +139,7 @@
 hipError_t launch_weights(const WeightArgs& a, int n_pairs, hipStream_t st)
 {
     const bool hor = a.chor != nullptr;
+    if (a.cvert_t && (hor || a.cvert_orient != ORIENT_STRIP || a.cvert_t < 1 || a.cvert_t > 0xFFFE || !weights_stream_fits(a))) return hipErrorInvalidValue;
     if (a.chor_orient == ORIENT_T && a.cvert_orient == ORIENT_N && a.scratch) {
         WeightArgs b = a;
         b.chor = a.scratch; b.chor_orient = ORIENT_N; b.scratch = nullptr;
@@ -158,7 +159,9 @@
             while (rpb > 1 && (size_t)(rpb + 1) * (size_t)a.stride >= ((size_t)1 << 30)) rpb >>= 1;
             sgrid.y = (a.g.rh + rpb - 1) / rpb;
         }
-        if (a.ch == 1 && hor) hipLaunchKernelGGL((weights_stream_kernel<1, true>), sgrid, dim3(prep::WS_NT), 0, st, a);
+        if (a.cvert_t && a.ch == 1) hipLaunchKernelGGL((weights_stream_kernel<1, false, true>), sgrid, dim3(prep::WS_NT), 0, st, a);
+        else if (a.cvert_t && a.ch == 3) hipLaunchKernelGGL((weights_stream_kernel<3, false, true>), sgrid, dim3(prep::WS_NT), 0, st, a);
+        else if (a.ch == 1 && hor) hipLaunchKernelGGL((weights_stream_kernel<1, true>), sgrid, dim3(prep::WS_NT), 0, st, a);
         else if (a.ch == 1) hipLaunchKernelGGL((weights_stream_kernel<1, false>), sgrid, dim3(prep::WS_NT), 0, st, a);
         else if (a.ch == 3 && hor) hipLaunchKernelGGL((weights_stream_kernel<3, true>), sgrid, dim3(prep::WS_NT), 0, st, a);
         else if (a.ch == 3) hipLaunchKernelGGL((weights_stream_kernel<3, false>), sgrid, dim3(prep::WS_NT), 0, st, a);
diff --git a/addingdisparityfiltering_amd/ximgproc.py b/addingdisparityfiltering_amd/ximgproc.py
--- a/addingdisparityfiltering_amd/ximgproc.py
+++ b/addingdisparityfiltering_amd/ximgproc.py
@@ -15,7 +15,7 @@
 from ._lib import DTF_NC, DTF_IC, DTF_RF, DT_MAX_ITERS, DT_NC_MAX_RADIUS
 from ._lib import RGF_MAX_ITERS, AM_MAX_TREE_HEIGHT
 from ._lib import JBF_MAX_RADIUS, BORDER_REPLICATE, BORDER_REFLECT, BORDER_WRAP, BORDER_REFLECT_101
-from ._lib import AdfError, HANDOFF_IMAGE, HANDOFF_IMAGE_PAIR_TAIL, HANDOFF_PAIR_PLANE, PATH_CONF_BAND, PATH_FUSED_FIRST_PASS, PATH_MERGED_PREP, PATH_ROW_WEIGHTS_GUIDE, PATH_SCALED_FUSED, PATH_SCALED_HALF, Rect, SOLVER_EXACT, SOLVER_WAVE
+from ._lib import AdfError, CVERT_FLOAT, CVERT_INDEX16, HANDOFF_IMAGE, HANDOFF_IMAGE_PAIR_TAIL, HANDOFF_PAIR_PLANE, PATH_CONF_BAND, PATH_FUSED_FIRST_PASS, PATH_MERGED_PREP, PATH_ROW_WEIGHTS_GUIDE, PATH_SCALED_FUSED, PATH_SCALED_HALF, Rect, SOLVER_EXACT, SOLVER_WAVE
 
 try:
     import torch
@@ -219,6 +219,11 @@
     def getInnerHandoffs(self):
         full, tail = C.c_int(0), C.c_int(0)
         _lib.check(_lib.lib().adf_wls_get_inner_handoffs(self._h, C.byref(full), C.byref(tail)))
+        return full.value, tail.value
+
+    def getCvertForm(self):
+        full, tail = C.c_int(0), C.c_int(0)
+        _lib.check(_lib.lib().adf_wls_get_cvert_form(self._h, C.byref(full), C.byref(tail)))
         return full.value, tail.value
 
     def enableProfiling(self, on=True):
diff --git a/include/adf_wls.h b/include/adf_wls.h
--- a/include/adf_wls.h
+++ b/include/adf_wls.h
@@ -64,6 +64,9 @@
 #define ADF_HANDOFF_IMAGE_PAIR_TAIL 2
 int adf_wls_get_last_handoff(const adf_wls_t* h, int* form);
 int adf_wls_get_inner_handoffs(const adf_wls_t* h, int* full, int* tail);
+#define ADF_CVERT_FLOAT 0
+#define ADF_CVERT_INDEX16 1
+int adf_wls_get_cvert_form(const adf_wls_t* h, int* full, int* tail);
 
 int adf_wls_filter_device(adf_wls_t* h, int n_pairs,
                           const int16_t* disp_left, ptrdiff_t disp_left_stride, ptrdiff_t disp_left_pair_stride,
@@ -174,6 +177,7 @@
 void adf_release_cached_memory(void);
 #define ADF_WEIGHT_TABLE_LEVELS (3 * 256 * 256)
 int adf_weight_table_host(float sigma_color, float* table, int levels);
+int adf_cvert_index_host(float sigma_color, int channels, int* first_zero, int* allowed);
 int adf_fgs_get_device(const adf_fgs_t* h, int* device);
 int adf_fgs_get_solver(const adf_fgs_t* h, int* solver);
 
```

Result: no change. 44610 (median of 6 runs) (+0.7%).
